# hyeeiin/ECG-Multimodal-Model

Hardware: AMD Instinct MI355X
Metric: samples/sec fwd+bwd, batch-256 multimodal (img+sig+clin), 1->8 MI355X (higher is better)
Workload: dtype bf16; 1 GPU; full multimodal (image 3x224x224 + 5000-pt signal + 16-dim clinical), fwd+bwd+Adam, encoders unfrozen; image_hw=224x224, per_gpu_batch=256, global_batch=256, parallelism=dp1

## Files before the change

ecg-multimodal-model_amd/csrc/api.hip:

```cpp
#include <stdarg.h>

#include "ops.h"

static thread_local char g_err[512] = "";

void ecg_set_error(const char* fmt, ...) {
  va_list ap;
  va_start(ap, fmt);
  vsnprintf(g_err, sizeof(g_err), fmt, ap);
  va_end(ap);
}

static inline ConvGeom geom_of(const ecgmm_conv_desc* c) {
  return make_geom(c->N, c->H, c->W, c->Cin, c->Cout, c->R, c->S, c->stride, c->pad_h, c->pad_w);
}
#define S_(x) ((hipStream_t)(x))

extern "C" {

int ecgmm_version(void) { return ECGMM_VERSION; }
const char* ecgmm_last_error(void) { return g_err; }

const char* ecgmm_switch_name(int i) { return i >= 0 && i < sw::COUNT ? sw::ALL[i]->env : nullptr; }
int ecgmm_switch_get(const char* env_name, int64_t* value) {
// ... 172 lines not shown
                      const float* addc, const void* y_a, const float* coef_a, const float* gamma_a, float* dgamma_a,
                      float* dbeta_a, void* dy_a, const void* y_b, const float* coef_b, const float* gamma_b,
                      float* dgamma_b, float* dbeta_b, void* dy_b, void* dz, float* dbias, int64_t M, int C, void* scratch_a,
                      void* scratch_b, void* stream) {
  return ecg_bn_bwd_dual(dtype, dout, maskref, mask_bits, gate, addc, y_a, coef_a, gamma_a, dgamma_a, dbeta_a, dy_a, y_b,
                         coef_b, gamma_b, dgamma_b, dbeta_b, dy_b, dz, dbias, (long)M, C, (float*)scratch_a, (float*)scratch_b,
                         S_(stream));
}

int ecgmm_conv_bwd_data_bnred(int dtype, const ecgmm_conv_desc* c, const void* dy, const void* w_dgrad,
                              const void* addend, void* dx, const void* bn_y, const void* bn_mask, const float* bn_coef,
                              float* rows, int* nrows, void* stream) {
  if (!bn_y || !bn_coef || !rows || !nrows) ECG_FAIL(ECGMM_ERR_SHAPE, "conv_bwd_data_bnred: null BatchNorm operand");
  const ConvGeom g = geom_of(c);
  *nrows = 0;
  if (!ecg_conv_halo_ok(dtype, 1, g))
    return ecg_conv_igemm(dtype, 1, g, dy, w_dgrad, dx, nullptr, addend, nullptr, 0, S_(stream));
  ConvEpi e = {};
  e.wg_rows = 1; e.red_y = bn_y; e.red_mask = bn_mask; e.red_coef = bn_coef; e.red_rows = rows;
  int rc = ecg_conv_igemm(dtype, 1, g, dy, w_dgrad, dx, nullptr, addend, nullptr, 0, S_(stream), &e);
  if (rc == 0 && e.red_done) *nrows = e.red_rows_n;
  return rc;
}
int ecgmm_conv_fwd_wgrows(int dtype, const ecgmm_conv_desc* c, const void* x, const void* w_fwd, const float* bias, void* y,
                          float* stats, int* nrows, int act, void* stream) {
  if (!stats || !nrows) ECG_FAIL(ECGMM_ERR_SHAPE, "conv_fwd_wgrows: null statistics buffer / row count");
  const ConvGeom g = geom_of(c);
  ConvEpi e = {};
  e.wg_rows = 1;
  int rc = ecg_conv_igemm(dtype, 0, g, x, w_fwd, y, bias, nullptr, stats, act, S_(stream), &e);
  *nrows = e.stats_rows > 0 ? e.stats_rows : ecg_conv_stats_rows((long)g.N * g.OH * g.OW);
  return rc;
}
int ecgmm_conv_bwd_data_bnred_rows(int dtype, const ecgmm_conv_desc* c) {
  const ConvGeom g = geom_of(c);
  return ecg_conv_halo_ok(dtype, 1, g) ? ecg_conv_halo_rows(1, g) : 0;
}
int ecgmm_conv_bwd_data_with_downsample(int dtype, const ecgmm_conv_desc* c, const void* dy, const void* w_dgrad,
                                        const void* dy_down, const void* w_down_dgrad, void* dx, void* tmp,
                                        void* stream) {
  if (!dy_down || !w_down_dgrad) ECG_FAIL(ECGMM_ERR_SHAPE, "conv_bwd_data_with_downsample: null downsample operand");
  const ConvGeom g = geom_of(c);
  if (g.stride != 2) ECG_FAIL(ECGMM_ERR_SHAPE, "conv_bwd_data_with_downsample: stride %d (the main convolution must have stride 2)", g.stride);
  ConvEpi e = {};
  e.src2 = dy_down; e.wpk2 = w_down_dgrad;
  ECG_TRY(ecg_conv_igemm(dtype, 1, g, dy, w_dgrad, dx, nullptr, nullptr, nullptr, 0, S_(stream), &e));
  if (e.src2_done) return 0;
  if (!tmp) ECG_FAIL(ECGMM_ERR_WORKSPACE, "conv_bwd_data_with_downsample: this geometry needs the temporary");
  ConvGeom gd = g;
  gd.R = gd.S = 1; gd.pad_h = gd.pad_w = 0;
  ECG_TRY(ecg_conv_igemm(dtype, 1, gd, dy_down, w_down_dgrad, tmp, nullptr, nullptr, nullptr, 0, S_(stream)));
  return ecg_conv_igemm(dtype, 1, g, dy, w_dgrad, dx, nullptr, tmp, nullptr, 0, S_(stream));
}
int ecgmm_bn_bwd_from_rows(int dtype, const void* dout, const void* maskref, const void* y, const float* coef,
                           const float* gamma, float* dgamma, float* dbeta, void* dy, const float* rows, int nrows,
                           int64_t M, int C, void* scratch, void* stream) {
  return ecg_bn_bwd_tail(dtype, dout, maskref, y, coef, gamma, dgamma, dbeta, dy, rows, nrows, (long)M, C,
                         (float*)scratch, S_(stream));
}

int ecgmm_bnrelu_maxpool(int dtype, const void* y, const float* coef, void* out, uint8_t* idx, int N, int H, int W,
                         int C, void* stream) {
  return ecg_bnrelu_maxpool(dtype, y, coef, out, idx, N, H, W, C, S_(stream));
}
int ecgmm_maxpool_relu_bwd(int dtype, const void* dp, const void* pooled, const uint8_t* idx, void* dz, int N, int H,
                           int W, int C, void* stream) {
  return ecg_maxpool_relu_bwd(dtype, dp, pooled, idx, dz, N, H, W, C, S_(stream));
}
int ecgmm_pool_bn_bwd(int dtype, const void* dp, const void* pooled, const uint8_t* idx, const void* y, const float* coef,
                      const float* gamma, float* dgamma, float* dbeta, void* dy, float* dbias, int N, int H, int W, int C,
                      void* scratch, void* stream) {
  return ecg_pool_bn_bwd(dtype, dp, pooled, idx, y, coef, gamma, dgamma, dbeta, dy, dbias, N, H, W, C, (float*)scratch,
                         S_(stream));
}
int ecgmm_conv_fwd_fused(int dtype, const ecgmm_conv_desc* c, const void* x, const void* w_fwd, const float* bias,
                         const void* addend, void* y, int act, void* stream) {
  if (dtype != ECGMM_BF16 && dtype != ECGMM_F32) ECG_FAIL(ECGMM_ERR_DTYPE, "conv_fwd_fused: bad dtype %d", dtype);
  if (!c || !x || !w_fwd || !y) ECG_FAIL(ECGMM_ERR_SHAPE, "conv_fwd_fused: null operand");
  if (act != ECGMM_ACT_NONE && act != ECGMM_ACT_RELU) ECG_FAIL(ECGMM_ERR_SHAPE, "conv_fwd_fused: act %d (none or ReLU)", act);
  if (c->N < 1 || c->H < 1 || c->W < 1 || c->Cin < 1 || c->Cout < 1 || c->R < 1 || c->S < 1 || c->stride < 1 ||
      c->pad_h < 0 || c->pad_w < 0 || c->H + 2 * c->pad_h < c->R || c->W + 2 * c->pad_w < c->S)
    ECG_FAIL(ECGMM_ERR_SHAPE, "conv_fwd_fused: bad geometry");
  return ecg_conv_igemm(dtype, 0, geom_of(c), x, w_fwd, y, bias, addend, nullptr, act, S_(stream));
}
int ecgmm_fold_conv_bn(int dtype, int layout, const float* w, const float* conv_bias, const float* gamma, const float* beta,
                       const float* running_mean, const float* running_var, float eps, void* w_out, float* b_out,
                       float* scale_out, int Cout, int Cin, int RS, void* stream) {
  if (layout != 0 && layout != 1) ECG_FAIL(ECGMM_ERR_SHAPE, "fold_conv_bn: layout %d (0 = forward pack, 1 = stem pack)", layout);
  if (dtype != ECGMM_BF16 && dtype != ECGMM_F32) ECG_FAIL(ECGMM_ERR_DTYPE, "fold_conv_bn: bad dtype %d", dtype);
  if (layout == 0 && RS > 9)
    ECG_FAIL(ECGMM_ERR_SHAPE, "fold_conv_bn: %d taps unsupported (1..9; a 5x5 convolution folds through ecgmm_fold_conv5_bn)", RS);
  EcgFoldItem it = {};
  it.kind = layout == 1 ? ECG_FOLD_STEM : ECG_FOLD_CONV;
  it.w = w; it.conv_bias = conv_bias; it.gamma = gamma; it.beta = beta; it.rm = running_mean; it.rv = running_var;
  it.wout = w_out; it.bout = b_out; it.scale_out = scale_out; it.Cout = Cout; it.Cin = Cin; it.RS = RS;
  return ecg_fold_batch(dtype, &it, 1, eps, S_(stream));
}
int ecgmm_fold_conv5_bn(int dtype, int layout, const float* w, const float* conv_bias, const float* gamma, const float* beta,
                        const float* running_mean, const float* running_var, float eps, void* w_out, float* b_out,
                        float* scale_out, int Cout, int Cin, void* stream) {
  if (layout != 0 && layout != 1)
    ECG_FAIL(ECGMM_ERR_SHAPE, "fold_conv5_bn: layout %d (0 = forward pack, 1 = OIHW fp32)", layout);
  EcgFoldItem it = {};
  it.kind = layout == 1 ? ECG_FOLD_OIHW : ECG_FOLD_CONV;
  it.w = w; it.conv_bias = conv_bias; it.gamma = gamma; it.beta = beta; it.rm = running_mean; it.rv = running_var;
  it.wout = w_out; it.bout = b_out; it.scale_out = scale_out; it.Cout = Cout; it.Cin = Cin; it.RS = 25;
// ... 193 lines not shown
```

ecg-multimodal-model_amd/csrc/common.h:

```cpp
#pragma once
#include <hip/hip_runtime.h>
#include <stdint.h>
#include <stdio.h>
#include <stdlib.h>
#include <string.h>

#include "../../include/ecgmm.h"

typedef unsigned short bf16_t;
typedef __attribute__((ext_vector_type(4))) float f32x4;
typedef __attribute__((ext_vector_type(8))) __bf16 bf16x8_t;
typedef __attribute__((ext_vector_type(4))) short s16x4;
typedef __attribute__((ext_vector_type(4))) unsigned int u32x4;

#define ECG_WAVE 64
#define ECG_TAIL_ROWS 64

void ecg_set_error(const char* fmt, ...);
#define ECG_FAIL(code, ...)       \
  do {                            \
    ecg_set_error(__VA_ARGS__);   \
    return (code);                \
  } while (0)
#define ECG_CHECK_LAUNCH(name)                                                     \
  do {                                                                             \
    hipError_t e_ = hipGetLastError();                                             \
    if (e_ != hipSuccess) ECG_FAIL(ECGMM_ERR_LAUNCH, "%s: %s", name, hipGetErrorString(e_)); \
  } while (0)
#define ECG_TRY(expr)             \
  do {                            \
    int rc_ = (expr);             \
    if (rc_ != 0) return rc_;     \
  } while (0)

__device__ __forceinline__ float bf2f(bf16_t v) { return __uint_as_float(((unsigned)v) << 16); }
__device__ __forceinline__ bf16_t f2bf(float f) {
  __bf16 b = (__bf16)f;
  return __builtin_bit_cast(bf16_t, b);
}

template <typename T> struct Elem;
template <> struct Elem<float> {
  static constexpr int VEC = 4;
  __device__ static __forceinline__ float ld(const float* p) { return *p; }
  __device__ static __forceinline__ void st(float* p, float v) { *p = v; }
};
template <> struct Elem<bf16_t> {
  static constexpr int VEC = 8;
  __device__ static __forceinline__ float ld(const bf16_t* p) { return bf2f(*p); }
  __device__ static __forceinline__ void st(bf16_t* p, float v) { *p = f2bf(v); }
};

template <typename T> __device__ __forceinline__ void unpack16(const u32x4& v, float* f);
template <> __device__ __forceinline__ void unpack16<float>(const u32x4& v, float* f) {
#pragma unroll
  for (int i = 0; i < 4; ++i) f[i] = __uint_as_float(v[i]);
}
template <> __device__ __forceinline__ void unpack16<bf16_t>(const u32x4& v, float* f) {
#pragma unroll
  for (int i = 0; i < 4; ++i) {
    f[2 * i] = __uint_as_float(v[i] << 16);
    f[2 * i + 1] = __uint_as_float(v[i] & 0xFFFF0000u);
  }
}
template <typename T> __device__ __forceinline__ u32x4 pack16(const float* f);
template <> __device__ __forceinline__ u32x4 pack16<float>(const float* f) {
  u32x4 v;
#pragma unroll
  for (int i = 0; i < 4; ++i) v[i] = __float_as_uint(f[i]);
  return v;
}
template <> __device__ __forceinline__ u32x4 pack16<bf16_t>(const float* f) {
  u32x4 v;
#pragma unroll
  for (int i = 0; i < 4; ++i) v[i] = (unsigned)f2bf(f[2 * i]) | ((unsigned)f2bf(f[2 * i + 1]) << 16);
  return v;
}

__device__ __forceinline__ float wave_sum(float v) {
#pragma unroll
  for (int o = 32; o > 0; o >>= 1) v += __shfl_xor(v, o, 64);
  return v;
}
__device__ __forceinline__ float wave_max(float v) {
#pragma unroll
  for (int o = 32; o > 0; o >>= 1) v = fmaxf(v, __shfl_xor(v, o, 64));
  return v;
}

template <int CTRL> __device__ __forceinline__ float dpp_mov(float v) {
  return __int_as_float(__builtin_amdgcn_update_dpp(0, __float_as_int(v), CTRL, 0xF, 0xF, true));
}
__device__ __forceinline__ float row16_sum(float v) {
  v += dpp_mov<0xB1>(v);
  v += dpp_mov<0x4E>(v);
  v += dpp_mov<0x141>(v);
  v += dpp_mov<0x140>(v);
  return v;
}

__device__ __forceinline__ void mfma_bf16_inplace(f32x4& acc, const u32x4& a, const u32x4& b) {
#if defined(__HIP_DEVICE_COMPILE__)
  asm volatile("s_nop 1\n\tv_mfma_f32_16x16x32_bf16 %0, %1, %2, %0" : "+a"(acc) : "v"(a), "v"(b));
#endif
}
__device__ __forceinline__ void mfma_bf16_first(f32x4& acc, const u32x4& a, const u32x4& b) {
#if defined(__HIP_DEVICE_COMPILE__)
  asm volatile("s_nop 1\n\tv_mfma_f32_16x16x32_bf16 %0, %1, %2, 0" : "=a"(acc) : "v"(a), "v"(b));
#endif
}
__device__ __forceinline__ void mfma_drain() {
#if defined(__HIP_DEVICE_COMPILE__)
  asm volatile("s_nop 7\n\ts_nop 7\n\ts_nop 3" ::: "memory");
#endif
}

static inline bool env_on(const char* name) { const char* e = getenv(name); return !(e && e[0] == '0'); }
static inline bool env_off(const char* name) { const char* e = getenv(name); return e && e[0] == '1'; }
static inline long env_int(const char* name, long def) { const char* e = getenv(name); return e ? atol(e) : def; }
static inline int env_level(const char* name, int hi, int def) {
  const char* e = getenv(name);
  return e && e[0] >= '0' && e[0] <= '0' + hi ? e[0] - '0' : def;
}

static inline int ceil_div(long a, long b) { return (int)((a + b - 1) / b); }
static inline size_t align_up(size_t a, size_t b) { return (a + b - 1) / b * b; }
static inline size_t dtype_size(int dt) { return dt == ECGMM_BF16 ? 2 : 4; }

struct ConvGeom {
  int N, H, W, Cin;
// ... 13 lines not shown
```

ecg-multimodal-model_amd/csrc/conv_halo.hip:

```cpp
#include <type_traits>

#include "ops.h"

namespace {

constexpr int HBM_ = 256;
constexpr unsigned H_OOB = 0x80000000u;

#ifdef ECG_STAMP
__device__ unsigned long long g_hstamp[8];
#define HSTAMP_AT(t)                                                          \
  do {                                                                        \
    __builtin_amdgcn_sched_barrier(0);                                        \
    asm volatile("s_memtime %0\n\ts_waitcnt lgkmcnt(0)" : "=s"(t)::"memory"); \
    __builtin_amdgcn_sched_barrier(0);                                        \
  } while (0)
#endif

struct HaloParams {
  const void* src;
  const void* wpk;
  void* dst;
  const float* bias;
  const void* addend;
  float* stats;
  const void* red_y;
  const void* red_mask;
  const float* red_coef;
  float* red_rows;
  int wg_rows;
  int M, H, W, Cs, Cd, ph, pw, act;
  int ncs;
  int HL;
  int hrows;
  int ntm;
  int ntn;
  int stagger;
  unsigned mul_hw, sh_hw, mul_w, sh_w;
};

__device__ __forceinline__ void hdma16(__amdgpu_buffer_rsrc_t rs, unsigned char* lds_wave_base, unsigned voffset,
                                       unsigned soffset) {
#if defined(__HIP_DEVICE_COMPILE__)
  __builtin_amdgcn_raw_ptr_buffer_load_lds(rs, (__attribute__((address_space(3))) void*)lds_wave_base, 16, voffset,
                                           soffset, 0, 0);
#endif
}

template <int N> __device__ __forceinline__ void wait_vmcnt() {
#if defined(__HIP_DEVICE_COMPILE__)
  asm volatile("s_waitcnt vmcnt(%0)" ::"n"(N) : "memory");
#endif
}
__device__ __forceinline__ void wait_lds() {
#if defined(__HIP_DEVICE_COMPILE__)
  __builtin_amdgcn_s_waitcnt(0xC07F);
#endif
}

typedef __attribute__((ext_vector_type(2))) float f32x2_t;
typedef __attribute__((ext_vector_type(2))) __bf16 bf16x2_t;
__device__ __forceinline__ unsigned pack_bf16x2(float lo, float hi) {
  return __builtin_bit_cast(unsigned, __builtin_convertvector((f32x2_t){lo, hi}, bf16x2_t));
}

template <int BN, int NW = 8> struct HaloCfg {
  static_assert(NW == 8 || (NW == 4 && BN == 64), "4-wave workgroups: 64-channel tiles only");
  static constexpr int HCAP = BN == 128 ? 320 : 384;
  static constexpr int HBUF = (HCAP + 8) * 128;
  static constexpr int NHB = NW == 8 ? 2 : 1;
  static constexpr int WSTAGE = BN * 128;
  static constexpr int NWS = NW == 8 ? 4 : 3;
  static constexpr int WBASE = NHB * HBUF;
  static constexpr int SBASE = WBASE + NWS * WSTAGE;
  static constexpr int CBASE = SBASE + 4 * 2 * BN * 4;
  static constexpr int TRASH = CBASE + 3 * BN * 4;
  static constexpr int MBASE = TRASH + 256;
  static constexpr int MBUF = 6 * 256 * 4;
  static constexpr int LDS = MBASE + (BN == 64 && NW == 8 ? 2 * MBUF : 0);
  static constexpr int WPS = BN / (8 * NW);
  static constexpr int NPW_MAX = HCAP / (8 * NW);
  static constexpr int WCN = NW / 4;
  static constexpr int CPW = BN / WCN;
};

template <int BN, int RS, int MODE, bool NCS1 = false, int NW = 8, bool PP = false, bool ST = false, bool AD = false>
__global__ __launch_bounds__(NW * 64, NW == 8 ? 2 : 2) void conv_halo_kernel(HaloParams p) {
  using C = HaloCfg<BN, NW>;
  static_assert(!ST || (BN == 64 && RS == 9 && NCS1 && NW == 8 && !PP && MODE != 1), "stream form: 64 -> 64 channel 3x3 tiles, no fused reduction");
  static_assert(!AD || (ST && MODE == 2), "AD = the stream form of the input gradient with a residual addend");
  static_assert(!PP || (NW == 8 && !NCS1), "ping-pong: 8-wave workgroups");
  static_assert(!(NCS1 && NW == 4), "one halo buffer: the next tile's halo cannot stream in during the K loop");
  static_assert(NW == 8 || RS % 3 == 0, "3-slot ring: the slot of a step is its tap index mod 3");
  constexpr int HTHREADS = NW * 64;
  constexpr int D = C::NWS - 1;
  constexpr int TP = 4;
  constexpr int TC = C::CPW / 16;
#ifndef HALO_HPS9
#define HALO_HPS9 1
#endif
  constexpr int HPS = RS == 9 ? HALO_HPS9 : C::NPW_MAX;
  extern __shared__ __attribute__((aligned(16))) unsigned char smem[];

  const int tid = threadIdx.x;
  const int lane = tid & 63;
  const int wv = __builtin_amdgcn_readfirstlane(tid >> 6);
  const int wp = wv & 3, wc = wv >> 2;
  const bool late = !PP && NW == 8 && BN == 64 && p.stagger != 0 && wv >= 4;
  auto slot_of = [](int g, int t) -> int { return C::NWS == 4 ? (g & 3) : (t % 3); };
  auto hbuf_of = [](int q) -> unsigned { return C::NHB == 2 ? (unsigned)(q & 1) * C::HBUF : 0u; };
  const int fr = lane & 15, fq = lane >> 4;
  const int G = gridDim.x;
  const int nt = (int)blockIdx.x % p.ntn, kq = (int)blockIdx.x / p.ntn, Gk = G / p.ntn;
  const int n0 = nt * BN;
  const unsigned pixb = (unsigned)p.Cs * 2u;
  const __amdgpu_buffer_rsrc_t rs_src = __builtin_amdgcn_make_buffer_rsrc((void*)p.src, 0, (int)((size_t)p.M * pixb), 0x00020000);
  const __amdgpu_buffer_rsrc_t rs_w = __builtin_amdgcn_make_buffer_rsrc(
      (void*)p.wpk, 0, (int)((size_t)p.Cd * RS * p.Cs * 2), 0x00020000);

  const int lrow8 = lane >> 3;
  const unsigned lchunkb = (unsigned)(((lane & 7) ^ lrow8) << 4);
  unsigned hoff[C::NPW_MAX];
  auto set_hoff = [&](int m0) {
#pragma unroll
    for (int kk = 0; kk < C::NPW_MAX; ++kk) {
      const int row = (kk * NW + wv) * 8 + lrow8;
      const int pix = m0 - p.HL + row;
      const bool ok = row < p.hrows && pix >= 0 && pix < p.M;
      hoff[kk] = ok ? (unsigned)pix * pixb + lchunkb : H_OOB;
    }
  };
  auto set_wrow = [&](unsigned (&wr)[C::WPS], int n0) {
#pragma unroll
    for (int i = 0; i < C::WPS; ++i) wr[i] = (unsigned)(n0 + (i * NW + wv) * 8 + lrow8) * (unsigned)RS * pixb + lchunkb;
  };
  auto dma_halo = [&](unsigned hbuf, int cs, int k0, int k1) {
#pragma unroll
    for (int kk = 0; kk < C::NPW_MAX; ++kk)
      if (kk >= k0 && kk < k1) hdma16(rs_src, smem + hbuf + (kk * NW + wv) * 1024, hoff[kk], (unsigned)cs * 128u);
  };
  auto dma_w = [&](const unsigned (&wr)[C::WPS], int slot, int cs, int t) {
// ... 96 lines not shown
        acc[a][b] = __builtin_amdgcn_mfma_f32_16x16x32_bf16(__builtin_bit_cast(bf16x8_t, fa[a]),
                                                            __builtin_bit_cast(bf16x8_t, fb[b]), (f32x4){0.f, 0.f, 0.f, 0.f}, 0, 0, 0);
    __builtin_amdgcn_s_setprio(0);
  };
  auto mma = [&](const u32x4 (&fa)[TC], const u32x4 (&fb)[TP]) {
#if defined(HALO_ABL) && HALO_ABL == 1
#pragma unroll
    for (int a = 0; a < TC; ++a) asm volatile("" ::"v"(fa[a]));
#pragma unroll
    for (int b = 0; b < TP; ++b) asm volatile("" ::"v"(fb[b]));
    return;
#endif
    __builtin_amdgcn_s_setprio(1);
#pragma unroll
    for (int a = 0; a < TC; ++a)
#pragma unroll
      for (int b = 0; b < TP; ++b)
        acc[a][b] = __builtin_amdgcn_mfma_f32_16x16x32_bf16(__builtin_bit_cast(bf16x8_t, fa[a]),
                                                            __builtin_bit_cast(bf16x8_t, fb[b]), acc[a][b], 0, 0, 0);
    __builtin_amdgcn_s_setprio(0);
  };

  int mt = kq;
  int m0 = mt * HBM_;
  unsigned wrow[C::WPS];
  set_wrow(wrow, n0);
  int g0 = 0;
  int qs = 0;
  auto tile_fills = [&](int m0_, bool with_halo) {
    if (with_halo) {
      set_hoff(m0_);
      dma_halo(hbuf_of(qs), 0, 0, C::NPW_MAX);
    }
#pragma unroll
    for (int t = 0; t < D; ++t) dma_w(wrow, slot_of(g0 + t, t), 0, t);
  };
  if (tid < 8 * C::NHB) *reinterpret_cast<u32x4*>(smem + (tid >> 3) * C::HBUF + C::HCAP * 128 + (tid & 7) * 16) = (u32x4){0u, 0u, 0u, 0u};
  float* const sacc = reinterpret_cast<float*>(smem + C::SBASE);
  for (int i = tid; i < 4 * 2 * BN; i += HTHREADS) sacc[i] = 0.f;
  float* const scoef = reinterpret_cast<float*>(smem + C::CBASE);
  if (MODE == 1 && p.red_y)
    for (int i = tid; i < 3 * BN; i += HTHREADS) scoef[i] = p.red_coef[(i / BN) * p.Cd + n0 + (i % BN)];
  tile_fills(m0, true);

  u32x4 fa0[TC], fb0[TP], fa1[TC], fb1[TP];

  const bf16_t* const pf_base[3] = {(const bf16_t*)p.addend, MODE == 1 ? (const bf16_t*)p.red_y : nullptr,
                                    MODE == 1 && p.red_mask != p.red_y ? (const bf16_t*)p.red_mask : nullptr};
  auto prefetch_epilogue_operands = [&]() {
#if defined(__HIP_DEVICE_COMPILE__)
    const size_t e = (size_t)(m0 + wp * 64 + lane) * p.Cd + n0 + wc * C::CPW;
#pragma unroll
    for (int k = 0; k < 3; ++k) {
      const bf16_t* g = pf_base[k] ? pf_base[k] + e : (const bf16_t*)p.wpk;
      __builtin_amdgcn_global_load_lds((const __attribute__((address_space(1))) void*)g,
                                       (__attribute__((address_space(3))) void*)(smem + C::TRASH), 4, 0, 0);
    }
#endif
  };

  auto slice = [&](int cs, auto last_tag) {
    constexpr bool LAST = decltype(last_tag)::value;
    const unsigned hb = hbuf_of(qs), hbn = hbuf_of(qs + 1);
#pragma unroll
    for (int b = 0; b < TP; ++b)
#pragma unroll
      for (int t2 = 0; t2 < RSP; ++t2) asm volatile("" : "+v"(baddr[b][t2]));
#pragma unroll
    for (int t = 0; t < RS; ++t) {
      const int s = g0 + t;
      ld_a(fa1, slot_of(s, t), 64u);
#pragma unroll
      for (int b = 0; b < TP; ++b) fb1[b] = ld_b((bad(b, t) ^ 64u) + hb);
      const auto n_halo = [](int tt, bool last) { return (!(last && !NCS1) && tt < RS - 1 && tt * HPS < C::NPW_MAX)
                                                      ? ((tt + 1) * HPS < C::NPW_MAX ? HPS : C::NPW_MAX - tt * HPS) : 0; };
      const auto n_fill = [&](int tt, bool last) {
        return ((last && tt + D >= RS) ? 0 : C::WPS) + n_halo(tt, last) + ((last && tt == 0) ? 3 : 0);
      };
      const bool wrap = t + D >= RS;
      if (LAST && t == 0) prefetch_epilogue_operands();
#if !(defined(HALO_ABL) && HALO_ABL == 3)
      if (!(LAST && wrap)) dma_w(wrow, slot_of(s + D, (t + D) % RS), cs + (wrap ? 1 : 0), (t + D) % RS);
      if (n_halo(t, LAST) > 0) dma_halo(hbn, NCS1 ? 0 : cs + 1, t * HPS, (t + 1) * HPS);
#endif
      if (!late) mma(fa0, fb0);
      const int outstanding = (D == 3 ? (t == 0 ? n_fill(RS - 1, false) : n_fill(t - 1, LAST)) : 0) + n_fill(t, LAST);
      if (outstanding == 0) wait_vmcnt<0>();
      else if (outstanding == 1) wait_vmcnt<1>();
      else if (outstanding == 2) wait_vmcnt<2>();
      else if (outstanding == 3) wait_vmcnt<3>();
      else if (outstanding == 4) wait_vmcnt<4>();
      else if (outstanding == 5) wait_vmcnt<5>();
      else if (outstanding == 6) wait_vmcnt<6>();
      else if (outstanding == 7) wait_vmcnt<7>();
      else if (outstanding == 8) wait_vmcnt<8>();
      else if (outstanding == 9) wait_vmcnt<9>();
      else if (outstanding == 10) wait_vmcnt<10>();
      else if (outstanding == 11) wait_vmcnt<11>();
      else if (outstanding == 12) wait_vmcnt<12>();
      else if (outstanding == 13) wait_vmcnt<13>();
      else if (outstanding == 14) wait_vmcnt<14>();
      else if (outstanding == 15) wait_vmcnt<15>();
      else wait_vmcnt<0>();
      wait_lds();
#if !(defined(HALO_ABL) && HALO_ABL == 5)
      __builtin_amdgcn_s_barrier();
#endif
// ... 72 lines not shown
  constexpr bool RACC = BN == 64 && MODE == 0 && NW == 8;
#endif
  constexpr int TA_ = TC / 2;
  float rs1[RACC && MODE == 0 ? TC : 1][4], rs2[RACC && MODE == 0 ? TC : 1][4];
  float rq1[RACC && MODE == 1 ? TA_ : 1][8], rq2[RACC && MODE == 1 ? TA_ : 1][8];
#pragma unroll
  for (int a = 0; a < (RACC && MODE == 0 ? TC : 1); ++a)
#pragma unroll
    for (int j = 0; j < 4; ++j) rs1[a][j] = rs2[a][j] = 0.f;
#pragma unroll
  for (int a = 0; a < (RACC && MODE == 1 ? TA_ : 1); ++a)
#pragma unroll
    for (int j = 0; j < 8; ++j) rq1[a][j] = rq2[a][j] = 0.f;
  const bool racc = RACC && p.wg_rows != 0;
  bool first_tile = true;
#ifdef ECG_STAMP
  unsigned long long hs_a, hs_b, hs_c, hs_d, hs_e, hs_w0, hs_acc[4] = {0, 0, 0, 0}, hs_tiles = 0, hs_bar = 0;
  HSTAMP_AT(hs_w0);
#endif
  if constexpr (ST) {
    auto produce_masks = [&](int m0_, unsigned buf) {
      const int pixel = tid & 255;
      const int q = m0_ + pixel;
      const int n = (int)(((unsigned long long)(unsigned)q * p.mul_hw) >> p.sh_hw), rem = q - n * HW;
      const int h = (int)(((unsigned long long)(unsigned)rem * p.mul_w) >> p.sh_w), w = rem - h * p.W;
      const unsigned first_r = MODE == 0 ? 0x007u : 0x1C0u, last_r = MODE == 0 ? 0x1C0u : 0x007u;
      const unsigned first_s = MODE == 0 ? 0x049u : 0x124u, last_s = MODE == 0 ? 0x124u : 0x049u;
      unsigned v = 0x1FFu;
      v &= h == 0 ? ~first_r : ~0u;
      v &= h == p.H - 1 ? ~last_r : ~0u;
      v &= w == 0 ? ~first_s : ~0u;
      v &= w == p.W - 1 ? ~last_s : ~0u;
      const int k0 = wc * 3;
      unsigned* tb = reinterpret_cast<unsigned*>(smem + C::MBASE + buf * C::MBUF) + k0 * 256 + pixel;
#pragma unroll
      for (int j = 0; j < 3; ++j) {
        const unsigned lo = (unsigned)__builtin_amdgcn_sbfe((int)v, 2 * (k0 + j), 1) & 0xFFFFu;
        const unsigned hi = (unsigned)__builtin_amdgcn_sbfe((int)v, 2 * (k0 + j) + 1, 1) & 0xFFFF0000u;
        tb[j * 256] = lo | hi;
      }
    };
    unsigned mk[TP];
    const unsigned mlane = (unsigned)C::MBASE + (unsigned)(wp * 64 + fr) * 4u;
    auto fetch_masks = [&](int t2, unsigned buf) {
#pragma unroll
      for (int b = 0; b < TP; ++b) mk[b] = *reinterpret_cast<const unsigned*>(smem + mlane + buf * C::MBUF + t2 * 1024 + b * 64);
    };
    auto rebuild = [&](int t2) {
      const unsigned zz = zaddr | (zaddr << 16);
#pragma unroll
      for (int b = 0; b < TP; ++b) baddr[b][t2] = (avalid[b][t2] & mk[b]) | (zz & ~mk[b]);
    };
    constexpr auto st_ = [](int t) { t = (t + RS) % RS; return AD ? (t >= 4 && t <= 7 ? 1 : 0) : (t >= 1 && t <= 4 ? 1 : 0); };
    constexpr auto ld_ = [](int t) { t = (t + RS) % RS; return AD && t >= 1 && t <= 4 ? 1 : 0; };
    constexpr auto pf_ = [](int t) { t = (t + RS) % RS; return AD && t == 5 ? 1 : 0; };
    constexpr auto ex_ = [=](int t) { return st_(t) + ld_(t) + pf_(t); };
    constexpr auto hl_ = [](int t) { t = (t + RS) % RS; return t < C::NPW_MAX ? 1 : 0; };
    static_assert(C::NPW_MAX <= RS - 1 && HPS == 1, "one halo piece per step, none in the tile's last step");
    const int cw = n0 + wc * C::CPW;
    const int cl = (fq & 1) ? 16 + (fq - 1) * 4 : fq * 4;
    f32x4 accp[TC][TP];
    static_assert(TC == 2, "one channel-tile pair per wave");
    u32x4 adv[3];
    auto load_addend = [&](int b, int m0_) {
      adv[b % 3] = *reinterpret_cast<const u32x4*>(addend + (size_t)(m0_ + wp * 64 + b * 16 + fr) * p.Cd + cw + cl);
    };
    auto prefetch_addend = [&](int m0_) {
#if defined(__HIP_DEVICE_COMPILE__)
      __builtin_amdgcn_global_load_lds((const __attribute__((address_space(1))) void*)(addend + (size_t)(m0_ + wp * 64 + lane) * p.Cd + cw),
                                       (__attribute__((address_space(3))) void*)(smem + C::TRASH), 4, 0, 0);
#endif
    };
    auto epi_unit = [&](int b, int m0_) {
#if defined(__HIP_DEVICE_COMPILE__)
      f32x4 v0 = accp[0][b], v1 = accp[1][b];
      if constexpr (AD) {
        const u32x4 ao = adv[b % 3];
        auto ax = __builtin_amdgcn_permlane16_swap(ao[0], ao[2], false, false);
        auto ay = __builtin_amdgcn_permlane16_swap(ao[1], ao[3], false, false);
        v0 += (f32x4){__uint_as_float(ax[0] << 16), __uint_as_float(ax[0] & 0xFFFF0000u), __uint_as_float(ay[0] << 16), __uint_as_float(ay[0] & 0xFFFF0000u)};
        v1 += (f32x4){__uint_as_float(ax[1] << 16), __uint_as_float(ax[1] & 0xFFFF0000u), __uint_as_float(ay[1] << 16), __uint_as_float(ay[1] & 0xFFFF0000u)};
      }
      if constexpr (MODE == 0) {
        if (b < TC) {
          f32x4 t1, t2;
#pragma unroll
          for (int bb = 0; bb < TP; ++bb) {
            const f32x4 v = accp[b][bb];
#pragma unroll
            for (int j = 0; j < 4; ++j) {
              t1[j] = bb == 0 ? v[j] : t1[j] + v[j];
              t2[j] = __builtin_fmaf(v[j], v[j], bb == 0 ? 0.f : t2[j]);
            }
          }
#pragma unroll
          for (int j = 0; j < 4; ++j) {
            rs1[b][j] += t1[j];
            rs2[b][j] += t2[j];
          }
        }
      }
      const unsigned x0 = pack_bf16x2(v0[0], v0[1]), y0 = pack_bf16x2(v0[2], v0[3]);
      const unsigned x1 = pack_bf16x2(v1[0], v1[1]), y1 = pack_bf16x2(v1[2], v1[3]);
      auto lo = __builtin_amdgcn_permlane16_swap(x0, x1, false, false);
      auto hi = __builtin_amdgcn_permlane16_swap(y0, y1, false, false);
#if defined(HALO_ABL) && HALO_ABL == 11
      asm volatile("" ::"v"(lo[0]), "v"(hi[0]), "v"(lo[1]), "v"(hi[1]));
      __builtin_amdgcn_global_load_lds((const __attribute__((address_space(1))) void*)p.wpk,
                                       (__attribute__((address_space(3))) void*)(smem + C::TRASH), 4, 0, 0);
#else
      *reinterpret_cast<u32x4*>(dst + (size_t)(m0_ + wp * 64 + b * 16 + fr) * p.Cd + cw + cl) = (u32x4){lo[0], hi[0], lo[1], hi[1]};
#endif
#endif
    };
    auto dummy_vm = [&]() {
#if defined(__HIP_DEVICE_COMPILE__)
      __builtin_amdgcn_global_load_lds((const __attribute__((address_space(1))) void*)p.wpk,
                                       (__attribute__((address_space(3))) void*)(smem + C::TRASH), 4, 0, 0);
#endif
    };
    set_baddr(m0);
    produce_masks(m0, 0u);
    set_hoff(mt + Gk < p.ntm ? (mt + Gk) * HBM_ : p.M + 4 * HBM_);
    wait_vmcnt<0>();
    wait_lds();
    __builtin_amdgcn_s_barrier();
    ld_a(fa0, slot_of(g0, 0), 0u);
#pragma unroll
    for (int b = 0; b < TP; ++b) fb0[b] = ld_b(bad(b, 0) + hbuf_of(qs));
#pragma unroll
    for (int a = 0; a < TC; ++a)
#pragma unroll
      for (int b = 0; b < TP; ++b) accp[a][b] = (f32x4){0.f, 0.f, 0.f, 0.f};
    int m0_prev = m0;
    for (;;) {
      const bool more = mt + Gk < p.ntm;
      const int m0n = (mt + Gk) * HBM_;
      const unsigned hb = hbuf_of(qs), hbn = hbuf_of(qs + 1);
      const unsigned mcur = (unsigned)(qs & 1);
#pragma unroll
      for (int b = 0; b < TP; ++b)
#pragma unroll
        for (int t2 = 0; t2 < RSP; ++t2) asm volatile("" : "+v"(baddr[b][t2]));
#pragma unroll
      for (int t = 0; t < RS; ++t) {
        const int s = g0 + t;
        if (t == 0) fetch_masks(4, mcur);
        if (t == 2 || t == 4 || t == 6 || t == 8) fetch_masks(t / 2 - 1, mcur ^ 1u);
        ld_a(fa1, slot_of(s, t), 64u);
#pragma unroll
        for (int b = 0; b < TP; ++b) fb1[b] = ld_b((bad(b, t) ^ 64u) + hb);
#if !(defined(HALO_ABL) && HALO_ABL == 13)
        dma_w(wrow, slot_of(s + D, (t + D) % RS), 0, (t + D) % RS);
        if (hl_(t)) dma_halo(hbn, 0, t, t + 1);
#endif
        auto extra = [&]() {
          if (st_(t)) {
#if defined(HALO_ABL) && HALO_ABL == 10
            dummy_vm();
#else
            epi_unit(AD ? t - 4 : t - 1, m0_prev);
#endif
          }
          if (ld_(t)) load_addend(t - 1, m0_prev);
// ... 104 lines not shown
      {
        const unsigned hb = hbuf_of(qs);
#pragma unroll
        for (int b = 0; b < TP; ++b) fb0[b] = ld_b(bad(b, 0) + hb);
      }
      for (int cs = 0; cs + 1 < p.ncs; ++cs) slice(cs, F_{});
      slice(p.ncs - 1, T_{});
    }
#pragma unroll
    for (int a = 0; a < TC; ++a)
#pragma unroll
      for (int b = 0; b < TP; ++b) asm volatile("" : "+v"(acc[a][b]));
    __builtin_amdgcn_sched_barrier(0);
#ifdef ECG_STAMP
    HSTAMP_AT(hs_d);
#endif
    const bool more = mt + Gk < p.ntm;
    const int mt_cur = mt, m0_cur = m0, n0_cur = n0;
    if (more) {
      mt += Gk;
      m0 = mt * HBM_;
    }

#if !(defined(HALO_ABL) && HALO_ABL == 4)
    {
      constexpr int TA = TC / 2;
      const bf16_t* __restrict__ red_y = MODE == 1 ? (const bf16_t*)p.red_y : nullptr;
      const bf16_t* __restrict__ red_m = MODE == 1 ? (const bf16_t*)p.red_mask : nullptr;
      const bool red = red_y != nullptr, red_sep = red && red_m != red_y;
      const int cw = n0_cur + wc * C::CPW;
      const int cl = (fq & 1) ? 16 + (fq - 1) * 4 : fq * 4;
      size_t prow[TP];
#pragma unroll
      for (int b = 0; b < TP; ++b) prow[b] = (size_t)(m0_cur + wp * 64 + b * 16 + fr) * p.Cd + cw;
      float s1[TC][4], s2[TC][4];
      float q1[TA][8], q2[TA][8];
      f32x4 bias4[TC];
#pragma unroll
      for (int a = 0; a < TC; ++a) {
#pragma unroll
        for (int j = 0; j < 4; ++j) s1[a][j] = s2[a][j] = 0.f;
        bias4[a] = p.bias ? *reinterpret_cast<const f32x4*>(p.bias + cw + a * 16 + fq * 4) : (f32x4){0.f, 0.f, 0.f, 0.f};
      }
#pragma unroll
      for (int ap = 0; ap < TA; ++ap)
#pragma unroll
        for (int j = 0; j < 8; ++j) q1[ap][j] = q2[ap][j] = 0.f;
      auto unpk = [](unsigned lo, unsigned hi) -> f32x4 {
        return (f32x4){__uint_as_float(lo << 16), __uint_as_float(lo & 0xFFFF0000u), __uint_as_float(hi << 16),
                       __uint_as_float(hi & 0xFFFF0000u)};
      };
      uint2 adv[2][TC][2];
      u32x4 yq[2][TA][2], mq[2][TA][2], oq[2][TA][2];
      auto loads = [&](auto h_tag) {
        constexpr int h = decltype(h_tag)::value;
#pragma unroll
        for (int bb = 0; bb < 2; ++bb) {
          const int b = h * 2 + bb;
          if (addend) {
#pragma unroll
            for (int a = 0; a < TC; ++a) adv[h][a][bb] = *reinterpret_cast<const uint2*>(addend + prow[b] + a * 16 + fq * 4);
          }
          if (MODE == 1 && red) {
#pragma unroll
            for (int ap = 0; ap < TA; ++ap) {
              yq[h][ap][bb] = *reinterpret_cast<const u32x4*>(red_y + prow[b] + ap * 32 + cl);
              if (red_sep) mq[h][ap][bb] = *reinterpret_cast<const u32x4*>(red_m + prow[b] + ap * 32 + cl);
            }
          }
        }
      };
      auto compute = [&](auto h_tag) {
        constexpr int h = decltype(h_tag)::value;
#if defined(__HIP_DEVICE_COMPILE__)
#pragma unroll
        for (int ap = 0; ap < TA; ++ap) {
          const int a = 2 * ap;
          f32x4 c_sc[2], c_sh[2], c_mu[2];
          if (MODE == 1 && red) {
            const float* cf = scoef + wc * C::CPW + ap * 32 + cl;
            c_sc[0] = *reinterpret_cast<const f32x4*>(cf); c_sc[1] = *reinterpret_cast<const f32x4*>(cf + 4);
            c_sh[0] = *reinterpret_cast<const f32x4*>(cf + BN); c_sh[1] = *reinterpret_cast<const f32x4*>(cf + BN + 4);
            c_mu[0] = *reinterpret_cast<const f32x4*>(cf + 2 * BN); c_mu[1] = *reinterpret_cast<const f32x4*>(cf + 2 * BN + 4);
          }
#pragma unroll
          for (int bb = 0; bb < 2; ++bb) {
            const int b = h * 2 + bb;
            f32x4 v0 = acc[a][b], v1 = acc[a + 1][b];
            if (p.bias) {
              v0 += bias4[a];
              v1 += bias4[a + 1];
            }
            if (addend) {
              v0 += unpk(adv[h][a][bb].x, adv[h][a][bb].y);
              v1 += unpk(adv[h][a + 1][bb].x, adv[h][a + 1][bb].y);
            }
            if (p.act == 1) {
#pragma unroll
              for (int j = 0; j < 4; ++j) {
                v0[j] = fmaxf(v0[j], 0.f);
                v1[j] = fmaxf(v1[j], 0.f);
              }
            }
            if (MODE == 0) {
#pragma unroll
              for (int j = 0; j < 4; ++j) {
                s1[a][j] += v0[j];
                s2[a][j] = __builtin_fmaf(v0[j], v0[j], s2[a][j]);
                s1[a + 1][j] += v1[j];
                s2[a + 1][j] = __builtin_fmaf(v1[j], v1[j], s2[a + 1][j]);
              }
            }
            const unsigned x0 = pack_bf16x2(v0[0], v0[1]), y0 = pack_bf16x2(v0[2], v0[3]);
            const unsigned x1 = pack_bf16x2(v1[0], v1[1]), y1 = pack_bf16x2(v1[2], v1[3]);
            auto lo = __builtin_amdgcn_permlane16_swap(x0, x1, false, false);
            auto hi = __builtin_amdgcn_permlane16_swap(y0, y1, false, false);
            u32x4 o = (u32x4){lo[0], hi[0], lo[1], hi[1]};
            if (MODE == 1 && red) {
              const f32x4 d[2] = {unpk(o[0], o[1]), unpk(o[2], o[3])};
              const u32x4 yr = yq[h][ap][bb];
              const f32x4 yv[2] = {unpk(yr[0], yr[1]), unpk(yr[2], yr[3])};
              f32x4 g[2];
              if (red_sep) {
                const u32x4 mr = mq[h][ap][bb];
                const f32x4 mv[2] = {unpk(mr[0], mr[1]), unpk(mr[2], mr[3])};
#pragma unroll
                for (int u = 0; u < 2; ++u)
#pragma unroll
                  for (int j = 0; j < 4; ++j) g[u][j] = mv[u][j] > 0.f ? d[u][j] : 0.f;
                o = (u32x4){pack_bf16x2(g[0][0], g[0][1]), pack_bf16x2(g[0][2], g[0][3]), pack_bf16x2(g[1][0], g[1][1]),
                            pack_bf16x2(g[1][2], g[1][3])};
              } else {
#pragma unroll
                for (int u = 0; u < 2; ++u)
#pragma unroll
                  for (int j = 0; j < 4; ++j) g[u][j] = (yv[u][j] * c_sc[u][j] + c_sh[u][j]) > 0.f ? d[u][j] : 0.f;
              }
#pragma unroll
              for (int u = 0; u < 2; ++u)
#pragma unroll
                for (int j = 0; j < 4; ++j) {
                  q1[ap][u * 4 + j] += g[u][j];
                  q2[ap][u * 4 + j] += g[u][j] * (yv[u][j] - c_mu[u][j]);
                }
            }
            oq[h][ap][bb] = o;
          }
        }
#endif
      };
      auto stores = [&](auto h_tag) {
        constexpr int h = decltype(h_tag)::value;
#if defined(HALO_ABL) && HALO_ABL == 6
#pragma unroll
        for (int ap = 0; ap < TA; ++ap)
#pragma unroll
          for (int bb = 0; bb < 2; ++bb) asm volatile("" ::"v"(oq[h][ap][bb]));
        return;
#endif
#pragma unroll
        for (int ap = 0; ap < TA; ++ap)
#pragma unroll
          for (int bb = 0; bb < 2; ++bb) *reinterpret_cast<u32x4*>(dst + prow[h * 2 + bb] + ap * 32 + cl) = oq[h][ap][bb];
      };
      using H0 = std::integral_constant<int, 0>;
      using H1 = std::integral_constant<int, 1>;
      if (addend == nullptr && !red) {
        if (more) tile_fills(m0, !NCS1);
        __builtin_amdgcn_sched_barrier(0);
        compute(H0{});
        stores(H0{});
        compute(H1{});
        stores(H1{});
      } else {
        loads(H0{});
        compute(H0{});
        loads(H1{});
        __builtin_amdgcn_sched_barrier(0);
        if (more) tile_fills(m0, !NCS1);
        __builtin_amdgcn_sched_barrier(0);
        stores(H0{});
        compute(H1{});
        stores(H1{});
      }
#if defined(HALO_ABL) && HALO_ABL == 7
      if (false) {
#else
      if ((MODE == 0 && p.stats) || (MODE == 1 && red)) {
#endif
        float* lrow = sacc + wp * 2 * BN + wc * C::CPW;
        if (RACC && racc) {
          if constexpr (RACC && MODE == 0) {
#pragma unroll
            for (int a = 0; a < TC; ++a)
#pragma unroll
              for (int j = 0; j < 4; ++j) {
                rs1[a][j] += s1[a][j];
                rs2[a][j] += s2[a][j];
              }
          }
          if constexpr (RACC && MODE == 1) {
#pragma unroll
            for (int ap = 0; ap < TA; ++ap)
#pragma unroll
              for (int j = 0; j < 8; ++j) {
                rq1[ap][j] += q1[ap][j];
                rq2[ap][j] += q2[ap][j];
              }
          }
        } else if (MODE == 0) {
          float* srow = p.stats + (size_t)(mt_cur * 4 + wp) * 2 * p.Cd + cw + fq * 4;
#pragma unroll
          for (int a = 0; a < TC; ++a) {
            f32x4 r1, r2;
#pragma unroll
            for (int j = 0; j < 4; ++j) {
              r1[j] = row16_sum(s1[a][j]);
              r2[j] = row16_sum(s2[a][j]);
            }
            if (fr == 0) {
// ... 72 lines not shown
      for (int ap = 0; ap < TA_; ++ap) {
        f32x4 r1[2], r2[2];
#pragma unroll
        for (int j = 0; j < 8; ++j) {
          r1[j >> 2][j & 3] = row16_sum(rq1[ap][j]);
          r2[j >> 2][j & 3] = row16_sum(rq2[ap][j]);
        }
        if (fr == 0) {
#pragma unroll
          for (int u = 0; u < 2; ++u) {
            *reinterpret_cast<f32x4*>(lrow + ap * 32 + cl + u * 4) = r1[u];
            *reinterpret_cast<f32x4*>(lrow + BN + ap * 32 + cl + u * 4) = r2[u];
          }
        }
      }
    }
  }
  if (p.wg_rows && (p.stats || p.red_y)) {
    __syncthreads();
    float* rows = p.red_y ? p.red_rows : p.stats;
    for (int i = tid; i < 2 * BN; i += HTHREADS) {
      const int which = i / BN, c = i - which * BN;
      const float v = ((sacc[0 * 2 * BN + i] + sacc[1 * 2 * BN + i]) + sacc[2 * 2 * BN + i]) + sacc[3 * 2 * BN + i];
      rows[((size_t)kq * 2 + which) * p.Cd + n0 + c] = v;
    }
  }
}

void halo_magic_div(unsigned d, unsigned& m, unsigned& sh) {
  int l = 0;
  while ((1u << l) < d) ++l;
  m = (unsigned)(((1ull << (31 + l)) + d - 1) / d);
  sh = 31 + l;
}
int halo_gk(int ntn, int ntm, int wg_per_cu = 1) {
  static int ncu[16] = {0};
  int dev = 0, cus = 256;
  (void)hipGetDevice(&dev);
  if (dev >= 0 && dev < 16) {
    if (ncu[dev] == 0) {
      hipDeviceProp_t prop;
      ncu[dev] = hipGetDeviceProperties(&prop, dev) == hipSuccess && prop.multiProcessorCount > 0 ? prop.multiProcessorCount : 256;
    }
    cus = ncu[dev];
  }
  const long cu_cap = sw::HALO_CUS.get();
  if (cu_cap > 0 && cus > cu_cap) cus = (int)cu_cap;
  int Gk = cus * wg_per_cu / (ntn < 1 ? 1 : ntn);
  if (Gk > ntm) Gk = ntm;
  if (Gk > 512) Gk = 512;
  return Gk < 1 ? 1 : Gk;
}

template <int BN, int RS, int MODE, bool NCS1 = false, int NW = 8, bool PP = false, bool ST = false, bool AD = false>
int launch_halo(const HaloParams& p, int* rows_out, hipStream_t stream) {
  using C = HaloCfg<BN, NW>;
  static bool attr_set[16] = {false};
  int dev = 0;
  (void)hipGetDevice(&dev);
  if (dev >= 0 && dev < 16 && !attr_set[dev]) {
    if (hipFuncSetAttribute((const void*)conv_halo_kernel<BN, RS, MODE, NCS1, NW, PP, ST, AD>, hipFuncAttributeMaxDynamicSharedMemorySize,
                            C::LDS) != hipSuccess)
      ECG_FAIL(ECGMM_ERR_LAUNCH, "conv_halo: cannot reserve %d bytes of LDS", C::LDS);
    attr_set[dev] = true;
  }
  HaloParams q = p;
  q.ntm = p.M / HBM_;
  q.ntn = p.Cd / BN;
  const int Gk = halo_gk(q.ntn, q.ntm, NW == 4 ? 2 : 1);
  *rows_out = Gk;
  hipLaunchKernelGGL((conv_halo_kernel<BN, RS, MODE, NCS1, NW, PP, ST, AD>), dim3(Gk * q.ntn), dim3(NW * 64), C::LDS, stream, q);
  ECG_CHECK_LAUNCH("conv_halo_kernel");
  return 0;
}

}

#ifdef ECG_STAMP
extern "C" int ecgmm_hstamp_read(unsigned long long* out8, int reset) {
  if (hipMemcpyFromSymbol(out8, HIP_SYMBOL(g_hstamp), sizeof(g_hstamp)) != hipSuccess) return 1;
  if (reset) {
    unsigned long long z[8] = {0};
    if (hipMemcpyToSymbol(HIP_SYMBOL(g_hstamp), z, sizeof(z)) != hipSuccess) return 1;
  }
  return 0;
}
#endif

bool ecg_conv_halo_ok(int dtype, int mode, const ConvGeom& g) {
  const long level = sw::CONV_HALO.get();
  if (!level || dtype != ECGMM_BF16 || g.stride != 1 || g.S != 3) return false;
  if (!((g.R == 3 && g.pad_h == 1) || (g.R == 1 && g.pad_h == 0)) || g.pad_w != 1) return false;
  if (g.OH != g.H || g.OW != g.W) return false;
  const int Cs = mode == 0 ? g.Cin : g.Cout, Cd = mode == 0 ? g.Cout : g.Cin;
  const long M = (long)g.N * g.H * g.W;
  if (M % HBM_ != 0 || Cs % 64 != 0 || Cd % 64 != 0 || (Cd > 64 && Cd % 128 != 0)) return false;
  const int HL = g.pad_h * g.W + g.pad_w, hrows = 256 + 2 * HL;
  if (hrows > (Cd > 64 ? HaloCfg<128>::HCAP : HaloCfg<64>::HCAP)) return false;
  if ((double)M * Cs * 2.0 > 2.0e9 || (double)M * Cd * 2.0 > 8.0e9) return false;
  if (level == 2) return true;
  return g.R == 3 || Cs >= 128;
}

static bool halo_w4(const ConvGeom& g, int Cs, int Cd) {
  return sw::HALO_W4.get() && g.R == 3 && Cs == 64 && Cd == 64;
}
int ecg_conv_halo_rows(int mode, const ConvGeom& g) {
  const int Cd = mode == 0 ? g.Cout : g.Cin;
  const int ntn = Cd > 64 ? Cd / 128 : 1, ntm = g.N * g.H * g.W / HBM_;
  return halo_gk(ntn, ntm, 1);
}

int ecg_conv_halo(int mode, const ConvGeom& g, const void* src, const void* wpk, void* dst, const float* bias,
                  const void* addend, float* stats, int act, ConvEpi* epi, hipStream_t stream) {
  HaloParams p;
  memset(&p, 0, sizeof(p));
  p.src = src; p.wpk = wpk; p.dst = dst; p.bias = bias; p.addend = addend; p.stats = stats; p.act = act;
  p.M = g.N * g.H * g.W; p.H = g.H; p.W = g.W; p.ph = g.pad_h; p.pw = g.pad_w;
  p.Cs = mode == 0 ? g.Cin : g.Cout;
  p.Cd = mode == 0 ? g.Cout : g.Cin;
  p.ncs = p.Cs / 64;
  p.HL = g.pad_h * g.W + g.pad_w;
  p.hrows = 256 + 2 * p.HL;
  halo_magic_div((unsigned)(g.H * g.W), p.mul_hw, p.sh_hw);
  halo_magic_div((unsigned)g.W, p.mul_w, p.sh_w);
  if (epi) {
    p.wg_rows = epi->wg_rows;
    if (epi->red_y) {
      if (stats || !epi->red_coef || !epi->red_rows || !epi->wg_rows)
        ECG_FAIL(ECGMM_ERR_SHAPE, "conv_halo: fused BatchNorm-backward reduction needs coefficients, rows, wg_rows and no forward statistics");
      p.red_y = epi->red_y; p.red_mask = epi->red_mask ? epi->red_mask : epi->red_y; p.red_coef = epi->red_coef;
      p.red_rows = epi->red_rows;
    }
  }
  p.stagger = (int)sw::HALO_STAGGER.get();
  int wg = 0;
  const bool wide = p.Cd > 64;
  int rc;
  if (halo_w4(g, p.Cs, p.Cd) && !p.red_y) {
    if (mode == 0) rc = launch_halo<64, 9, 0, false, 4>(p, &wg, stream);
    else rc = launch_halo<64, 9, 2, false, 4>(p, &wg, stream);
  } else if (g.R == 3 && !wide && p.ncs == 1 && sw::HALO_NCS1.get()) {
    const bool st = sw::HALO_STREAM.get() != 0;
    if (mode == 0 && st && (!p.stats || p.wg_rows) && !p.addend && !p.bias && p.act != 1) rc = launch_halo<64, 9, 0, true, 8, false, true>(p, &wg, stream);
    else if (mode != 0 && st && !p.red_y && !p.addend && !p.bias && p.act != 1) rc = launch_halo<64, 9, 2, true, 8, false, true>(p, &wg, stream);
    else if (mode != 0 && st && !p.red_y && p.addend && !p.bias && p.act != 1) rc = launch_halo<64, 9, 2, true, 8, false, true, true>(p, &wg, stream);
    else if (mode == 0) rc = launch_halo<64, 9, 0, true>(p, &wg, stream);
    else if (p.red_y) rc = launch_halo<64, 9, 1, true>(p, &wg, stream);
    else rc = launch_halo<64, 9, 2, true>(p, &wg, stream);
  } else if (wide && g.R == 3 && sw::HALO_PP.get()) {
    if (mode == 0) rc = launch_halo<128, 9, 0, false, 8, true>(p, &wg, stream);
    else if (p.red_y) rc = launch_halo<128, 9, 1, false, 8, true>(p, &wg, stream);
    else rc = launch_halo<128, 9, 2, false, 8, true>(p, &wg, stream);
  } else if (g.R == 3) {
    if (mode == 0) rc = wide ? launch_halo<128, 9, 0>(p, &wg, stream) : launch_halo<64, 9, 0>(p, &wg, stream);
    else if (p.red_y) rc = wide ? launch_halo<128, 9, 1>(p, &wg, stream) : launch_halo<64, 9, 1>(p, &wg, stream);
    else rc = wide ? launch_halo<128, 9, 2>(p, &wg, stream) : launch_halo<64, 9, 2>(p, &wg, stream);
  } else {
    if (mode == 0) rc = wide ? launch_halo<128, 3, 0>(p, &wg, stream) : launch_halo<64, 3, 0>(p, &wg, stream);
    else if (p.red_y) rc = wide ? launch_halo<128, 3, 1>(p, &wg, stream) : launch_halo<64, 3, 1>(p, &wg, stream);
    else rc = wide ? launch_halo<128, 3, 2>(p, &wg, stream) : launch_halo<64, 3, 2>(p, &wg, stream);
  }
  if (epi) {
    epi->stats_rows = p.wg_rows ? wg : 2 * ceil_div(p.M, 128);
    epi->red_done = p.red_y != nullptr;
    epi->red_rows_n = p.red_y ? wg : 0;
  }
  return rc;
}
```

ecg-multimodal-model_amd/csrc/conv_igemm.hip:

```cpp
#include "ops.h"

namespace {

template <typename T> struct Mma;
template <> struct Mma<bf16_t> {
  static __device__ __forceinline__ void run(f32x4& acc, const u32x4& a, const u32x4& b) {
    acc = __builtin_amdgcn_mfma_f32_16x16x32_bf16(__builtin_bit_cast(bf16x8_t, a), __builtin_bit_cast(bf16x8_t, b),
                                                  acc, 0, 0, 0);
  }
};
template <> struct Mma<float> {
  static __device__ __forceinline__ void run(f32x4& acc, const u32x4& a, const u32x4& b) {
#pragma unroll
    for (int j = 0; j < 4; ++j)
      acc = __builtin_amdgcn_mfma_f32_16x16x4f32(__uint_as_float(a[j]), __uint_as_float(b[j]), acc, 0, 0, 0);
  }
};

__device__ __forceinline__ void dma16(__amdgpu_buffer_rsrc_t rs, unsigned char* lds_wave_base, unsigned voffset) {
#if defined(__HIP_DEVICE_COMPILE__)
  __builtin_amdgcn_raw_ptr_buffer_load_lds(rs, (__attribute__((address_space(3))) void*)lds_wave_base, 16, voffset, 0, 0,
                                           0);
#endif
}

struct IgemmParams {
  const void* src;
  const void* wpk;
  void* dst;
  const float* bias;
  const void* addend;
  float* stats;
  int Nimg, Hs, Ws, Cs, Hd, Wd, Cd, R, S, stride, pad_h, pad_w;
  int M;
  int act;
  const void* src2;
  const void* wpk2;
  unsigned mul_hw[4], sh_hw[4], mul_w[4], sh_w[4];
};

#ifdef ECG_STAMP
__device__ unsigned long long g_stamp[8];
#define ECG_STAMP_AT(t)                                                                   \
  do {                                                                                    \
    __builtin_amdgcn_sched_barrier(0);                                                    \
    asm volatile("s_memtime %0\n\ts_waitcnt lgkmcnt(0)" : "=s"(t)::"memory");             \
    __builtin_amdgcn_sched_barrier(0);                                                    \
  } while (0)
#endif

constexpr int BM = 128;
constexpr int ROWB = 128;
constexpr int NTHREADS = 256;

template <typename T, int BN, int MODE, int ST>
__global__ __launch_bounds__(NTHREADS) void igemm_kernel(IgemmParams p) {
  constexpr int VEC = Elem<T>::VEC;
  constexpr int KBE = ROWB / (int)sizeof(T);
  constexpr int TP = 4;
  constexpr int TC = BN / 32;
  constexpr int NWV = BN / 32;
  extern __shared__ __attribute__((aligned(16))) unsigned char smem[];
  constexpr int STAGE_BYTES = (BN + BM) * ROWB;

  const int tid = threadIdx.x;
  const int lane = tid & 63, wave = tid >> 6;
  const int wp = wave & 1, wc = wave >> 1;
  int mt;
  {
    const int nwg = gridDim.x, q = nwg >> 3, r = nwg & 7, xcd = blockIdx.x & 7, k = blockIdx.x >> 3;
    mt = (xcd < r ? xcd * (q + 1) : r * (q + 1) + (xcd - r) * q) + k;
  }
  const int m0 = mt * BM, n0 = blockIdx.y * BN;
  const T* __restrict__ src = (const T*)p.src;
  const T* __restrict__ wpk = (const T*)p.wpk;

  const int wv = __builtin_amdgcn_readfirstlane(wave);
  const int lrow8 = lane >> 3;
  const int lchunk = (lane & 7) ^ (lrow8 & 7);
  constexpr bool PAR = (MODE == 1 && ST == 2);
  constexpr int TSTEP = PAR ? 2 : 1;
  int ph = 0, pw = 0, Hc = p.Hd, Wc = p.Wd, r0 = 0, s0 = 0, Rc = p.R, Sc = p.S, Mc = p.M;
  const int cz = PAR ? (p.Hd > 1 ? 3 - (int)blockIdx.z : (int)blockIdx.z) : 0;
  if (PAR) {
    ph = cz >> 1;
    pw = cz & 1;
    Hc = (p.Hd - ph + 1) >> 1;
    Wc = (p.Wd - pw + 1) >> 1;
    r0 = (ph + p.pad_h) & 1;
    s0 = (pw + p.pad_w) & 1;
    Rc = p.R > r0 ? (p.R - r0 + 1) >> 1 : 0;
    Sc = p.S > s0 ? (p.S - s0 + 1) >> 1 : 0;
    Mc = p.Nimg * Hc * Wc;
    if (m0 >= Mc) return;
  }
  const int HWd = Hc * Wc;
  const int cls = PAR ? cz : 0;
  const unsigned mhw = p.mul_hw[cls], shw = p.sh_hw[cls], mw = p.mul_w[cls], sw_ = p.sh_w[cls];
  auto div_hw = [&](int x) -> int { return (int)(((unsigned long long)(unsigned)x * mhw) >> shw); };
  auto div_w = [&](int x) -> int { return (int)(((unsigned long long)(unsigned)x * mw) >> sw_); };
  const int n_first = div_hw(m0);
  const size_t img_elems = (size_t)p.Hs * p.Ws * p.Cs;
  const size_t left = ((size_t)p.Nimg - n_first) * img_elems * sizeof(T);
  const __amdgpu_buffer_rsrc_t rs_src = __builtin_amdgcn_make_buffer_rsrc(
      (void*)(src + (size_t)n_first * img_elems), 0, left > 0xFFFFFFF0ull ? (int)0xFFFFFFF0u : (int)left, 0x00020000);
  const __amdgpu_buffer_rsrc_t rs_w = __builtin_amdgcn_make_buffer_rsrc(
      (void*)wpk, 0, (int)((size_t)p.Cd * p.R * p.S * p.Cs * sizeof(T)), 0x00020000);
  constexpr unsigned OOB = 0xFFFFFFFFu;
  constexpr int SGN = MODE == 0 ? 1 : -1;
// ... 41 lines not shown
      left > 0xFFFFFFF0ull ? (int)0xFFFFFFF0u : (int)left, 0x00020000);
  const __amdgpu_buffer_rsrc_t rs_w2 = __builtin_amdgcn_make_buffer_rsrc(
      (void*)(has2 ? p.wpk2 : p.wpk), 0, (int)((size_t)p.Cd * p.Cs * sizeof(T)), 0x00020000);
  int g_n = 0;

  int g_r = 0, g_s = 0, g_cc = 0;
  auto dma = [&](int stage) {
    unsigned char* sW = smem + stage * STAGE_BYTES;
    unsigned char* sX = sW + BN * ROWB;
    if (PAR && g_n >= nk_main) {
      const int ch = (g_n - nk_main) * KBE + lchunk * VEC;
      const unsigned chb = ch < p.Cs ? (unsigned)ch * (unsigned)sizeof(T) : OOB;
#pragma unroll
      for (int i = 0; i < 4; ++i) {
        const bool ok = (unsigned)hq[i] < (unsigned)p.Hs && (unsigned)wq[i] < (unsigned)p.Ws;
        dma16(rs_src2, sX + (wv * 4 + i) * 1024, (ok && chb != OOB) ? offb[i] + chb : OOB);
      }
#pragma unroll
      for (int i = 0; i < NWV; ++i)
        dma16(rs_w2, sW + (wv * NWV + i) * 1024, (wrow[i] != OOB && chb != OOB) ? wrow[i] / (unsigned)RS + chb : OOB);
      ++g_n;
      return;
    }
    ++g_n;
    const int r = r0 + g_r * TSTEP, s = s0 + g_s * TSTEP;
    const int ch = g_cc * KBE + lchunk * VEC;
    const unsigned chb = ch < p.Cs ? (unsigned)ch * (unsigned)sizeof(T) : OOB;
    const unsigned tapd = (unsigned)(SGN * (g_r * p.Ws + g_s)) * pix_bytes;
#pragma unroll
    for (int i = 0; i < 4; ++i) {
      const bool ok = (unsigned)(hq[i] + SGN * g_r) < (unsigned)p.Hs && (unsigned)(wq[i] + SGN * g_s) < (unsigned)p.Ws;
      dma16(rs_src, sX + (wv * 4 + i) * 1024, (ok && chb != OOB) ? offb[i] + tapd + chb : OOB);
    }
    const unsigned tapb = (unsigned)(r * p.S + s) * pix_bytes + chb;
#pragma unroll
    for (int i = 0; i < NWV; ++i)
      dma16(rs_w, sW + (wv * NWV + i) * 1024, (wrow[i] != OOB && chb != OOB) ? wrow[i] + tapb : OOB);
    if (++g_cc == cpt) {
      g_cc = 0;
      if (++g_s == Sc) {
        g_s = 0;
        ++g_r;
      }
    }
  };

  f32x4 acc[TC][TP];
#pragma unroll
  for (int a = 0; a < TC; ++a)
#pragma unroll
    for (int b = 0; b < TP; ++b) acc[a][b] = (f32x4){0.f, 0.f, 0.f, 0.f};

  const int fr = lane & 15, fq = lane >> 4;
  auto compute = [&](int stage) {
    const unsigned char* sW = smem + stage * STAGE_BYTES;
    const unsigned char* sX = sW + BN * ROWB;
#pragma unroll
    for (int ks = 0; ks < 2; ++ks) {
      u32x4 fa[TC], fb[TP];
      const int lch = ks * 4 + fq;
#pragma unroll
      for (int a = 0; a < TC; ++a) {
        int row = wc * (BN / 2) + a * 16 + fr;
        fa[a] = *reinterpret_cast<const u32x4*>(sW + row * ROWB + ((lch ^ (row & 7)) << 4));
      }
#pragma unroll
      for (int b = 0; b < TP; ++b) {
        int row = wp * 64 + b * 16 + fr;
        fb[b] = *reinterpret_cast<const u32x4*>(sX + row * ROWB + ((lch ^ (row & 7)) << 4));
      }
      if (BN == 128) __builtin_amdgcn_s_setprio(1);
#pragma unroll
      for (int a = 0; a < TC; ++a)
#pragma unroll
        for (int b = 0; b < TP; ++b) Mma<T>::run(acc[a][b], fa[a], fb[b]);
      if (BN == 128) __builtin_amdgcn_s_setprio(0);
    }
  };

  if (nk > 0) {
    dma(0);
    __syncthreads();
  }
#ifdef ECG_STAMP
  unsigned long long sA = 0, sB = 0, sC = 0, t0, t1, t2, t3, tk0, tk1;
  ECG_STAMP_AT(tk0);
#endif
  for (int it = 0; it < nk; ++it) {
#ifdef ECG_STAMP
    ECG_STAMP_AT(t0);
#endif
    if (it + 1 < nk) dma((it + 1) & 1);
#ifdef ECG_STAMP
    ECG_STAMP_AT(t1);
#endif
    compute(it & 1);
#ifdef ECG_STAMP
    ECG_STAMP_AT(t2);
#endif
    __syncthreads();
#ifdef ECG_STAMP
    ECG_STAMP_AT(t3);
    sA += t1 - t0; sB += t2 - t1; sC += t3 - t2;
#endif
  }
#ifdef ECG_STAMP
// ... 24 lines not shown
        prow[b] = (size_t)pix * p.Cd + n0 + wc * (BN / 2);
      }
      float s1[TC][4], s2[TC][4];
      f32x4 bias4[TC];
#pragma unroll
      for (int a = 0; a < TC; ++a) {
#pragma unroll
        for (int j = 0; j < 4; ++j) s1[a][j] = s2[a][j] = 0.f;
        bias4[a] = p.bias ? *reinterpret_cast<const f32x4*>(p.bias + n0 + wc * (BN / 2) + a * 16 + fq * 4)
                          : (f32x4){0.f, 0.f, 0.f, 0.f};
      }
#ifdef ECG_STAMP
      unsigned long long tf0;
      ECG_STAMP_AT(tf0);
#endif
#pragma unroll
      for (int a = 0; a < TC; a += 2)
#pragma unroll
        for (int b = 0; b < TP; ++b) {
          f32x4 v0 = acc[a][b], v1 = acc[a + 1][b];
          if (p.bias) {
            v0 += bias4[a];
            v1 += bias4[a + 1];
          }
          if (addend) {
            const T* ap = addend + prow[b] + fq * 4;
            const uint2 p0 = *reinterpret_cast<const uint2*>(ap + a * 16), p1 = *reinterpret_cast<const uint2*>(ap + (a + 1) * 16);
            v0 += (f32x4){__uint_as_float(p0.x << 16), __uint_as_float(p0.x & 0xFFFF0000u), __uint_as_float(p0.y << 16),
                          __uint_as_float(p0.y & 0xFFFF0000u)};
            v1 += (f32x4){__uint_as_float(p1.x << 16), __uint_as_float(p1.x & 0xFFFF0000u), __uint_as_float(p1.y << 16),
                          __uint_as_float(p1.y & 0xFFFF0000u)};
          }
          if (p.act == 1) {
#pragma unroll
            for (int j = 0; j < 4; ++j) {
              v0[j] = fmaxf(v0[j], 0.f);
              v1[j] = fmaxf(v1[j], 0.f);
            }
          }
#pragma unroll
          for (int j = 0; j < 4; ++j) {
            s1[a][j] += v0[j];
            s2[a][j] += v0[j] * v0[j];
            s1[a + 1][j] += v1[j];
            s2[a + 1][j] += v1[j] * v1[j];
          }
          const unsigned x0 = (unsigned)f2bf(v0[0]) | ((unsigned)f2bf(v0[1]) << 16);
          const unsigned y0 = (unsigned)f2bf(v0[2]) | ((unsigned)f2bf(v0[3]) << 16);
          const unsigned x1 = (unsigned)f2bf(v1[0]) | ((unsigned)f2bf(v1[1]) << 16);
          const unsigned y1 = (unsigned)f2bf(v1[2]) | ((unsigned)f2bf(v1[3]) << 16);
          auto lo = __builtin_amdgcn_permlane16_swap(x0, x1, false, false);
          auto hi = __builtin_amdgcn_permlane16_swap(y0, y1, false, false);
          const int ch = (fq & 1) ? (a + 1) * 16 + (fq - 1) * 4 : a * 16 + fq * 4;
          *reinterpret_cast<u32x4*>(dst + prow[b] + ch) = (u32x4){lo[0], hi[0], lo[1], hi[1]};
        }
#ifdef ECG_STAMP
      unsigned long long tf1;
      ECG_STAMP_AT(tf1);
      if (threadIdx.x == 0) {
        atomicAdd(&g_stamp[7], tf1 - tf0);
      }
#endif
      if (p.stats) {
        float* srow = p.stats + (size_t)(mt * 2 + wp) * 2 * p.Cd + n0 + wc * (BN / 2) + fq * 4;
#pragma unroll
        for (int a = 0; a < TC; ++a) {
          f32x4 r1, r2;
#pragma unroll
          for (int j = 0; j < 4; ++j) {
            r1[j] = row16_sum(s1[a][j]);
            r2[j] = row16_sum(s2[a][j]);
          }
          if (fr == 0) {
            *reinterpret_cast<f32x4*>(srow + a * 16) = r1;
            *reinterpret_cast<f32x4*>(srow + p.Cd + a * 16) = r2;
          }
        }
      }
#ifdef ECG_STAMP
      ECG_STAMP_AT(te1);
#endif
    }
  }
#endif
  if (!fast) {
  uint2 opk[TC][TP];
  int wpix[TP];
#pragma unroll
  for (int a = 0; a < TC; ++a) {
    const int ch0 = n0 + wc * (BN / 2) + a * 16 + fq * 4;
    float bv[4] = {0.f, 0.f, 0.f, 0.f};
    if (p.bias) {
#pragma unroll
      for (int j = 0; j < 4; ++j)
        if (ch0 + j < p.Cd) bv[j] = p.bias[ch0 + j];
    }
    float s1[4] = {0.f, 0.f, 0.f, 0.f}, s2[4] = {0.f, 0.f, 0.f, 0.f};
#pragma unroll
    for (int b = 0; b < TP; ++b) {
      int pix = m0 + wp * 64 + b * 16 + fr;
      const bool pok = pix < Mc;
      if (PAR) {
        int pp = pok ? pix : m0;
        int n = div_hw(pp);
        int rem = pp - n * HWd;
        int h2 = div_w(rem), w2 = rem - h2 * Wc;
        pix = (n * p.Hd + h2 * 2 + ph) * p.Wd + w2 * 2 + pw;
// ... 66 lines not shown
          if (ch0 + j < p.Cd) {
            row[ch0 + j] = s1[j];
            row[p.Cd + ch0 + j] = s2[j];
          }
      }
    }
  }
#ifdef ECG_STAMP
  ECG_STAMP_AT(te1);
#endif
  if (wide) {
#if defined(__HIP_DEVICE_COMPILE__)
#pragma unroll
    for (int a = 0; a < TC; a += 2)
#pragma unroll
      for (int b = 0; b < TP; ++b) {
        auto lo = __builtin_amdgcn_permlane16_swap(opk[a][b].x, opk[a + 1][b].x, false, false);
        auto hi = __builtin_amdgcn_permlane16_swap(opk[a][b].y, opk[a + 1][b].y, false, false);
        const int ch = n0 + wc * (BN / 2) + ((fq & 1) ? (a + 1) * 16 + (fq - 1) * 4 : a * 16 + fq * 4);
        if (wpix[b] >= 0 && n0 + wc * (BN / 2) + a * 16 < p.Cd)
          *reinterpret_cast<u32x4*>(dst + (size_t)wpix[b] * p.Cd + ch) = (u32x4){lo[0], hi[0], lo[1], hi[1]};
      }
#endif
  }
  }
#ifdef ECG_STAMP
  {
    unsigned long long te;
    ECG_STAMP_AT(te);
    if (threadIdx.x == 0) {
      atomicAdd(&g_stamp[0], sA);
      atomicAdd(&g_stamp[1], sB);
      atomicAdd(&g_stamp[2], sC);
      atomicAdd(&g_stamp[3], te1 - tk1);
      atomicAdd(&g_stamp[4], tk1 - tk0);
      atomicAdd(&g_stamp[5], te - tk1);
      atomicAdd(&g_stamp[6], 1ull);
    }
  }
#endif
}

#ifdef ECG_STAMP
extern "C" int ecgmm_stamp_read(unsigned long long* out8, int reset) {
  if (hipMemcpyFromSymbol(out8, HIP_SYMBOL(g_stamp), sizeof(g_stamp)) != hipSuccess) return 1;
  if (reset) {
    unsigned long long z[8] = {0};
    if (hipMemcpyToSymbol(HIP_SYMBOL(g_stamp), z, sizeof(z)) != hipSuccess) return 1;
  }
  return 0;
}
#endif

template <typename T, int BN, int MODE, int ST>
int launch_one(const IgemmParams& p, hipStream_t stream) {
  dim3 grid(ceil_div(p.M, BM), ceil_div(p.Cd, BN));
  if (MODE == 1 && ST == 2) {
    long mc = (long)p.Nimg * ((p.Hd + 1) / 2) * ((p.Wd + 1) / 2);
    grid = dim3(ceil_div(mc, BM), ceil_div(p.Cd, BN), 4);
  }
  size_t lds = 2 * (size_t)(BN + BM) * ROWB;
  static bool attr_set = false;
  if (!attr_set) {
    (void)hipFuncSetAttribute((const void*)igemm_kernel<T, BN, MODE, ST>, hipFuncAttributeMaxDynamicSharedMemorySize,
                        (int)lds);
    attr_set = true;
  }
  hipLaunchKernelGGL((igemm_kernel<T, BN, MODE, ST>), grid, dim3(NTHREADS), lds, stream, p);
  ECG_CHECK_LAUNCH("igemm_kernel");
  return 0;
}

template <typename T>
int launch_T(const IgemmParams& p, int mode, hipStream_t stream) {
  const bool wide = p.Cd > 64;
  if (mode == 0) return wide ? launch_one<T, 128, 0, 1>(p, stream) : launch_one<T, 64, 0, 1>(p, stream);
  if (p.stride == 1) return wide ? launch_one<T, 128, 1, 1>(p, stream) : launch_one<T, 64, 1, 1>(p, stream);
  if (p.stride == 2) return wide ? launch_one<T, 128, 1, 2>(p, stream) : launch_one<T, 64, 1, 2>(p, stream);
  ECG_FAIL(ECGMM_ERR_SHAPE, "conv dgrad: stride %d unsupported (1 or 2)", p.stride);
}

}

int ecg_conv_stats_rows(long M) { return 2 * ceil_div(M, BM); }

static inline double conv_flops(const ConvGeom& g) {
  return 2.0 * (double)g.N * g.OH * g.OW * g.Cout * g.R * g.S * g.Cin;
}

int ecg_conv_igemm(int dtype, int mode, const ConvGeom& g, const void* src, const void* wpk, void* dst,
                   const float* bias, const void* addend, float* stats, int act, hipStream_t stream, ConvEpi* epi) {
  IgemmParams p;
  memset(&p, 0, sizeof(p));
  p.src = src; p.wpk = wpk; p.dst = dst; p.bias = bias; p.addend = addend; p.stats = stats; p.act = act;
  p.Nimg = g.N; p.R = g.R; p.S = g.S; p.stride = g.stride; p.pad_h = g.pad_h; p.pad_w = g.pad_w;
  if (mode == 0) {
    p.Hs = g.H; p.Ws = g.W; p.Cs = g.Cin; p.Hd = g.OH; p.Wd = g.OW; p.Cd = g.Cout;
  } else {
    p.Hs = g.OH; p.Ws = g.OW; p.Cs = g.Cout; p.Hd = g.H; p.Wd = g.W; p.Cd = g.Cin;
  }
  long M = (long)g.N * p.Hd * p.Wd;
  if (M <= 0 || M > 0x7fffffffL) ECG_FAIL(ECGMM_ERR_SHAPE, "conv: pixel count %ld out of range", M);
  {
    auto magic = [](unsigned d, unsigned& m, unsigned& sh) {
      if (d < 1) d = 1;
      int l = 0;
      while ((1u << l) < d) ++l;
      m = (unsigned)(((1ull << (31 + l)) + d - 1) / d);
      sh = 31 + l;
    };
    const bool par = mode == 1 && g.stride == 2;
    for (int c = 0; c < 4; ++c) {
      const int ph_ = par ? c >> 1 : 0, pw_ = par ? c & 1 : 0;
      const int Hc_ = par ? (p.Hd - ph_ + 1) >> 1 : p.Hd, Wc_ = par ? (p.Wd - pw_ + 1) >> 1 : p.Wd;
      magic((unsigned)(Hc_ * Wc_), p.mul_hw[c], p.sh_hw[c]);
      magic((unsigned)Wc_, p.mul_w[c], p.sh_w[c]);
    }
  }
  p.M = (int)M;
  const int vec = dtype == ECGMM_BF16 ? 8 : 4;
  if (p.Cs % vec != 0) ECG_FAIL(ECGMM_ERR_SHAPE, "conv: reduction channels %d not a multiple of %d", p.Cs, vec);
  if (dtype != ECGMM_BF16 && dtype != ECGMM_F32) ECG_FAIL(ECGMM_ERR_DTYPE, "conv: bad dtype %d", dtype);
  {
    const double esz = (double)dtype_size(dtype);
    double bytes = esz * ((double)g.N * p.Hs * p.Ws * p.Cs + (double)M * p.Cd * (addend ? 2.0 : 1.0) +
                          (double)g.R * g.S * g.Cin * g.Cout);
    if (epi && epi->red_y) bytes += esz * (double)M * p.Cd * (epi->red_mask ? 2.0 : 1.0);
    if (epi && epi->src2 && mode == 1 && g.stride == 2) bytes += esz * ((double)g.N * p.Hs * p.Ws * p.Cs + (double)g.Cin * g.Cout);
    ecg_prof_begin(dtype == ECGMM_F32 ? (mode == 0 ? ECG_PROF_IGEMM_F32_FWD : ECG_PROF_IGEMM_F32_DGRAD)
                                      : (mode == 0 ? ECG_PROF_IGEMM_FWD : ECG_PROF_IGEMM_DGRAD),
                   conv_flops(g), bytes, stream);
  }
  if (epi) epi->src2_done = 0;
  if (epi && epi->src2 && mode == 1 && g.stride == 2 && g.pad_h <= 1 && g.pad_w <= 1 && !addend) {
    p.src2 = epi->src2; p.wpk2 = epi->wpk2;
    epi->src2_done = 1;
  }
  int rc;
  if (ecg_conv_halo_ok(dtype, mode, g)) {
    rc = ecg_conv_halo(mode, g, src, wpk, dst, bias, addend, stats, act, epi, stream);
  } else {
    if (epi) {
      epi->stats_rows = ecg_conv_stats_rows(M);
      epi->red_done = 0;
      epi->red_rows_n = 0;
    }
    rc = dtype == ECGMM_BF16 ? launch_T<bf16_t>(p, mode, stream) : launch_T<float>(p, mode, stream);
  }
  ecg_prof_end(stream);
  return rc;
}
```

ecg-multimodal-model_amd/csrc/elementwise.hip:

```cpp
#include "ops.h"

namespace {

constexpr int EW_THREADS = 256;

__device__ __forceinline__ u32x4 ld16(const void* p) { return *reinterpret_cast<const u32x4*>(p); }
__device__ __forceinline__ u32x4 ld16s(const void* p) {
#ifndef EW_NO_NT
  return __builtin_nontemporal_load(reinterpret_cast<const u32x4*>(p));
#else
  return *reinterpret_cast<const u32x4*>(p);
#endif
}
struct RowDiv { unsigned mul, sh; };
__device__ __forceinline__ long row_div(long r, RowDiv d) { return (long)(((unsigned long long)(unsigned)r * d.mul) >> d.sh); }
static RowDiv make_row_div(int d) {
  unsigned dd = d < 1 ? 1u : (unsigned)d;
  int l = 0;
  while ((1u << l) < dd) ++l;
  RowDiv r;
  r.mul = (unsigned)(((1ull << (31 + l)) + dd - 1) / dd);
  r.sh = 31u + (unsigned)l;
  return r;
}
// ... 529 lines not shown
  const T* ya = (const T*)p.y[0];
  const T* yb = (const T*)p.y[1];
  const long rfirst = (long)blockIdx.x * rpi + r0;
  const float* bc[2] = {p.bcoef[0] + c0, p.bcoef[1] + c0};
  int bcs = p.C;
  u32x4 pd = {}, pa = {}, pb = {};
  bool pre = APPLY && p.fin[0].partial != nullptr && rfirst < p.M;
  if (pre) {
    pd = ld16s(dout + rfirst * p.C + c0);
    pa = ld16s(ya + rfirst * p.C + c0);
    pb = ld16s(yb + rfirst * p.C + c0);
  }
  if (APPLY && p.fin[0].partial) {
    bn_bwd_fin_prologue<BWD_THREADS>(p.fin[0], p.coef[0], p.C, cs, s_bcoef, s_red);
    bn_bwd_fin_prologue<BWD_THREADS>(p.fin[1], p.coef[1], p.C, cs, s_bcoef + 3 * 512, s_red);
    bc[0] = s_bcoef + chunk * VEC;
    bc[1] = s_bcoef + 3 * 512 + chunk * VEC;
    bcs = cs.W;
  }
  float mean[2][VEC], inv[2][VEC], k1[2][VEC], k2[2][VEC], k3[2][VEC], a1[VEC], a2[2][VEC];
#pragma unroll
  for (int b = 0; b < 2; ++b) {
#pragma unroll
    for (int j = 0; j < VEC; ++j) {
      mean[b][j] = p.coef[b][2 * p.C + c0 + j];
      inv[b][j] = p.coef[b][3 * p.C + c0 + j];
      a1[j] = a2[b][j] = 0.f;
      if (APPLY) {
        k1[b][j] = bc[b][j];
        k2[b][j] = bc[b][bcs + j];
        k3[b][j] = bc[b][2 * bcs + j];
      }
    }
  }
  const T* mref = (const T*)p.maskref;
  for (long r = rfirst; r < p.M; r += (long)gridDim.x * rpi) {
    float d[VEC], va[VEC], vb[VEC];
    if (pre) {
      unpack16<T>(pd, d);
      unpack16<T>(pa, va);
      unpack16<T>(pb, vb);
      pre = false;
    } else {
      const u32x4 qd = ld16s(dout + r * p.C + c0), qa = ld16s(ya + r * p.C + c0), qb = ld16s(yb + r * p.C + c0);
      unpack16<T>(qd, d);
      unpack16<T>(qa, va);
      unpack16<T>(qb, vb);
    }
    if (!APPLY) {
      if (VEC == 8 && p.mask_bits) {
        const unsigned bits = p.mask_bits[r * (p.C / VEC) + c0 / VEC];
#pragma unroll
        for (int j = 0; j < VEC; ++j) d[j] = (bits >> j) & 1u ? d[j] : 0.f;
      } else {
        float m[VEC];
        unpack16<T>(ld16s(mref + r * p.C + c0), m);
#pragma unroll
        for (int j = 0; j < VEC; ++j) d[j] = m[j] > 0.f ? d[j] : 0.f;
      }
      st16((T*)p.dz + r * p.C + c0, pack16<T>(d));
#pragma unroll
      for (int j = 0; j < VEC; ++j) {
        const float xa = (va[j] - mean[0][j]) * inv[0][j];
        const float xb = (vb[j] - mean[1][j]) * inv[1][j];
        a1[j] += d[j];
        a2[0][j] += d[j] * xa;
        a2[1][j] += d[j] * xb;
      }
    } else {
      float oa[VEC], ob[VEC];
#pragma unroll
      for (int j = 0; j < VEC; ++j) {
        const float xa = (va[j] - mean[0][j]) * inv[0][j];
        oa[j] = k1[0][j] * (d[j] - k2[0][j] - xa * k3[0][j]);
      }
      st16((T*)p.dy[0] + r * p.C + c0, pack16<T>(oa));
#pragma unroll
      for (int j = 0; j < VEC; ++j) {
        const float xb = (vb[j] - mean[1][j]) * inv[1][j];
        ob[j] = k1[1][j] * (d[j] - k2[1][j] - xb * k3[1][j]);
      }
      st16((T*)p.dy[1] + r * p.C + c0, pack16<T>(ob));
    }
  }
  if (!APPLY) {
#pragma unroll
    for (int b = 0; b < 2; ++b) {
      if (b) __syncthreads();
#pragma unroll
      for (int j = 0; j < VEC; ++j) {
        shm[threadIdx.x][j] = a1[j];
        shm[threadIdx.x][VEC + j] = a2[b][j];
      }
      __syncthreads();
      for (int o = threadIdx.x; o < 2 * p.C; o += BWD_THREADS) {
        int which = o / p.C, c = o % p.C;
        int ck = c / VEC, j = c % VEC;
        float s = 0.f;
        for (int k = 0; k < rpi; ++k) s += shm[k * cpr + ck][which * VEC + j];
        p.partial[b][(size_t)blockIdx.x * 2 * p.C + o] = s;
      }
    }
  }
}

__global__ __launch_bounds__(1024) void bn_bwd_finalize_kernel(const float* __restrict__ partial, int rows, int C,
                                                               double count, const float* __restrict__ gamma,
                                                               const float* __restrict__ coef, float* dgamma,
                                                               float* dbeta, float* __restrict__ bcoef, int centered) {
  __shared__ double sh[2][16][64];
  const int c = blockIdx.x * 64 + (threadIdx.x & 63);
  const int slice = threadIdx.x >> 6;
  double s1 = 0.0, s2 = 0.0;
// ... 563 lines not shown
  float* const outs[4] = {dg, a1o, a2o, a3o};
#pragma unroll
  for (int q = 0; q < 4; ++q) {
#pragma unroll
    for (int j = 0; j < VEC; ++j) sh[threadIdx.x][j] = q == 0 ? ag[j] : q == 1 ? a1[j] : q == 2 ? a2[j] : a3[j];
    __syncthreads();
    for (int c = threadIdx.x; c < C; c += EW_THREADS) {
      const int ck = c / VEC, j = c % VEC;
      float s_ = 0.f;
      for (int k = 0; k < nsl; ++k) s_ += sh[k * cpr + ck][j];
      outs[q][(size_t)n * C + c] = s_;
    }
    __syncthreads();
  }
}

constexpr int SE_ROWS = 16;
__global__ __launch_bounds__(256) void se_bn_rows_kernel(const float* __restrict__ a1, const float* __restrict__ a2,
                                                         const float* __restrict__ a3, const float* __restrict__ gate,
                                                         const float* __restrict__ addc, int N, int R, int C,
                                                         float* __restrict__ rows) {
  __shared__ float sh[2][4][64];
  const int c = blockIdx.x * 64 + (threadIdx.x & 63), sl = threadIdx.x >> 6, j = blockIdx.y;
  float s1 = 0.f, s2 = 0.f;
  if (c < C)
    for (int n = j + SE_ROWS * sl; n < N; n += SE_ROWS * 4) {
      const size_t o = (size_t)n * C + c;
      const float g = gate ? gate[o] : 1.f, ad = addc ? addc[o] : 0.f;
      s1 += g * a1[o] + ad * (float)R;
      s2 += g * a2[o] + ad * a3[o];
    }
  sh[0][sl][threadIdx.x & 63] = s1;
  sh[1][sl][threadIdx.x & 63] = s2;
  __syncthreads();
  if (sl == 0 && c < C) {
    float* row = rows + (size_t)j * 2 * C;
    row[c] = (sh[0][0][threadIdx.x] + sh[0][1][threadIdx.x]) + (sh[0][2][threadIdx.x] + sh[0][3][threadIdx.x]);
    row[C + c] = (sh[1][0][threadIdx.x] + sh[1][1][threadIdx.x]) + (sh[1][2][threadIdx.x] + sh[1][3][threadIdx.x]);
  }
}

template <typename T>
__global__ void bcast_rows_kernel(const float* __restrict__ v, T* __restrict__ out, long total, int R, int C,
                                  float scale) {
  for (long i = (long)blockIdx.x * blockDim.x + threadIdx.x; i < total; i += (long)gridDim.x * blockDim.x) {
    int c = (int)(i % C);
    long n = i / ((long)R * C);
    Elem<T>::st(out + i, v[n * C + c] * scale);
  }
}

template <typename T>
__global__ __launch_bounds__(1024) void bcast_rows_vec_kernel(const float* __restrict__ v, T* __restrict__ out, long M,
                                                              RowDiv rdiv, int C, float scale) {
  constexpr int VEC = Elem<T>::VEC;
  const int cpr = C / VEC, rpi = 1024 / cpr;
  const int c0 = (threadIdx.x % cpr) * VEC, r0 = threadIdx.x / cpr;
  for (long r = (long)blockIdx.x * rpi + r0; r < M; r += (long)gridDim.x * rpi) {
    const float* src = v + row_div(r, rdiv) * C + c0;
    float f[VEC];
#pragma unroll
    for (int j = 0; j < VEC; ++j) f[j] = src[j] * scale;
    st16(out + r * C + c0, pack16<T>(f));
  }
}

template <typename T>
__global__ void pack_weight_kernel(const float* __restrict__ w, T* __restrict__ fwd, T* __restrict__ dgr, int Cout,
                                   int Cin, int RS) {
  long total = (long)Cout * Cin * RS;
  for (long i = (long)blockIdx.x * blockDim.x + threadIdx.x; i < total; i += (long)gridDim.x * blockDim.x) {
    int tap = (int)(i % RS);
    long r = i / RS;
    int ci = (int)(r % Cin), co = (int)(r / Cin);
    float v = w[i];
    if (fwd) Elem<T>::st(fwd + ((size_t)co * RS + tap) * Cin + ci, v);
    if (dgr) Elem<T>::st(dgr + ((size_t)ci * RS + tap) * Cout + co, v);
  }
}

struct PackBatch {
  const float* w[ECG_PACK_MAX];
  void* fwd[ECG_PACK_MAX];
  void* dgr[ECG_PACK_MAX];
  int cout[ECG_PACK_MAX], cin[ECG_PACK_MAX], rs[ECG_PACK_MAX];
  int blk0[ECG_PACK_MAX + 1];
  int n;
};
constexpr int PACK_T = 32, PACK_RS_MAX = 9;
template <typename T>
__global__ __launch_bounds__(256) void pack_weight_batch_kernel(PackBatch b) {
  __shared__ float tile[PACK_T][PACK_T * PACK_RS_MAX + 1];
  int t = 0;
  while (t + 1 < b.n && (int)blockIdx.x >= b.blk0[t + 1]) ++t;
  const int Cout = b.cout[t], Cin = b.cin[t], RS = b.rs[t];
  const float* __restrict__ w = b.w[t];
  T* __restrict__ fwd = (T*)b.fwd[t];
  T* __restrict__ dgr = (T*)b.dgr[t];
  const int ci_tiles = (Cin + PACK_T - 1) / PACK_T;
  const int lb = blockIdx.x - b.blk0[t];
  const int co0 = (lb / ci_tiles) * PACK_T, ci0 = (lb % ci_tiles) * PACK_T;
  const int nci = min(PACK_T, Cin - ci0), nco = min(PACK_T, Cout - co0);
  const int run = nci * RS;
  for (int i = threadIdx.x; i < nco * run; i += 256) {
    const int co = i / run, k = i - co * run;
    tile[co][k] = w[((size_t)(co0 + co) * Cin + ci0) * RS + k];
  }
  __syncthreads();
  if (fwd) {
    for (int i = threadIdx.x; i < nco * RS * PACK_T; i += 256) {
      const int ci = i % PACK_T, ct = i / PACK_T, tap = ct % RS, co = ct / RS;
      if (ci < nci) Elem<T>::st(fwd + ((size_t)(co0 + co) * RS + tap) * Cin + ci0 + ci, tile[co][ci * RS + tap]);
    }
  }
  if (dgr) {
// ... 224 lines not shown
  p.mask_bits = mask_bits;
  const bool dz_early = dy && dz_out && (mask_bits || (maskref && maskref != y)) && dz_out != dout;
  if (dz_early) p.dz_out = dz_out;
  DISPATCH_T(dtype, (bn_bwd_launch<bf16_t, false>(p, grid, stream)), (bn_bwd_launch<float, false>(p, grid, stream)), "bn_bwd");
  ECG_CHECK_LAUNCH("bn_bwd_reduce");
  const bool fold = dy && !dbias && ecg_bn_fold_ok(C, grid);
  if (!fold) {
    const float* pr = partial;
    int rows = grid;
    hipLaunchKernelGGL(bn_bwd_finalize_kernel, dim3(ceil_div(C, 64)), dim3(1024), 0, stream, pr, rows, C, (double)M,
                       gamma, coef, dgamma, dbeta, bcoef, 0);
    ECG_CHECK_LAUNCH("bn_bwd_finalize");
  }
  if (!dy) return 0;
  p.bcoef = bcoef; p.dy = dy; p.dz_out = dz_out;
  if (fold) {
    p.fin.partial = partial; p.fin.rows = grid; p.fin.count = (double)M; p.fin.gamma = gamma; p.fin.dgamma = dgamma;
    p.fin.dbeta = dbeta; p.fin.centered = 0;
  }
  if (dz_early) { p.dout = dz_out; p.maskref = nullptr; p.mask_bits = nullptr; p.dz_out = nullptr; }
  p.partial = dbias ? partial : nullptr;
  const dim3 agrid = bn_bwd_apply_grid(dtype, p, grid);
  DISPATCH_T(dtype, (bn_bwd_launch<bf16_t, true>(p, agrid, stream)), (bn_bwd_launch<float, true>(p, agrid, stream)), "bn_bwd");
  ECG_CHECK_LAUNCH("bn_bwd_apply");
  if (dbias) {
    hipLaunchKernelGGL(rows_sum_kernel, dim3(ceil_div(C, 64)), dim3(1024), 0, stream, partial, grid, C, dbias, 0);
    ECG_CHECK_LAUNCH("rows_sum");
  }
  return 0;
}

static int g_bn_dual = 1;
void ecg_bn_dual_set(int on) { g_bn_dual = on != 0; }
bool ecg_bn_dual_on() { return g_bn_dual != 0; }

template <typename T, bool APPLY>
static void bn_bwd_dual_launch(const BnBwdDualParams& p, dim3 grid, hipStream_t stream) {
  constexpr size_t lds = APPLY ? 0 : (size_t)BWD_THREADS * (2 * Elem<T>::VEC + 1) * sizeof(float);
  static bool attr_set = false;
  if (lds > 64 * 1024 && !attr_set) {
    (void)hipFuncSetAttribute((const void*)bn_bwd_dual_kernel<T, APPLY>, hipFuncAttributeMaxDynamicSharedMemorySize, (int)lds);
    attr_set = true;
  }
  hipLaunchKernelGGL((bn_bwd_dual_kernel<T, APPLY>), grid, dim3(BWD_THREADS), lds, stream, p);
}

int ecg_bn_bwd_dual(int dtype, const void* dout, const void* maskref, const unsigned char* mask_bits, const float* gate,
                    const float* addc, const void* y_a, const float* coef_a, const float* gamma_a, float* dgamma_a,
                    float* dbeta_a, void* dy_a, const void* y_b, const float* coef_b, const float* gamma_b, float* dgamma_b,
                    float* dbeta_b, void* dy_b, void* dz, float* dbias, long M, int C, float* scratch_a, float* scratch_b,
                    hipStream_t stream) {
  if (!chunk_ok(C, dtype)) ECG_FAIL(ECGMM_ERR_SHAPE, "bn_bwd_dual: C=%d unsupported", C);
  if (gate || addc || dbias) ECG_FAIL(ECGMM_ERR_SHAPE, "bn_bwd_dual: gate / addc / dbias are not supported");
  if (dtype != ECGMM_BF16) mask_bits = nullptr;
  if (!dout || !y_a || !y_b || !coef_a || !coef_b || !dy_a || !dy_b || !dz || !scratch_a || !scratch_b || M < 1)
    ECG_FAIL(ECGMM_ERR_SHAPE, "bn_bwd_dual: null operand");
  if ((!mask_bits && !maskref) || maskref == y_a || maskref == y_b)
    ECG_FAIL(ECGMM_ERR_SHAPE, "bn_bwd_dual: needs the ReLU mask as bits (bf16) or as a tensor of its own");
  const int grid = bn_bwd_rows(dtype, M, C);
  const float* const gamma[2] = {gamma_a, gamma_b};
  float* const dgamma[2] = {dgamma_a, dgamma_b};
  float* const dbeta[2] = {dbeta_a, dbeta_b};
  float* bcoef[2];
  BnBwdDualParams p;
  memset(&p, 0, sizeof(p));
  p.dout = dout; p.maskref = mask_bits ? nullptr : maskref; p.mask_bits = mask_bits; p.dz = dz; p.M = M; p.C = C;
  p.y[0] = y_a; p.y[1] = y_b; p.coef[0] = coef_a; p.coef[1] = coef_b;
  for (int b = 0; b < 2; ++b) {
    p.partial[b] = b ? scratch_b : scratch_a;
    bcoef[b] = p.partial[b] + (size_t)(grid + ECG_TAIL_ROWS) * 2 * C;
  }
  DISPATCH_T(dtype, (bn_bwd_dual_launch<bf16_t, false>(p, grid, stream)), (bn_bwd_dual_launch<float, false>(p, grid, stream)),
             "bn_bwd_dual");
  ECG_CHECK_LAUNCH("bn_bwd_dual_reduce");
  const bool fold = ecg_bn_fold_ok(C, grid);
  dim3 agrid(grid);
  for (int b = 0; b < 2; ++b) {
    if (fold) {
      p.fin[b].partial = p.partial[b]; p.fin[b].rows = grid; p.fin[b].count = (double)M; p.fin[b].gamma = gamma[b];
      p.fin[b].dgamma = dgamma[b]; p.fin[b].dbeta = dbeta[b]; p.fin[b].centered = 0;
    } else {
      hipLaunchKernelGGL(bn_bwd_finalize_kernel, dim3(ceil_div(C, 64)), dim3(1024), 0, stream, (const float*)p.partial[b], grid, C,
                         (double)M, gamma[b], p.coef[b], dgamma[b], dbeta[b], bcoef[b], 0);
      ECG_CHECK_LAUNCH("bn_bwd_finalize");
    }
    p.bcoef[b] = bcoef[b];
  }
  if (fold) agrid = bn_fold_grid(dtype, M, C, bn_fold_slices(C), BWD_THREADS, 8);
  p.dout = dz; p.maskref = nullptr; p.mask_bits = nullptr; p.dz = nullptr;
  p.dy[0] = dy_a; p.dy[1] = dy_b;
  DISPATCH_T(dtype, (bn_bwd_dual_launch<bf16_t, true>(p, agrid, stream)), (bn_bwd_dual_launch<float, true>(p, agrid, stream)),
             "bn_bwd_dual");
  ECG_CHECK_LAUNCH("bn_bwd_dual_apply");
  return 0;
}

int ecg_bn_bwd_tail(int dtype, const void* dout, const void* maskref, const void* y, const float* coef,
                    const float* gamma, float* dgamma, float* dbeta, void* dy, const float* partial, int rows, long M,
                    int C, float* scratch, hipStream_t stream, const float* gate, const float* addc,
                    int rows_per_sample, float* dbias) {
  if (!chunk_ok(C, dtype)) ECG_FAIL(ECGMM_ERR_SHAPE, "bn_bwd: C=%d unsupported", C);
  if (rows < 1 || rows > 512) ECG_FAIL(ECGMM_ERR_SHAPE, "bn_bwd_tail: %d partial rows (1..512)", rows);
  const int grid = bn_bwd_rows(dtype, M, C);
  float* bcoef = scratch + (size_t)(grid + ECG_TAIL_ROWS) * 2 * C;
  const bool fold = ecg_bn_fold_ok(C, rows);
  if (!fold) {
    hipLaunchKernelGGL(bn_bwd_finalize_kernel, dim3(ceil_div(C, 64)), dim3(1024), 0, stream, partial, rows, C, (double)M,
                       gamma, coef, dgamma, dbeta, bcoef, 1);
    ECG_CHECK_LAUNCH("bn_bwd_finalize");
  }
  BnBwdParams p;
  memset(&p, 0, sizeof(p));
  p.dout = dout; p.maskref = maskref; p.y = y; p.coef = coef; p.M = M; p.C = C;
  p.gate = gate; p.addc = addc; p.rows_per_sample = rows_per_sample > 0 ? rows_per_sample : 1;
  p.rdiv = make_row_div(p.rows_per_sample);
  p.bcoef = bcoef; p.dy = dy;
  if (fold) {
    p.fin.partial = partial; p.fin.rows = rows; p.fin.count = (double)M; p.fin.gamma = gamma; p.fin.dgamma = dgamma;
    p.fin.dbeta = dbeta; p.fin.centered = 1;
  }
  p.partial = dbias ? scratch : nullptr;
  const dim3 agrid = bn_bwd_apply_grid(dtype, p, grid);
  DISPATCH_T(dtype, (bn_bwd_launch<bf16_t, true>(p, agrid, stream)), (bn_bwd_launch<float, true>(p, agrid, stream)), "bn_bwd");
  ECG_CHECK_LAUNCH("bn_bwd_apply");
  if (dbias) {
    hipLaunchKernelGGL(rows_sum_kernel, dim3(ceil_div(C, 64)), dim3(1024), 0, stream, (const float*)scratch, grid, C, dbias, 0);
    ECG_CHECK_LAUNCH("rows_sum");
  }
  return 0;
}

template <typename T>
static void pool_bwd_launch(const void* dp, const void* pooled, const unsigned char* idx, const void* y, const float* coef,
                            const float* gamma, float* dgamma, float* dbeta, void* dy, float* dbias, int N, int H, int W,
                            int C, int OH, int OW, float* scratch, int rows, hipStream_t stream) {
  constexpr int VEC = Elem<T>::VEC;
  constexpr size_t lds2 = (size_t)BWD_THREADS * (2 * VEC + 1) * sizeof(float), ldsp = (size_t)POOL_THREADS * (VEC + 1) * sizeof(float);
  static bool attr_set = false;
  if (!attr_set) {
    (void)hipFuncSetAttribute((const void*)pool_bwd_reduce_kernel<T>, hipFuncAttributeMaxDynamicSharedMemorySize, (int)lds2);
    attr_set = true;
  }
// ... 62 lines not shown
  return 0;
}

int ecg_rows_sum(const float* partial, int rows, int C, float* out, int accumulate, hipStream_t stream) {
  hipLaunchKernelGGL(rows_sum_kernel, dim3(ceil_div(C, 64)), dim3(1024), 0, stream, partial, rows, C, out, accumulate);
  ECG_CHECK_LAUNCH("rows_sum");
  return 0;
}

int ecg_bnrelu_maxpool(int dtype, const void* y, const float* coef, void* out, unsigned char* idx, int N, int H, int W,
                       int C, hipStream_t stream) {
  if (!chunk_ok(C, dtype)) ECG_FAIL(ECGMM_ERR_SHAPE, "maxpool: C=%d unsupported", C);
  int OH = (H + 2 - 3) / 2 + 1, OW = (W + 2 - 3) / 2 + 1;
  int vec = dtype == ECGMM_BF16 ? 8 : 4;
  int grid = ew_grid((long)N * OH * ((OW + 1) / 2) * (C / vec), EW_THREADS);
  DISPATCH_T(dtype,
             hipLaunchKernelGGL(bnrelu_maxpool_kernel<bf16_t>, dim3(grid), dim3(EW_THREADS), 0, stream,
                                (const bf16_t*)y, coef, (bf16_t*)out, idx, N, H, W, C, OH, OW),
             hipLaunchKernelGGL(bnrelu_maxpool_kernel<float>, dim3(grid), dim3(EW_THREADS), 0, stream, (const float*)y,
                                coef, (float*)out, idx, N, H, W, C, OH, OW),
             "maxpool");
  ECG_CHECK_LAUNCH("bnrelu_maxpool");
  return 0;
}

int ecg_maxpool_relu_bwd(int dtype, const void* dp, const void* pooled, const unsigned char* idx, void* dz, int N,
                         int H, int W, int C, hipStream_t stream) {
  if (!chunk_ok(C, dtype)) ECG_FAIL(ECGMM_ERR_SHAPE, "maxpool bwd: C=%d unsupported", C);
  int OH = (H + 2 - 3) / 2 + 1, OW = (W + 2 - 3) / 2 + 1;
  int vec = dtype == ECGMM_BF16 ? 8 : 4;
  int grid = ew_grid((long)N * ((H + 1) / 2) * ((W + 1) / 2) * (C / vec), EW_THREADS);
  DISPATCH_T(dtype,
             hipLaunchKernelGGL(maxpool_relu_bwd_kernel<bf16_t>, dim3(grid), dim3(EW_THREADS), 0, stream,
                                (const bf16_t*)dp, (const bf16_t*)pooled, idx, (bf16_t*)dz, N, H, W, C, OH, OW),
             hipLaunchKernelGGL(maxpool_relu_bwd_kernel<float>, dim3(grid), dim3(EW_THREADS), 0, stream,
                                (const float*)dp, (const float*)pooled, idx, (float*)dz, N, H, W, C, OH, OW),
             "maxpool bwd");
  ECG_CHECK_LAUNCH("maxpool_relu_bwd");
  return 0;
}

int ecg_avgpool(int dtype, const void* x, float* out, int N, int R, int C, const float* coef, hipStream_t stream) {
  if (!chunk_ok(C, dtype)) ECG_FAIL(ECGMM_ERR_SHAPE, "avgpool: C=%d unsupported", C);
  DISPATCH_T(dtype,
             hipLaunchKernelGGL((sample_reduce_kernel<bf16_t, false>), dim3(N), dim3(EW_THREADS), 0, stream,
                                (const bf16_t*)x, (const bf16_t*)nullptr, (const bf16_t*)nullptr, coef, out, R, C),
             hipLaunchKernelGGL((sample_reduce_kernel<float, false>), dim3(N), dim3(EW_THREADS), 0, stream,
                                (const float*)x, (const float*)nullptr, (const float*)nullptr, coef, out, R, C),
             "avgpool");
  ECG_CHECK_LAUNCH("avgpool");
  return 0;
}

int ecg_bcast_rows(int dtype, const float* v, void* out, int N, int R, int C, float scale, hipStream_t stream) {
  long total = (long)N * R * C;
  const int vecw = dtype == ECGMM_BF16 ? 8 : 4;
  if (C % vecw == 0 && C / vecw <= 1024 && 1024 % (C / vecw) == 0 && ((uintptr_t)out & 15) == 0) {
    const long M = (long)N * R;
    int g = ew_grid(M, (1024 / (C / vecw)) * 4);
    if (g > 256) g = 256;
    DISPATCH_T(dtype,
               hipLaunchKernelGGL(bcast_rows_vec_kernel<bf16_t>, dim3(g), dim3(1024), 0, stream, v, (bf16_t*)out, M, make_row_div(R), C, scale),
               hipLaunchKernelGGL(bcast_rows_vec_kernel<float>, dim3(g), dim3(1024), 0, stream, v, (float*)out, M, make_row_div(R), C, scale),
               "bcast_rows");
    ECG_CHECK_LAUNCH("bcast_rows_vec");
    return 0;
  }
  int grid = ew_grid(total, 256);
  DISPATCH_T(dtype,
             hipLaunchKernelGGL(bcast_rows_kernel<bf16_t>, dim3(grid), dim3(256), 0, stream, v, (bf16_t*)out, total, R,
                                C, scale),
             hipLaunchKernelGGL(bcast_rows_kernel<float>, dim3(grid), dim3(256), 0, stream, v, (float*)out, total, R, C,
                                scale),
             "bcast_rows");
  ECG_CHECK_LAUNCH("bcast_rows");
  return 0;
}

int ecg_se_gate_grad(int dtype, const void* dout, const void* maskref, const void* y, const float* coef, float* dg,
                     int N, int R, int C, hipStream_t stream) {
  if (!chunk_ok(C, dtype)) ECG_FAIL(ECGMM_ERR_SHAPE, "se_gate_grad: C=%d unsupported", C);
  DISPATCH_T(dtype,
             hipLaunchKernelGGL((sample_reduce_kernel<bf16_t, true>), dim3(N), dim3(EW_THREADS), 0, stream,
                                (const bf16_t*)dout, (const bf16_t*)maskref, (const bf16_t*)y, coef, dg, R, C),
             hipLaunchKernelGGL((sample_reduce_kernel<float, true>), dim3(N), dim3(EW_THREADS), 0, stream,
                                (const float*)dout, (const float*)maskref, (const float*)y, coef, dg, R, C),
             "se_gate_grad");
  ECG_CHECK_LAUNCH("se_gate_grad");
  return 0;
}

int ecg_se_gate_bn(int dtype, const void* dout, const void* maskref, const void* y, const float* coef, void* dz,
                   float* dg, float* a1, float* a2, float* a3, int N, int R, int C, hipStream_t stream) {
  if (!chunk_ok(C, dtype)) ECG_FAIL(ECGMM_ERR_SHAPE, "se_gate_bn: C=%d unsupported", C);
  DISPATCH_T(dtype,
             hipLaunchKernelGGL(se_gate_bn_kernel<bf16_t>, dim3(N), dim3(EW_THREADS), 0, stream, (const bf16_t*)dout,
                                (const bf16_t*)maskref, (const bf16_t*)y, coef, (bf16_t*)dz, dg, a1, a2, a3, R, C),
             hipLaunchKernelGGL(se_gate_bn_kernel<float>, dim3(N), dim3(EW_THREADS), 0, stream, (const float*)dout,
                                (const float*)maskref, (const float*)y, coef, (float*)dz, dg, a1, a2, a3, R, C),
             "se_gate_bn");
  ECG_CHECK_LAUNCH("se_gate_bn");
  return 0;
}
int ecg_se_bn_rows(const float* a1, const float* a2, const float* a3, const float* gate, const float* addc, int N, int R,
                   int C, float* rows, hipStream_t stream) {
  hipLaunchKernelGGL(se_bn_rows_kernel, dim3(ceil_div(C, 64), SE_ROWS), dim3(256), 0, stream, a1, a2, a3, gate, addc, N, R,
                     C, rows);
  ECG_CHECK_LAUNCH("se_bn_rows");
  return 0;
}
int ecg_se_bn_nrows() { return SE_ROWS; }

int ecg_pack_weight(int dtype, const float* w_oihw, void* fwd, void* dgrad, int Cout, int Cin, int RS,
                    hipStream_t stream) {
  long total = (long)Cout * Cin * RS;
  int grid = ew_grid(total, 256);
// ... 68 lines not shown
```

ecg-multimodal-model_amd/csrc/ops.h:

```cpp
#pragma once
#include "common.h"
#include "switches.h"

int ecg_iir_lanes(const double* a, int order, int E);

int ecg_conv_stats_rows(long M);
struct ConvEpi {
  const void* red_y;
  const void* red_mask;
  const float* red_coef;
  float* red_rows;
  int wg_rows;
  const void* src2;
  const void* wpk2;
  int src2_done;
  int stats_rows;
  int red_done;
  int red_rows_n;
};
int ecg_conv_igemm(int dtype, int mode, const ConvGeom& g, const void* src, const void* wpk, void* dst,
                   const float* bias, const void* addend, float* stats, int act, hipStream_t stream,
                   ConvEpi* epi = nullptr);
bool ecg_conv_halo_ok(int dtype, int mode, const ConvGeom& g);
int ecg_conv_halo_rows(int mode, const ConvGeom& g);
int ecg_conv_halo(int mode, const ConvGeom& g, const void* src, const void* wpk, void* dst, const float* bias,
                  const void* addend, float* stats, int act, ConvEpi* epi, hipStream_t stream);
size_t ecg_conv_wgrad_workspace(int dtype, const ConvGeom& g);
void ecg_conv_wgrad_narrow(bool narrow, int slots = 256);
int ecg_conv_wgrad(int dtype, const ConvGeom& g, const void* x, const void* dy, float* grad_oihw, int accumulate,
                   void* workspace, size_t workspace_bytes, hipStream_t stream);
size_t ecg_stem_packed_elems(int Cin, int R);
int ecg_stem_stats_rows(int N, int Cin, int H, int W, int R);
int ecg_stem_pack(int dtype, const float* w, void* out, int Cin, int R, hipStream_t stream);
int ecg_stem_fwd(int dtype, const float* x, const void* wpk, const float* bias, void* y, float* stats, int N, int Cin,
                 int H, int W, int R, hipStream_t stream);
size_t ecg_stem_wgrad_workspace(int N, int Cin, int H, int W, int R);
int ecg_stem_wgrad(int dtype, const float* x, const void* dy, float* grad, int accumulate, void* workspace,
                   size_t workspace_bytes, int N, int Cin, int H, int W, int R, hipStream_t stream);
int ecg_stem_stats_only_rows(int N, int Cin, int H, int W, int R);
int ecg_stem_wg_stats_rows(int N, int Cin, int H, int W, int R);
int ecg_stem_fwd_wgrows(int dtype, const float* x, const void* wpk, const float* bias, void* y, float* stats, int N, int Cin,
                        int H, int W, int R, hipStream_t stream);
int ecg_stem_stats_only(int dtype, const float* x, const void* wpk, const float* bias, float* stats, int N, int Cin, int H,
                        int W, int R, hipStream_t stream);
int ecg_stem_wgrad_reduce(const float* slab, float* grad, int rows, int NG, int accumulate, hipStream_t stream);
int ecg_stem_dgrad(int dtype, const void* dy, const float* w, float* dx, int N, int Cin, int H, int W, int R,
                   hipStream_t stream);
bool ecg_stem_fused_ok(int dtype, int Cin, int R);
int ecg_stem_pool_fwd(const float* x, const void* wpk, const float* coef, void* pooled, unsigned char* idx, int N, int Cin,
                      int H, int W, hipStream_t stream);
size_t ecg_stem_pool_bwd_workspace(int N, int Cin, int H, int W);
int ecg_stem_pool_bwd(const float* x, const void* wpk, const float* coef, const float* gamma, const void* dp, const void* pooled,
                      const unsigned char* idx, float* dgamma, float* dbeta, float* dw, void* ws, size_t ws_bytes, int N,
                      int Cin, int H, int W, hipStream_t stream);
int ecg_pool_bn_bwd_reduce(int dtype, const void* dp, const void* pooled, const float* coef, const float* gamma, float* dgamma,
                           float* dbeta, int N, int H, int W, int C, float* scratch, const float** bcoef_out,
                           hipStream_t stream);
int ecg_bn_rows(int dtype, long M, int C);
int ecg_bn_finalize(const float* partial, int rows, int C, double count, const float* gamma, const float* beta,
                    float* rm, float* rv, long long* nbt, float momentum, float eps, float* coef, hipStream_t stream);
int ecg_bn_eval_coef(int C, const float* gamma, const float* beta, const float* rm, const float* rv, float eps,
                     float* coef, hipStream_t stream);
int ecg_col_stats(int dtype, const void* x, long M, int C, float* partial, int* rows_out, hipStream_t stream);
struct EcgBnFold {
  const float* partial; int rows; double count;
  const float* gamma; const float* beta;
  float* rm; float* rv; long long* nbt;
  float momentum, eps;
};
bool ecg_bn_fold_ok(int C, int rows);
int ecg_bn_act_fold(int dtype, const void* y, float* coef, const EcgBnFold& f, const void* res, const float* rcoef,
                    const float* gate, int rows_per_sample, int relu, void* out, long M, int C, hipStream_t stream,
                    unsigned char* relu_bits = nullptr);
int ecg_bn_act(int dtype, const void* y, const float* coef, const void* res, const float* rcoef, const float* gate,
               int rows_per_sample, int relu, void* out, long M, int C, hipStream_t stream, unsigned char* relu_bits = nullptr);
size_t ecg_bn_bwd_scratch(int dtype, long M, int C);
int ecg_bn_bwd(int dtype, const void* dout, const void* maskref, const float* gate, const float* addc,
               int rows_per_sample, const void* y, const float* coef, const float* gamma, float* dgamma, float* dbeta,
               void* dy, void* dz_out, float* dbias, long M, int C, float* scratch, hipStream_t stream,
               const unsigned char* mask_bits = nullptr);
int ecg_bn_bwd_dual(int dtype, const void* dout, const void* maskref, const unsigned char* mask_bits, const float* gate,
                    const float* addc, const void* y_a, const float* coef_a, const float* gamma_a, float* dgamma_a,
                    float* dbeta_a, void* dy_a, const void* y_b, const float* coef_b, const float* gamma_b, float* dgamma_b,
                    float* dbeta_b, void* dy_b, void* dz, float* dbias, long M, int C, float* scratch_a, float* scratch_b,
                    hipStream_t stream);
void ecg_bn_dual_set(int on);
bool ecg_bn_dual_on();
int ecg_bn_bwd_tail(int dtype, const void* dout, const void* maskref, const void* y, const float* coef,
                    const float* gamma, float* dgamma, float* dbeta, void* dy, const float* partial, int rows, long M,
                    int C, float* scratch, hipStream_t stream, const float* gate = nullptr, const float* addc = nullptr,
                    int rows_per_sample = 1, float* dbias = nullptr);
int ecg_bn_eval_bwd(int dtype, const void* dout, const void* maskref, const float* gate, const float* addc,
                    int rows_per_sample, const void* y, const float* coef, float* dgamma, float* dbeta, void* dy,
                    void* dz_out, float* dbias, long M, int C, float* scratch, hipStream_t stream);
int ecg_bn_small_eval_bwd(const float* x, const float* dy, const float* gamma, const float* save, float* dx, float* dgamma,
                          float* dbeta, int N, int C, int accumulate, hipStream_t stream);
int ecg_gradcam(int dtype, const void* act, const float* dpooled, float* small, float* out, int N, int Hs, int Ws, int C,
                int H, int W, hipStream_t stream);
size_t ecg_crnn_gradcam_workspace(int B, int Tp, int Fp, int C);
int ecg_crnn_gradcam(const float* seq, const float* dseq, const int* steps, const int* frames, void* ws, size_t ws_bytes,
                     float* cam, int B, int Tp, int C, int Fp, int F, int T, hipStream_t stream);
int ecg_se_gate_bn(int dtype, const void* dout, const void* maskref, const void* y, const float* coef, void* dz,
                   float* dg, float* a1, float* a2, float* a3, int N, int R, int C, hipStream_t stream);
int ecg_se_bn_nrows();
int ecg_se_bn_rows(const float* a1, const float* a2, const float* a3, const float* gate, const float* addc, int N, int R,
                   int C, float* rows, hipStream_t stream);
int ecg_rows_sum(const float* partial, int rows, int C, float* out, int accumulate, hipStream_t stream);
int ecg_bnrelu_maxpool(int dtype, const void* y, const float* coef, void* out, unsigned char* idx, int N, int H, int W,
                       int C, hipStream_t stream);
int ecg_maxpool_relu_bwd(int dtype, const void* dp, const void* pooled, const unsigned char* idx, void* dz, int N,
                         int H, int W, int C, hipStream_t stream);
int ecg_pool_bn_bwd(int dtype, const void* dp, const void* pooled, const unsigned char* idx, const void* y,
                    const float* coef, const float* gamma, float* dgamma, float* dbeta, void* dy, float* dbias, int N,
                    int H, int W, int C, float* scratch, hipStream_t stream);
bool ecg_stem_fuse_on();
int ecg_avgpool(int dtype, const void* x, float* out, int N, int R, int C, const float* coef, hipStream_t stream);
int ecg_bcast_rows(int dtype, const float* v, void* out, int N, int R, int C, float scale, hipStream_t stream);
int ecg_se_gate_grad(int dtype, const void* dout, const void* maskref, const void* y, const float* coef, float* dg,
                     int N, int R, int C, hipStream_t stream);
constexpr int ECG_PACK_MAX = 24;
struct EcgPackItem {
  const float* w;
  void* fwd;
  void* dgrad;
  int Cout, Cin, RS;
};
int ecg_pack_weight_batch(int dtype, const EcgPackItem* items, int n, hipStream_t stream);
constexpr int ECG_FOLD_MAX = 32;
enum { ECG_FOLD_CONV = 0,
       ECG_FOLD_STEM = 1,
       ECG_FOLD_COPY = 2,
       ECG_FOLD_OIHW = 3 };
struct EcgFoldItem {
  int kind;
  const float* w;
  const float* conv_bias;
  const float *gamma, *beta, *rm, *rv;
  void* wout;
  float* bout;
  float* scale_out;
  int Cout, Cin, RS;
};
int ecg_fold_batch(int dtype, const EcgFoldItem* items, int n, float eps, hipStream_t stream);
int ecg_relu_maxpool(int dtype, const void* y, void* out, int N, int H, int W, int C, hipStream_t stream);
int ecg_gate_res_relu(int dtype, const void* y, const float* gate, const void* res, void* out, long M, int C,
                      int rows_per_sample, hipStream_t stream);
int ecg_resnet1d_side_enable(int on);
int ecg_pack_weight(int dtype, const float* w_oihw, void* fwd, void* dgrad, int Cout, int Cin, int RS,
                    hipStream_t stream);
int ecg_nchw_to_nhwc(int dtype, const float* src, void* dst, int N, int C, long HW, hipStream_t stream);
int ecg_nhwc_to_nchw(int dtype, const void* src, float* dst, int N, int C, long HW, hipStream_t stream);
int ecg_cast(int dtype, const float* src, void* dst, long n, hipStream_t stream);
int ecg_uncast(int dtype, const void* src, float* dst, long n, hipStream_t stream);
int ecg_linear_fwd_valu(const float* x, const float* w, const float* bias, float* y, int B, int In, int Out, int act,
                        hipStream_t s);
int ecg_linear_dgrad_valu(const float* dy, const float* w, float* dx, int B, int In, int Out, int accumulate,
                          hipStream_t s);
int ecg_linear_wgrad_valu(const float* dy, const float* x, float* dw, float* db, int B, int In, int Out,
                          int accumulate, hipStream_t s);
int ecg_act_bwd(const float* dy, const float* y, float* dz, long n, int act, hipStream_t s);
int ecg_axpby(float a, const float* x, float b, float* y, long n, hipStream_t s);
int ecg_layernorm_fwd(const float* const* seg, const int* dims, int nseg, const float* fusion_w, const float* gamma,
                      const float* beta, float* out, float* stat, float* soft_w, int B, float eps, hipStream_t s);
size_t ecg_layernorm_bwd_scratch(int B, int D);
int ecg_layernorm_bwd(const float* const* seg, const int* dims, int nseg, const float* fusion_w, const float* gamma,
                      const float* stat, const float* dout, float* const* dseg, int dseg_accumulate, float* dgamma,
                      float* dbeta, float* dfusion_w, int B, float* scratch, hipStream_t s);
bool ecg_head_fused_ok(const int* dim, int B, int hidden, int num_classes);
int ecg_head_partial_floats(const int* dim, int num_classes);
int ecg_head_bwd_blocks(int B);
// ... 119 lines not shown
```

ecg-multimodal-model_amd/csrc/plan_resnet18.hip:

```cpp
#include "plan_common.h"
#include "side_stream.h"

namespace {
bool stem_recompute(int dtype) {
  return sw::STEM_RECOMPUTE.get() && ecg_stem_fused_ok(dtype, 3, 7);
}
bool relu_bits_on() { return sw::RELU_BITS.get() != 0; }

int build(const ecgmm_resnet18_desc* d, Net18& r) {
  ECG_TRY(net18_static(d, r, "resnet18"));
  return net18_shape(r, "resnet18");
}

struct FwdWs {
  void* wstem;
  void* y0; float* coef0; void* p0; unsigned char* idx0;
  BlockWs b[8];
  float* pooled;
  float* stats;
  float* stats_d;
  size_t bytes;
};

void layout_fwd(const Net18& r, void* base, FwdWs& w, WsTable* views = nullptr) {
// ... 237 lines not shown
      ECG_TRY(bn_coef(r.bn, w.stats_d, rows, k.cout, M, params, k.p_dbn, buffers, k.b_dbn, b.coefd, g_side.s));
      down_done = side_mark();
    }
    ECG_TRY(ecg_conv_igemm(dt, 0, g1, cur, b.w1f, b.y1, nullptr, nullptr, stats_rows ? w.stats : nullptr, 0, s, &e1));
    ECG_TRY(bn_then_act(r, w.stats, e1.stats_rows, k.cout, M, params, k.p_bn1, buffers, k.b_bn1, b.coef1, b.y1, nullptr,
                        nullptr, b.a1, s));
    ECG_TRY(ecg_conv_igemm(dt, 0, g2, b.a1, b.w2f, b.y2, nullptr, nullptr, stats_rows ? w.stats : nullptr, 0, s, &e2));
    if (k.down) {
      if (down_side) {
        main_wait(s, down_done);
      } else {
        ConvGeom gd = k.down_geom(N);
        ECG_TRY(ecg_conv_igemm(dt, 0, gd, cur, b.wdf, b.yd, nullptr, nullptr, stats_rows ? w.stats_d : nullptr, 0, s));
        ECG_TRY(bn_coef(r.bn, w.stats_d, rows, k.cout, M, params, k.p_dbn, buffers, k.b_dbn, b.coefd, s));
      }
      ECG_TRY(bn_then_act(r, w.stats, e2.stats_rows, k.cout, M, params, k.p_bn2, buffers, k.b_bn2, b.coef2, b.y2, b.yd,
                          b.coefd, b.out, s, r.d.training && relu_bits_on() ? b.bits : nullptr));
    } else {
      ECG_TRY(bn_then_act(r, w.stats, e2.stats_rows, k.cout, M, params, k.p_bn2, buffers, k.b_bn2, b.coef2, b.y2, cur,
                          nullptr, b.out, s, r.d.training && relu_bits_on() ? b.bits : nullptr));
    }
    cur = b.out;
    ecg_tl_mark(102 + i, s);
  }
  const Blk18& last = r.blk[7];
  ECG_TRY(ecg_avgpool(dt, cur, w.pooled, N, last.hout * last.wout, 512, nullptr, s));
  ECG_TRY(ecg_linear_fwd(w.pooled, P(params, r.p_fc), P(params, r.p_fc + 1), feat_out, N, 512, r.d.out_dim, 0, nullptr,
                         s));
  ecg_tl_mark(110, s);
  return 0;
}

static int r18_backward(const ecgmm_resnet18_desc* d, const float* image, const float* dfeat, const void* const* params,
                        void* const* grads, void* ws_fwd, void* ws_bwd, size_t ws_bwd_bytes, int stage_begin, int stage_end,
                        float* dimage, hipStream_t s) {
  Net18 r;
  ECG_TRY(build(d, r));
  const bool train = r.d.training != 0;
  if (stem_recompute(r.d.dtype) && (dimage || !train))
    ECG_FAIL(ECGMM_ERR_SHAPE, "resnet18 bwd: %s needs the stored stem conv output; switch ecgmm_stem_recompute(0) "
             "(ECGMM_STEM_RECOMPUTE) off", dimage ? "the input gradient" : "an eval-mode backward");
  FwdWs w;
  layout_fwd(r, ws_fwd, w);
  BwdWs q;
  layout_bwd(r, ws_bwd, q);
  ECG_NEED(ws_fwd && ws_bwd, ws_bwd_bytes, q.bytes, "resnet18 bwd: workspace");
  const int dt = r.d.dtype, N = r.d.N;
  ECG_TRY(side_init());
  const bool side = g_side.enabled;
  ecg_conv_wgrad_narrow(side, N >= 192 ? 192 : 256);
  struct NarrowOff { ~NarrowOff() { ecg_conv_wgrad_narrow(false); } } narrow_off;
  hipStream_t ws = side ? g_side.s : s;

  if (stage_begin == 0) ecg_tl_mark(200, s);
  for (int st = stage_begin; st < stage_end; ++st) {
    if (st > 0) ecg_tl_mark(200 + st, s);
    if (st == 0) {
      g_side.doneA = g_side.doneB = g_side.doneC = nullptr;
      for (int a = 0; a < 3; ++a) g_side.done2[a][0] = g_side.done2[a][1] = nullptr;
      const Blk18& last = r.blk[7];
      ECG_TRY(fc_bwd(r, w, q, dfeat, params, grads, s));
      const int R = last.hout * last.wout;
      ECG_TRY(ecg_bcast_rows(dt, q.dpooled, q.X[0], N, R, 512, 1.f / (float)R, s));
    } else if (st <= 8) {
      const int i = 8 - st;
      const Blk18& k = r.blk[i];
      BlockWs& b = w.b[i];
      const void* in = i == 0 ? w.p0 : w.b[i - 1].out;
      const void* dcur = q.X[(st - 1) & 1];
      void* din = q.X[st & 1];
      const long M = (long)N * k.hout * k.wout;
      ConvGeom g1 = k.conv1_geom(N);
      ConvGeom g2 = k.conv2_geom(N);
      const int pp = st & 1;
      void *dyb = q.dy[pp], *dy1b = q.dy1[pp], *dydb = q.dyd[pp];
      bool fused2 = false;
      int fused2_rows = 0;
      const bool fuse_here = train && sw::BN_FUSE.get() && M >= sw::BN_FUSE_MIN_M.get();
      if (fuse_here && i + 1 < 8 && !r.blk[i + 1].down) {
        const Blk18& kn = r.blk[i + 1];
        const ConvGeom gn = kn.conv1_geom(N);
        fused2 = ecg_conv_halo_ok(dt, 1, gn);
        fused2_rows = fused2 ? ecg_conv_halo_rows(1, gn) : 0;
      }
      main_wait(s, g_side.done2[0][pp]);
      const void* dzp = q.dz;
      const bool dual = k.down && train && !fused2 && ecg_bn_dual_on() &&
                        ecg_bn_bwd_scratch(dt, M, k.cout) <= RED_ROWS_FLOATS * sizeof(float);
      if (dual) {
        main_wait(s, g_side.done2[2][pp]);
        ECG_TRY(ecg_bn_bwd_dual(dt, dcur, b.out, relu_bits_on() ? b.bits : nullptr, nullptr, nullptr, b.y2, b.coef2,
                                P(params, k.p_bn2), G(grads, k.p_bn2), G(grads, k.p_bn2 + 1), dyb, b.yd, b.coefd,
                                P(params, k.p_dbn), G(grads, k.p_dbn), G(grads, k.p_dbn + 1), dydb, q.dz, nullptr, M, k.cout,
                                q.bn_scratch, q.red2, s));
      } else if (fused2) {
        dzp = dcur;
        ECG_TRY(ecg_bn_bwd_tail(dt, dcur, nullptr, b.y2, b.coef2, P(params, k.p_bn2), G(grads, k.p_bn2),
                                G(grads, k.p_bn2 + 1), dyb, q.red2, fused2_rows, M, k.cout, q.bn_scratch, s));
      } else {
        ECG_TRY(bn_bwd_mode(r.bn, dcur, b.out, nullptr, nullptr, 1, b.y2, b.coef2, P(params, k.p_bn2), G(grads, k.p_bn2),
                            G(grads, k.p_bn2 + 1), dyb, q.dz, nullptr, M, k.cout, q.bn_scratch, s,
                            train && relu_bits_on() ? b.bits : nullptr));
      }
      if (G(grads, k.p_conv2)) {
        if (side) side_fork(s);
        ECG_TRY(ecg_conv_wgrad(dt, g2, b.a1, dyb, G(grads, k.p_conv2), 0, q.wg_ws, q.wg_bytes, ws));
        if (side) g_side.done2[0][pp] = side_mark();
      }
      ConvEpi ea = {};
      if (fuse_here) { ea.wg_rows = 1; ea.red_y = b.y1; ea.red_mask = b.y1; ea.red_coef = b.coef1; ea.red_rows = q.red1; }
      ECG_TRY(ecg_conv_igemm(dt, 1, g2, dyb, b.w2d, q.da, nullptr, nullptr, nullptr, 0, s, &ea));
      main_wait(s, g_side.done2[1][pp]);
      if (ea.red_done) {
        ECG_TRY(ecg_bn_bwd_tail(dt, q.da, b.y1, b.y1, b.coef1, P(params, k.p_bn1), G(grads, k.p_bn1),
                                G(grads, k.p_bn1 + 1), dy1b, q.red1, ea.red_rows_n, M, k.cout, q.bn_scratch, s));
      } else {
        ECG_TRY(bn_bwd_mode(r.bn, q.da, b.y1, nullptr, nullptr, 1, b.y1, b.coef1, P(params, k.p_bn1), G(grads, k.p_bn1),
                            G(grads, k.p_bn1 + 1), dy1b, nullptr, nullptr, M, k.cout, q.bn_scratch, s));
      }
      if (G(grads, k.p_conv1)) {
        if (side) side_fork(s);
        ECG_TRY(ecg_conv_wgrad(dt, g1, in, dy1b, G(grads, k.p_conv1), 0, q.wg_ws, q.wg_bytes, ws));
        if (side) g_side.done2[1][pp] = side_mark();
      }
      if (k.down) {
        ConvGeom gd = k.down_geom(N);
        if (!dual) {
          main_wait(s, g_side.done2[2][pp]);
          ECG_TRY(bn_bwd_mode(r.bn, dzp, nullptr, nullptr, nullptr, 1, b.yd, b.coefd, P(params, k.p_dbn), G(grads, k.p_dbn),
                              G(grads, k.p_dbn + 1), dydb, nullptr, nullptr, M, k.cout, q.bn_scratch, s));
        }
        if (G(grads, k.p_dconv)) {
          if (side) side_fork(s);
          ECG_TRY(ecg_conv_wgrad(dt, gd, in, dydb, G(grads, k.p_dconv), 0, q.wg_ws, q.wg_bytes, ws));
          if (side) g_side.done2[2][pp] = side_mark();
        }
        ConvEpi ed = {};
        ed.src2 = dydb; ed.wpk2 = b.wdd;
        if (!sw::DOWN_FOLD.get()) ed.src2 = nullptr;
        if (ed.src2) {
          ECG_TRY(ecg_conv_igemm(dt, 1, g1, dy1b, b.w1d, din, nullptr, nullptr, nullptr, 0, s, &ed));
        }
        if (!ed.src2_done) {
          ECG_TRY(ecg_conv_igemm(dt, 1, gd, dydb, b.wdd, q.dtmp, nullptr, nullptr, nullptr, 0, s));
          ECG_TRY(ecg_conv_igemm(dt, 1, g1, dy1b, b.w1d, din, nullptr, q.dtmp, nullptr, 0, s));
        }
      } else {
        ConvEpi eb = {};
        if (fuse_here && i > 0 && ecg_conv_halo_ok(dt, 1, g1)) {
          const BlockWs& pb = w.b[i - 1];
          eb.wg_rows = 1; eb.red_y = pb.y2; eb.red_mask = pb.out; eb.red_coef = pb.coef2; eb.red_rows = q.red2;
        }
        ECG_TRY(ecg_conv_igemm(dt, 1, g1, dy1b, b.w1d, din, nullptr, dzp, nullptr, 0, s, &eb));
      }
    } else if (st == 9) {
      const void* dp0 = q.X[8 & 1];
      if (stem_recompute(dt)) {
        ECG_TRY(ecg_stem_pool_bwd(image, w.wstem, w.coef0, P(params, 1), dp0, w.p0, w.idx0, G(grads, 1), G(grads, 2),
                                  G(grads, 0), q.stem_ws, q.stem_bytes, N, 3, r.d.H, r.d.W, s));
        continue;
      }
      if (train && ecg_stem_fuse_on()) {
        ECG_TRY(ecg_pool_bn_bwd(dt, dp0, w.p0, w.idx0, w.y0, w.coef0, P(params, 1), G(grads, 1), G(grads, 2), q.big1,
                                nullptr, N, r.H1, r.W1, 64, q.bn_scratch, s));
      } else {
        ECG_TRY(ecg_maxpool_relu_bwd(dt, dp0, w.p0, w.idx0, q.big0, N, r.H1, r.W1, 64, s));
        ECG_TRY(bn_bwd_mode(r.bn, q.big0, nullptr, nullptr, nullptr, 1, w.y0, w.coef0, P(params, 1), G(grads, 1), G(grads, 2),
                            q.big1, nullptr, nullptr, (long)N * r.H1 * r.W1, 64, q.bn_scratch, s));
      }
      if (G(grads, 0)) {
        ECG_TRY(ecg_stem_wgrad(dt, image, q.big1, G(grads, 0), 0, q.stem_ws, q.stem_bytes, N, 3, r.d.H, r.d.W, 7, s));
      }
      if (dimage) ECG_TRY(ecg_stem_dgrad(dt, q.big1, P(params, 0), dimage, N, 3, r.d.H, r.d.W, 7, s));
    } else {
      ECG_FAIL(ECGMM_ERR_SHAPE, "resnet18 bwd: stage %d out of range", st);
    }
  }
  if (stage_end == 10) ecg_tl_mark(210, s);
  if (side && !g_side.defer_join) {
    hipEvent_t e = side_next_ev();
    (void)hipEventRecord(e, g_side.s);
    (void)hipStreamWaitEvent(s, e, 0);
  }
  if (stage_end == 10) ecg_tl_mark(211, s);
  return 0;
}

extern "C" int ecgmm_resnet18_backward(const ecgmm_resnet18_desc* d, const float* image, const float* dfeat,
                                       const void* const* params, void* const* grads, void* ws_fwd, void* ws_bwd,
                                       size_t ws_bwd_bytes, int stage_begin, int stage_end, void* stream_) {
  return r18_backward(d, image, dfeat, params, grads, ws_fwd, ws_bwd, ws_bwd_bytes, stage_begin, stage_end, nullptr,
                      (hipStream_t)stream_);
}

extern "C" int ecgmm_resnet18_backward_dx(const ecgmm_resnet18_desc* d, const float* image, const float* dfeat,
                                          const void* const* params, void* const* grads, void* ws_fwd, void* ws_bwd,
                                          size_t ws_bwd_bytes, int stage_begin, int stage_end, float* dimage,
                                          void* stream_) {
  return r18_backward(d, image, dfeat, params, grads, ws_fwd, ws_bwd, ws_bwd_bytes, stage_begin, stage_end, dimage,
                      (hipStream_t)stream_);
}

extern "C" int ecgmm_resnet18_gradcam(const ecgmm_resnet18_desc* d, const float* dfeat, const void* const* params,
                                      void* ws_fwd, void* ws_bwd, size_t ws_bwd_bytes, float* cam, void* stream_) {
  hipStream_t s = (hipStream_t)stream_;
  Net18 r;
  ECG_TRY(build(d, r));
// ... 13 lines not shown
```

ecg-multimodal-model_amd/csrc/switches.h:

```cpp
#pragma once
#include <limits.h>

#include "common.h"

struct Switch {
  enum Kind {
    ON,
    OFF,
    LEVEL,
    INT
  };
  const char* env;
  Kind kind;
  long def;
  long hi, neg;
  bool runtime;
  const char* doc;
  long v = LONG_MIN;

  long clamp(long x) const {
    if (kind == LEVEL) return x < 0 ? 0 : x > hi ? hi : x;
    if (kind == INT) return x < 0 ? neg : x;
    return x != 0;
  }
  long from_env() const {
    if (kind == ON) return env_on(env);
    if (kind == OFF) return env_off(env);
    if (kind == LEVEL) return env_level(env, (int)hi, (int)def);
    return clamp(env_int(env, def));
  }
  long get() {
    if (v == LONG_MIN) v = from_env();
    return v;
  }
  void set(long x) { v = clamp(x); }
};

namespace sw {
constexpr long NEVER = 1L << 40;
inline Switch CONV_HALO      {"ECGMM_CONV_HALO",       Switch::LEVEL, 1,     2, 0,     true,  "halo-resident conv kernel: 0 = never, 1 = where it is faster, 2 = wherever applicable"};
inline Switch HALO_CUS       {"ECGMM_HALO_CUS",        Switch::INT,   0,     0, 0,     true,  "cap on the CUs (persistent workgroups) of a halo-kernel launch; 0 or negative = all"};
inline Switch HALO_W4        {"ECGMM_HALO_W4",         Switch::OFF,   0,     0, 0,     true,  "64 -> 64 channel 3x3 tiles on 4-wave workgroups, two per CU"};
inline Switch HALO_STAGGER   {"ECGMM_HALO_STAGGER",    Switch::ON,    1,     0, 0,     true,  "waves 4-7 run a step's first MFMA block behind its barrier (0: lock step); bit-identical"};
inline Switch HALO_STREAM    {"ECGMM_HALO_STREAM",     Switch::ON,    1,     0, 0,     true,  "stream form of the 64 -> 64 channel 3x3 tiles (0: one tile at a time); bit-identical"};
inline Switch HALO_PP        {"ECGMM_HALO_PP",         Switch::ON,    1,     0, 0,     true,  "ping-pong K loop on the 128-channel 3x3 tiles (0: lock step); bit-identical"};
inline Switch HALO_NCS1      {"ECGMM_HALO_NCS1",       Switch::ON,    1,     0, 0,     false, "64-channel 3x3 layers prefetch the next tile's halo during the K loop"};
inline Switch WGRAD_RING     {"ECGMM_WGRAD_RING",      Switch::LEVEL, 1,     2, 0,     true,  "ring weight-gradient kernel: 0 = never, 1 = where it is faster, 2 = wherever applicable"};
inline Switch WGRAD_PP       {"ECGMM_WGRAD_PP",        Switch::OFF,   0,     0, 0,     true,  "ping-pong between the two wave groups of the ring weight gradient; bit-identical"};
inline Switch WGRAD_GROUPS   {"ECGMM_WGRAD_GROUPS",    Switch::OFF,   0,     0, 0,     false, "1 = 256-thread weight-gradient workgroups instead of two 4-wave groups sharing a slab tile"};
inline Switch WGRAD_WGS      {"ECGMM_WGRAD_WGS",       Switch::INT,   0,     0, 0,     false, "four-wave slots of a weight-gradient launch; 0 or negative = 512 alone, the plan's choice on the side stream"};
inline Switch BN_FOLD        {"ECGMM_BN_FOLD",         Switch::ON,    1,     0, 0,     true,  "BatchNorm finalize folded into its consumer pass (0: separate launches)"};
inline Switch BN_FOLD_SLICE  {"ECGMM_BN_FOLD_SLICE",   Switch::ON,    1,     0, 0,     true,  "folded passes at C >= 256 as (pixel chunk, 128-channel slice) workgroups; bit-identical"};
inline Switch BN_FUSE        {"ECGMM_BN_FUSE",         Switch::ON,    1,     0, 0,     false, "0 = BatchNorm-backward reductions always as their own pass, whatever the threshold"};
inline Switch BN_FUSE_MIN_M  {"ECGMM_BN_FUSE_MIN_M",   Switch::INT,   NEVER, 0, NEVER, true,  "pixel count from which a BatchNorm-backward reduction is fused into the producing dgrad; negative = never"};
inline Switch RELU_BITS      {"ECGMM_RELU_BITS",       Switch::ON,    1,     0, 0,     false, "bn2's backward reads the ReLU mask as bits the forward wrote (forward and backward must agree)"};
inline Switch STEM_FUSE      {"ECGMM_STEM_FUSE",       Switch::ON,    1,     0, 0,     false, "stem backward as one pool + BatchNorm pass (0: max-pool backward + full BatchNorm backward)"};
inline Switch STEM_RECOMPUTE {"ECGMM_STEM_RECOMPUTE",  Switch::OFF,   0,     0, 0,     true,  "image stem by recompute, without its full-resolution conv output (changes the workspace layouts)"};
inline Switch DOWN_FOLD      {"ECGMM_DOWN_FOLD",       Switch::ON,    1,     0, 0,     false, "downsample branch's input gradient folded into the stride-2 dgrad (0: own launch + addend)"};
inline Switch DOWN_SIDE      {"ECGMM_DOWN_SIDE",       Switch::ON,    1,     0, 0,     false, "downsample branch of the training forward on the side stream (0: the caller's stream)"};
inline Switch SIDE_WGRAD     {"ECGMM_SIDE_WGRAD",      Switch::ON,    1,     0, 0,     false, "initial state of each plan's weight-gradient side stream; per plan at run time: ecgmm_side_wgrad()"};
inline Switch INFER_DOWN_SIDE{"ECGMM_INFER_DOWN_SIDE", Switch::OFF,   0,     0, 0,     true,  "downsample convolution of the inference plans on a side stream beside conv1"};
inline Switch SE_MERGE       {"ECGMM_SE_MERGE",        Switch::ON,    1,     0, 0,     false, "ResNet1D_SE backward: SE-gate gradient and bn2's reduction in one pass (0: two passes)"};
inline Switch SE_MLP_FUSED   {"ECGMM_SE_MLP_FUSED",    Switch::ON,    1,     0, 0,     false, "the SE MLP as fused kernels (0: per-op launches)"};
inline Switch HEAD_FUSED     {"ECGMM_HEAD_FUSED",      Switch::ON,    1,     0, 0,     false, "fusion head on the row kernels of head_fused.hip (0: ~45 per-op launches)"};
inline Switch DENSE16        {"ECGMM_DENSE16",         Switch::ON,    1,     0, 0,     false, "batch-sized Linear layers on dense16_kernel (0: the implicit-GEMM route)"};

inline Switch* const ALL[] = {
    &CONV_HALO,  &HALO_CUS,      &HALO_W4,       &HALO_STAGGER, &HALO_STREAM,   &HALO_PP,   &HALO_NCS1,  &WGRAD_RING,      &WGRAD_PP,
    &WGRAD_GROUPS, &WGRAD_WGS,   &BN_FOLD,       &BN_FOLD_SLICE, &BN_FUSE,      &BN_FUSE_MIN_M, &RELU_BITS, &STEM_FUSE,    &STEM_RECOMPUTE,
    &DOWN_FOLD,  &DOWN_SIDE,     &SIDE_WGRAD,    &INFER_DOWN_SIDE, &SE_MERGE,   &SE_MLP_FUSED, &HEAD_FUSED, &DENSE16};
constexpr int COUNT = (int)(sizeof(ALL) / sizeof(ALL[0]));

inline Switch* find(const char* env) {
  for (Switch* s : ALL)
    if (env && strcmp(s->env, env) == 0) return s;
  return nullptr;
}
}
```

ecg-multimodal-model_amd/hip/lib.py:

```python
import ctypes as C
import os

F32, BF16 = 0, 1
ACT_NONE, ACT_RELU, ACT_SIGMOID = 0, 1, 2
RESNET18_NPARAMS, RESNET18_NBUFFERS = 62, 60
RESNET1D_NPARAMS, RESNET1D_NBUFFERS = 52, 27

_PKG_DIR = os.path.dirname(os.path.dirname(os.path.abspath(__file__)))
LIB_PATH = os.environ.get("ECGMM_LIB") or os.path.join(_PKG_DIR, "libecgmm_hip.so")

vp, i32, i64, u64, f32, f64, sz = C.c_void_p, C.c_int, C.c_int64, C.c_uint64, C.c_float, C.c_double, C.c_size_t


class ConvDesc(C.Structure):
    _fields_ = [(n, i32) for n in ("N", "H", "W", "Cin", "Cout", "R", "S", "stride", "pad_h", "pad_w")]


class ResNet18Desc(C.Structure):
    _fields_ = [("N", i32), ("H", i32), ("W", i32), ("out_dim", i32), ("dtype", i32), ("training", i32),
                ("bn_momentum", f32), ("bn_eps", f32)]


class ResNet1DDesc(C.Structure):
    _fields_ = [("N", i32), ("cin", i32), ("L", i32), ("num_classes", i32), ("dtype", i32), ("training", i32),
# ... 69 lines not shown
    "ecgmm_nhwc_to_nchw": (i32, [i32, vp, vp, i32, i32, i64, vp]),
    "ecgmm_cast": (i32, [i32, vp, vp, i64, vp]),
    "ecgmm_uncast": (i32, [i32, vp, vp, i64, vp]),
    "ecgmm_pack_conv_weight": (i32, [i32, vp, vp, vp, i32, i32, i32, vp]),
    "ecgmm_conv_stats_rows": (i32, [i64]),
    "ecgmm_conv_fwd": (i32, [i32, P(ConvDesc), vp, vp, vp, vp, vp, i32, vp]),
    "ecgmm_conv_fwd_wgrows": (i32, [i32, P(ConvDesc), vp, vp, vp, vp, vp, vp, i32, vp]),
    "ecgmm_conv_bwd_data": (i32, [i32, P(ConvDesc), vp, vp, vp, vp, vp]),
    "ecgmm_conv_bwd_weight_workspace": (sz, [i32, P(ConvDesc)]),
    "ecgmm_conv_bwd_weight": (i32, [i32, P(ConvDesc), vp, vp, vp, i32, vp, sz, vp]),
    "ecgmm_stem_packed_elems": (sz, [i32, i32]),
    "ecgmm_stem_stats_rows": (i32, [i32, i32, i32, i32, i32]),
    "ecgmm_stem_pack": (i32, [i32, vp, vp, i32, i32, vp]),
    "ecgmm_stem_fwd": (i32, [i32, vp, vp, vp, vp, vp, i32, i32, i32, i32, i32, vp]),
    "ecgmm_stem_wg_stats_rows": (i32, [i32, i32, i32, i32, i32]),
    "ecgmm_stem_fwd_wgrows": (i32, [i32, vp, vp, vp, vp, vp, i32, i32, i32, i32, i32, vp]),
    "ecgmm_stem_stats_only_rows": (i32, [i32, i32, i32, i32, i32]),
    "ecgmm_stem_stats_only": (i32, [i32, vp, vp, vp, vp, i32, i32, i32, i32, i32, vp]),
    "ecgmm_stem_pool_fwd": (i32, [vp, vp, vp, vp, vp, i32, i32, i32, i32, vp]),
    "ecgmm_stem_pool_bwd_workspace": (sz, [i32, i32, i32, i32]),
    "ecgmm_stem_pool_bwd": (i32, [vp, vp, vp, vp, vp, vp, vp, vp, vp, vp, vp, sz, i32, i32, i32, i32, vp]),
    "ecgmm_stem_bwd_weight_workspace": (sz, [i32, i32, i32, i32, i32]),
    "ecgmm_stem_bwd_weight": (i32, [i32, vp, vp, vp, i32, vp, sz, i32, i32, i32, i32, i32, vp]),
    "ecgmm_stem_bwd_data": (i32, [i32, vp, vp, vp, i32, i32, i32, i32, i32, vp]),
    "ecgmm_col_stats_rows": (i32, [i32, i64, i32]),
    "ecgmm_col_stats": (i32, [i32, vp, i64, i32, vp, vp]),
    "ecgmm_bn_finalize": (i32, [vp, i32, i32, f64, vp, vp, vp, vp, vp, f32, f32, vp, vp]),
    "ecgmm_bn_eval_coef": (i32, [i32, vp, vp, vp, vp, f32, vp, vp]),
    "ecgmm_bn_act": (i32, [i32, vp, vp, vp, vp, vp, i32, i32, vp, i64, i32, vp]),
    "ecgmm_bn_act_from_rows": (i32, [i32, vp, vp, i32, f64, vp, vp, vp, vp, vp, f32, f32, vp, vp, vp, vp, i32, i32, vp, i64, i32, vp]),
    "ecgmm_bn_bwd_scratch": (sz, [i32, i64, i32]),
    "ecgmm_bn_bwd": (i32, [i32, vp, vp, vp, vp, i32, vp, vp, vp, vp, vp, vp, vp, vp, i64, i32, vp, vp]),
    "ecgmm_bn_eval_bwd": (i32, [i32, vp, vp, vp, vp, i32, vp, vp, vp, vp, vp, vp, vp, i64, i32, vp, vp]),
    "ecgmm_conv_bwd_data_with_downsample": (i32, [i32, P(ConvDesc), vp, vp, vp, vp, vp, vp, vp]),
    "ecgmm_conv_bwd_data_bnred": (i32, [i32, P(ConvDesc), vp, vp, vp, vp, vp, vp, vp, vp, P(i32), vp]),
    "ecgmm_conv_bwd_data_bnred_rows": (i32, [i32, P(ConvDesc)]),
    "ecgmm_bn_bwd_from_rows": (i32, [i32, vp, vp, vp, vp, vp, vp, vp, vp, vp, i32, i64, i32, vp, vp]),
    "ecgmm_bnrelu_maxpool": (i32, [i32, vp, vp, vp, vp, i32, i32, i32, i32, vp]),
    "ecgmm_maxpool_relu_bwd": (i32, [i32, vp, vp, vp, vp, i32, i32, i32, i32, vp]),
    "ecgmm_bn_fuse_min_pixels": (i32, [i64]),
    "ecgmm_bn_fold": (i32, [i32]),
    "ecgmm_bn_fold_slice": (i32, [i32]),
    "ecgmm_bn_act_from_rows_bits": (i32, [i32, vp, vp, i32, f64, vp, vp, vp, vp, vp, f32, f32, vp, vp, vp, vp, i32, i32, vp, vp, i64, i32, vp]),
    "ecgmm_bn_bwd_bits": (i32, [i32, vp, vp, vp, vp, i32, vp, vp, vp, vp, vp, vp, vp, vp, i64, i32, vp, vp]),
    "ecgmm_bn_bwd_dual": (i32, [i32] + [vp] * 19 + [i64, i32, vp, vp, vp]),
    "ecgmm_bn_dual": (i32, [i32]),
    "ecgmm_tl_enable": (i32, [i32]),
    "ecgmm_tl_mark": (i32, [i32, vp]),
    "ecgmm_tl_collect": (i32, [i32, vp, vp]),
    "ecgmm_stem_recompute": (i32, [i32]),
    "ecgmm_pool_bn_bwd": (i32, [i32, vp, vp, vp, vp, vp, vp, vp, vp, vp, vp, i32, i32, i32, i32, vp, vp]),
    "ecgmm_avgpool": (i32, [i32, vp, vp, i32, i32, i32, vp, vp]),
    "ecgmm_bcast_rows": (i32, [i32, vp, vp, i32, i32, i32, f32, vp]),
    "ecgmm_se_gate_grad": (i32, [i32, vp, vp, vp, vp, vp, i32, i32, i32, vp]),
    "ecgmm_se_gate_bn": (i32, [i32, vp, vp, vp, vp, vp, vp, vp, vp, vp, i32, i32, i32, vp]),
    "ecgmm_se_mlp_fwd": (i32, [vp, vp, vp, vp, vp, vp, vp, i32, i32, i32, vp]),
    "ecgmm_se_mlp_bwd": (i32, [vp, vp, vp, vp, vp, vp, vp, vp, vp, vp, vp, vp, vp, i32, i32, i32, f32, vp]),
    "ecgmm_linear_fwd": (i32, [vp, vp, vp, vp, i32, i32, i32, i32, vp]),
    "ecgmm_linear_bwd_scratch": (sz, [i32, i32, i32]),
    "ecgmm_linear_bwd": (i32, [vp, vp, vp, vp, vp, vp, i32, i32, i32, vp, sz, vp]),
    "ecgmm_act_bwd": (i32, [vp, vp, vp, i64, i32, vp]),
    "ecgmm_layernorm_fwd": (i32, [P(vp), P(i32), i32, vp, vp, vp, vp, vp, vp, i32, f32, vp]),
    "ecgmm_layernorm_bwd_scratch": (sz, [i32, i32]),
    "ecgmm_layernorm_bwd": (i32, [P(vp), P(i32), i32, vp, vp, vp, vp, P(vp), i32, vp, vp, vp, i32, vp, vp]),
    "ecgmm_varloss_fwd": (i32, [vp, vp, vp, i32, i32, i32, i32, vp, vp, vp]),
    "ecgmm_varloss_bwd": (i32, [vp, i32, i32, vp, vp, i32, vp, i32, vp]),
    "ecgmm_ce_fwd": (i32, [vp, vp, i32, i32, i32, f32, f32, vp, vp, vp]),
    "ecgmm_ce_bwd": (i32, [vp, vp, i32, i32, vp, vp, vp, vp]),
    "ecgmm_ce_plus_fwd": (i32, [vp, vp, i32, i32, vp, f32, vp, vp, vp]),
    "ecgmm_ce_plus_bwd": (i32, [vp, vp, i32, i32, vp, vp, vp, vp, f32, vp]),
    "ecgmm_dropout_fwd": (i32, [vp, vp, vp, i64, f32, u64, u64, vp]),
    "ecgmm_dropout_bwd": (i32, [vp, vp, vp, i64, f32, vp]),
    "ecgmm_adam": (i32, [vp, vp, vp, vp, i64, f32, f32, f32, f32, f32, i64, f32, vp]),
    "ecgmm_axpby": (i32, [f32, vp, f32, vp, i64, vp]),
    "ecgmm_signal_preprocess_workspace": (sz, [i32, i32, i32]),
    "ecgmm_signal_preprocess": (i32, [vp, vp, i32, i32, vp, vp, i32, P(f64), P(f64), P(f64), i32, vp, sz, vp]),
    "ecgmm_signal_preprocess_i16": (i32, [vp, i32, i32, i32, P(i32), i32, vp, vp, i32, vp, i32, i32, P(f64), P(f64), P(f64),
                                          i32, vp]),
    "ecgmm_weighted_sample": (i32, [vp, i64, i64, vp, vp, i64, u64, u64, vp]),
    "ecgmm_signal_filter_zscore": (i32, [vp, vp, i32, i32, P(f64), P(f64), P(f64), i32, i32, f64, vp]),
    "ecgmm_signal_filter_lanes": (i32, [P(f64), i32, i32]),
    "ecgmm_signal_resample_len": (i32, [i32, f64]),
    "ecgmm_signal_resample_workspace": (sz, [i32, i32, i32]),
    "ecgmm_signal_resample": (i32, [vp, i32, i32, vp, i32, f64, vp, i32, vp, vp, sz, vp]),
    "ecgmm_signal_gather_augment": (i32, [vp, i64, i32, vp, i32, vp, vp, i32, f32, f32, f32, f32, i32, i32, u64, u64, vp]),
    "ecgmm_glu_fwd": (i32, [vp, vp, i64, i32, vp]),
    "ecgmm_glu_bwd": (i32, [vp, vp, vp, i64, i32, vp]),
    "ecgmm_sparsemax_fwd": (i32, [vp, vp, i64, i32, vp]),
    "ecgmm_sparsemax_bwd": (i32, [vp, vp, vp, i64, i32, vp]),
    "ecgmm_ew": (i32, [i32, vp, vp, vp, i64, f32, vp]),
    "ecgmm_split_cols": (i32, [vp, vp, vp, i64, i32, i32, i32, vp]),
    "ecgmm_split_cols_bwd": (i32, [vp, vp, vp, vp, i64, i32, i32, i32, vp]),
    "ecgmm_bn_small_fwd": (i32, [vp, vp, vp, vp, vp, vp, vp, vp, i32, i32, i32, f32, f32, vp]),
    "ecgmm_bn_small_bwd": (i32, [vp, vp, vp, vp, vp, vp, vp, i32, i32, i32, vp]),
    "ecgmm_bn_small_eval_bwd": (i32, [vp, vp, vp, vp, vp, vp, vp, i32, i32, i32, vp]),
    "ecgmm_entropy_fwd": (i32, [vp, vp, i64, i32, f32, vp]),
    "ecgmm_entropy_bwd": (i32, [vp, vp, vp, i64, i32, f32, vp]),
    "ecgmm_image_resize_tables_bytes": (sz, [i32, i32, i32, i32]),
    "ecgmm_image_resize_tables": (i32, [i32, i32, i32, i32, vp, sz]),
    "ecgmm_image_transform": (i32, [vp, vp, i32, i32, i32, i32, i32, vp, sz, P(f32), P(f32), vp]),
    "ecgmm_resnet18_infer_prepared_bytes": (sz, [P(ResNet18Desc)]),
    "ecgmm_resnet18_infer_prepare": (i32, [P(ResNet18Desc), P(vp), P(vp), vp, sz, vp]),
    "ecgmm_resnet18_infer_workspace": (sz, [P(ResNet18Desc)]),
    "ecgmm_resnet18_infer": (i32, [P(ResNet18Desc), vp, vp, sz, vp, vp, sz, vp]),
    "ecgmm_resnet1d_infer_prepared_bytes": (sz, [P(ResNet1DDesc)]),
    "ecgmm_resnet1d_infer_prepare": (i32, [P(ResNet1DDesc), P(vp), P(vp), vp, sz, vp]),
# ... 59 lines not shown
    "ecgmm_mha_weights": (i32, [P(MHADesc), vp, vp, vp, vp, i32, vp]),
    "ecgmm_mha_rollout_step": (i32, [P(MHADesc), vp, vp, vp, vp, vp, f32, vp]),
    "ecgmm_embed1d_fwd": (i32, [vp, vp, vp, vp, vp, i32, i32, i32, i32, vp]),
    "ecgmm_embed1d_bwd_workspace": (sz, [i32, i32, i32, i32]),
    "ecgmm_embed1d_bwd": (i32, [vp, vp, vp, vp, vp, vp, vp, i32, i32, i32, i32, i32, vp, sz, vp]),
    "ecgmm_linear_res_ln": (i32, [vp, vp, vp, vp, vp, vp, vp, i64, i32, i32, f32, vp]),
    "ecgmm_ffn_res_ln": (i32, [vp, vp, vp, vp, vp, vp, vp, vp, i64, i32, i32, f32, vp]),
    "ecgmm_transformer_infer_prepared_bytes": (sz, [P(TransformerInferDesc)]),
    "ecgmm_transformer_infer_prepare": (i32, [P(TransformerInferDesc), P(vp), vp, sz, vp]),
    "ecgmm_transformer_infer_workspace": (sz, [P(TransformerInferDesc)]),
    "ecgmm_transformer_infer": (i32, [P(TransformerInferDesc), vp, vp, vp, sz, vp, vp, sz, vp]),
    "ecgmm_tabnet_infer_prepared_bytes": (sz, [P(TabNetInferDesc)]),
    "ecgmm_tabnet_infer_prepare": (i32, [P(TabNetInferDesc), P(vp), vp, sz, vp]),
    "ecgmm_tabnet_infer": (i32, [P(TabNetInferDesc), vp, i64, vp, sz, vp, vp, vp, vp, vp]),
}

LATER_SYMBOLS = ("ecgmm_resnet18_backward_dx", "ecgmm_resnet18_gradcam", "ecgmm_resnet1d_backward_dx",
                 "ecgmm_resnet1d_gradcam", "ecgmm_stem_bwd_data", "ecgmm_bn_eval_bwd", "ecgmm_bn_small_eval_bwd",
                 "ecgmm_resnet18_infer_prepared_bytes", "ecgmm_resnet18_infer_prepare", "ecgmm_resnet18_infer_workspace",
                 "ecgmm_resnet18_infer", "ecgmm_resnet1d_infer_prepared_bytes", "ecgmm_resnet1d_infer_prepare",
                 "ecgmm_resnet1d_infer_workspace", "ecgmm_resnet1d_infer", "ecgmm_infer_down_side", "ecgmm_conv_fwd_fused",
                 "ecgmm_fold_conv_bn", "ecgmm_relu_maxpool", "ecgmm_gate_res_relu",
                 "ecgmm_signal_filter_zscore", "ecgmm_signal_gather_augment",
                 "ecgmm_lstm_fwd_workspace", "ecgmm_lstm_bwd_workspace", "ecgmm_lstm_forward", "ecgmm_lstm_backward",
                 "ecgmm_conv5_in1_stats_rows", "ecgmm_conv5_in1_fwd", "ecgmm_conv5_in1_bwd_weight_workspace",
                 "ecgmm_conv5_in1_bwd_weight", "ecgmm_conv5_bwd_weight_workspace", "ecgmm_conv5_bwd_weight",
                 "ecgmm_bnrelu_maxpool2", "ecgmm_pool2_bn_bwd_workspace", "ecgmm_pool2_bn_bwd",
                 "ecgmm_crnn_front_fwd_workspace", "ecgmm_crnn_front_bwd_workspace", "ecgmm_crnn_front_forward",
                 "ecgmm_crnn_front_backward",
                 "ecgmm_switch_name", "ecgmm_switch_get", "ecgmm_switch_set",
                 "ecgmm_log_spectrogram_frames", "ecgmm_log_spectrogram",
                 "ecgmm_se_mlp_fwd", "ecgmm_se_mlp_bwd",
                 "ecgmm_signal_preprocess_i16", "ecgmm_weighted_sample",
                 "ecgmm_resnet18_ws_view", "ecgmm_resnet1d_ws_view",
                 "ecgmm_lime_perturb", "ecgmm_lime_ridge_workspace", "ecgmm_lime_ridge", "ecgmm_lime_prob",
                 "ecgmm_shap_mlp_workspace", "ecgmm_shap_gradient", "ecgmm_shap_deep",
                 "ecgmm_bn_bwd_dual", "ecgmm_bn_dual",
                 "ecgmm_mha_bwd_workspace", "ecgmm_mha_forward", "ecgmm_mha_backward", "ecgmm_mha_keep_mask",
                 "ecgmm_embed1d_fwd", "ecgmm_embed1d_bwd_workspace", "ecgmm_embed1d_bwd",
                 "ecgmm_se_gate_bn",
                 "ecgmm_lstm_forward_varlen", "ecgmm_lstm_backward_varlen", "ecgmm_seq_mean_varlen_fwd",
                 "ecgmm_seq_mean_varlen_bwd",
                 "ecgmm_signal_filter_lanes",
                 "ecgmm_mha_forward_varlen", "ecgmm_mha_backward_varlen",
                 "ecgmm_mha_weights", "ecgmm_mha_rollout_step",
                 "ecgmm_crnn_front_backward_dx", "ecgmm_conv5_in1_bwd_data", "ecgmm_conv5_in1_bwd_data_tile",
                 "ecgmm_crnn_gradcam_workspace", "ecgmm_crnn_gradcam",
                 "ecgmm_signal_resample_len", "ecgmm_signal_resample_workspace", "ecgmm_signal_resample",
                 "ecgmm_relu_maxpool2", "ecgmm_conv5_in1_relu_pool2", "ecgmm_fold_conv5_bn",
                 "ecgmm_crnn_front_infer_prepared_bytes", "ecgmm_crnn_front_infer_prepare",
                 "ecgmm_crnn_front_infer_workspace", "ecgmm_crnn_front_infer",
                 "ecgmm_linear_res_ln", "ecgmm_ffn_res_ln", "ecgmm_transformer_infer_prepared_bytes",
                 "ecgmm_transformer_infer_prepare", "ecgmm_transformer_infer_workspace", "ecgmm_transformer_infer",
                 "ecgmm_tabnet_infer_prepared_bytes", "ecgmm_tabnet_infer_prepare", "ecgmm_tabnet_infer")

_lib = None


def _missing(name):
    def fail(*_a):
        raise RuntimeError(f"{LIB_PATH} does not export {name}: rebuild the HIP library (there is no fallback)")
    return fail


def lib():
    global _lib
    if _lib is None:
        if not os.path.exists(LIB_PATH):
            raise RuntimeError(
                f"libecgmm_hip.so not found at {LIB_PATH}: the HIP extension is the only compute path "
                "(no CPU fallback). Build it with `python __graft_entry__.py` or "
                "`make -C ecg-multimodal-model_amd/csrc`.")
        import torch
        h = C.CDLL(LIB_PATH)
        for name, (res, args) in SIGNATURES.items():
            if name in LATER_SYMBOLS and os.environ.get("ECGMM_LIB") and not hasattr(h, name):
                setattr(h, name, _missing(name))
                continue
            fn = getattr(h, name)
            fn.restype, fn.argtypes = res, args
        if h.ecgmm_version() != 100:
            raise RuntimeError(f"libecgmm_hip.so version {h.ecgmm_version()} != 100 (stale build?)")
        _lib = h
    return _lib


def check(rc, what=""):
    if rc != 0:
        msg = lib().ecgmm_last_error().decode(errors="replace")
        raise RuntimeError(f"ecgmm {what} failed (code {rc}): {msg}")
```

include/ecgmm.h:

```cpp
#ifndef ECGMM_H
#define ECGMM_H
#include <stddef.h>
#include <stdint.h>

#ifdef __cplusplus
extern "C" {
#endif

#define ECGMM_VERSION 100

enum { ECGMM_F32 = 0, ECGMM_BF16 = 1 };
enum { ECGMM_ACT_NONE = 0, ECGMM_ACT_RELU = 1, ECGMM_ACT_SIGMOID = 2 };
enum {
  ECGMM_OK = 0,
  ECGMM_ERR_SHAPE = 1,
  ECGMM_ERR_DTYPE = 2,
  ECGMM_ERR_WORKSPACE = 3,
  ECGMM_ERR_LAUNCH = 4
};

int ecgmm_version(void);
const char* ecgmm_last_error(void);

const char* ecgmm_switch_name(int i);
// ... 146 lines not shown
                        const void* pooled, const uint8_t* idx, float* dgamma, float* dbeta, float* dw_oihw, void* ws,
                        size_t ws_bytes, int N, int Cin, int H, int W, void* stream);

#define ECGMM_BN_TAIL_ROWS 64
int ecgmm_col_stats_rows(int dtype, int64_t M, int C);
int ecgmm_col_stats(int dtype, const void* x, int64_t M, int C, float* partial, void* stream);
int ecgmm_bn_finalize(const float* partial, int rows, int C, double count, const float* gamma, const float* beta,
                      float* running_mean, float* running_var, int64_t* num_batches_tracked, float momentum, float eps,
                      float* coef, void* stream);
int ecgmm_bn_eval_coef(int C, const float* gamma, const float* beta, const float* running_mean,
                       const float* running_var, float eps, float* coef, void* stream);
int ecgmm_bn_act(int dtype, const void* y, const float* coef, const void* res, const float* rcoef, const float* gate,
                 int rows_per_sample, int relu, void* out, int64_t M, int C, void* stream);
int ecgmm_bn_act_from_rows(int dtype, const void* y, const float* partial, int rows, double count, const float* gamma,
                           const float* beta, float* running_mean, float* running_var, int64_t* num_batches_tracked,
                           float momentum, float eps, float* coef_out, const void* res, const float* rcoef,
                           const float* gate, int rows_per_sample, int relu, void* out, int64_t M, int C, void* stream);
size_t ecgmm_bn_bwd_scratch(int dtype, int64_t M, int C);
int ecgmm_bn_bwd(int dtype, const void* dout, const void* maskref, const float* gate, const float* addc,
                 int rows_per_sample, const void* y, const float* coef, const float* gamma, float* dgamma,
                 float* dbeta, void* dy, void* dz_out, float* dbias, int64_t M, int C, void* scratch, void* stream);
int ecgmm_bn_eval_bwd(int dtype, const void* dout, const void* maskref, const float* gate, const float* addc,
                      int rows_per_sample, const void* y, const float* coef, float* dgamma, float* dbeta, void* dy,
                      void* dz_out, float* dbias, int64_t M, int C, float* scratch, void* stream);

int ecgmm_conv_bwd_data_bnred(int dtype, const ecgmm_conv_desc* c, const void* dy, const void* w_dgrad,
                              const void* addend, void* dx, const void* bn_y, const void* bn_mask, const float* bn_coef,
                              float* rows, int* nrows, void* stream);
int ecgmm_conv_bwd_data_bnred_rows(int dtype, const ecgmm_conv_desc* c);
int ecgmm_conv_bwd_data_with_downsample(int dtype, const ecgmm_conv_desc* c, const void* dy, const void* w_dgrad,
                                        const void* dy_down, const void* w_down_dgrad, void* dx, void* tmp,
                                        void* stream);
int ecgmm_bn_bwd_from_rows(int dtype, const void* dout, const void* maskref, const void* y, const float* coef,
                           const float* gamma, float* dgamma, float* dbeta, void* dy, const float* rows, int nrows,
                           int64_t M, int C, void* scratch, void* stream);

int ecgmm_bn_fuse_min_pixels(int64_t m);
int ecgmm_bn_fold(int on);
int ecgmm_bn_fold_slice(int on);
int ecgmm_bn_act_from_rows_bits(int dtype, const void* y, const float* partial, int rows, double count, const float* gamma,
                                const float* beta, float* running_mean, float* running_var, int64_t* num_batches_tracked,
                                float momentum, float eps, float* coef_out, const void* res, const float* rcoef,
                                const float* gate, int rows_per_sample, int relu, void* out, uint8_t* relu_bits, int64_t M,
                                int C, void* stream);
int ecgmm_bn_bwd_bits(int dtype, const void* dout, const uint8_t* mask_bits, const float* gate, const float* addc,
                      int rows_per_sample, const void* y, const float* coef, const float* gamma, float* dgamma,
                      float* dbeta, void* dy, void* dz_out, float* dbias, int64_t M, int C, void* scratch, void* stream);
int ecgmm_bn_bwd_dual(int dtype, const void* dout, const void* maskref, const uint8_t* mask_bits, const float* gate,
                      const float* addc, const void* y_a, const float* coef_a, const float* gamma_a, float* dgamma_a,
                      float* dbeta_a, void* dy_a, const void* y_b, const float* coef_b, const float* gamma_b,
                      float* dgamma_b, float* dbeta_b, void* dy_b, void* dz, float* dbias, int64_t M, int C, void* scratch_a,
                      void* scratch_b, void* stream);
int ecgmm_bn_dual(int on);
int ecgmm_stem_recompute(int on);

int ecgmm_bnrelu_maxpool(int dtype, const void* y, const float* coef, void* out, uint8_t* idx, int N, int H, int W,
                         int C, void* stream);
int ecgmm_maxpool_relu_bwd(int dtype, const void* dp, const void* pooled, const uint8_t* idx, void* dz, int N, int H,
                           int W, int C, void* stream);
int ecgmm_pool_bn_bwd(int dtype, const void* dp, const void* pooled, const uint8_t* idx, const void* y, const float* coef,
                      const float* gamma, float* dgamma, float* dbeta, void* dy, float* dbias, int N, int H, int W, int C,
                      void* scratch, void* stream);
int ecgmm_avgpool(int dtype, const void* x, float* out, int N, int R, int C, const float* coef, void* stream);
int ecgmm_bcast_rows(int dtype, const float* v, void* out, int N, int R, int C, float scale, void* stream);
int ecgmm_se_gate_grad(int dtype, const void* dout, const void* maskref, const void* y, const float* coef, float* dg,
                       int N, int R, int C, void* stream);
int ecgmm_se_gate_bn(int dtype, const void* dout, const void* maskref, const void* y, const float* coef, void* dz, float* dg,
                     float* a1, float* a2, float* a3, int N, int R, int C, void* stream);
int ecgmm_se_mlp_fwd(const float* m, const float* w1, const float* b1, const float* w2, const float* b2, float* h, float* g,
                     int N, int C, int CR, void* stream);
int ecgmm_se_mlp_bwd(const float* dg, const float* g, const float* h, const float* m, const float* w1, const float* w2,
                     float* ds, float* dh, float* dm, float* dw1, float* db1, float* dw2, float* db2, int N, int C, int CR,
                     float scale, void* stream);

int ecgmm_linear_fwd(const float* x, const float* w, const float* bias, float* y, int B, int In, int Out, int act,
                     void* stream);
size_t ecgmm_linear_bwd_scratch(int B, int In, int Out);
int ecgmm_linear_bwd(const float* dz, const float* x, const float* w, float* dx, float* dw, float* db, int B, int In,
                     int Out, void* scratch, size_t scratch_bytes, void* stream);
int ecgmm_act_bwd(const float* dy, const float* y, float* dz, int64_t n, int act, void* stream);

int ecgmm_layernorm_fwd(const float* const* seg, const int* dims, int nseg, const float* fusion_w, const float* gamma,
                        const float* beta, float* out, float* stat, float* soft_w, int B, float eps, void* stream);
size_t ecgmm_layernorm_bwd_scratch(int B, int D);
int ecgmm_layernorm_bwd(const float* const* seg, const int* dims, int nseg, const float* fusion_w, const float* gamma,
                        const float* stat, const float* dout, float* const* dseg, int dseg_accumulate, float* dgamma,
                        float* dbeta, float* dfusion_w, int B, void* scratch, void* stream);

int ecgmm_varloss_fwd(const float* f0, const float* f1, const float* f2, int B, int D0, int D1, int D2, float* loss,
                      float* scratch, void* stream);
int ecgmm_varloss_bwd(const float* f, int B, int D, const float* gout, const float* scratch, int which, float* df,
                      int accumulate, void* stream);

int ecgmm_ce_fwd(const float* logits, const int64_t* labels, int B, int C, int focal, float alpha, float gamma,
                 float* loss, float* dcoef, void* stream);
int ecgmm_ce_bwd(const float* logits, const int64_t* labels, int B, int C, const float* dcoef, const float* gout,
                 float* dlogits, void* stream);
int ecgmm_ce_plus_fwd(const float* logits, const int64_t* labels, int B, int C, const float* extra, float extra_w,
                      float* loss, float* dcoef, void* stream);
int ecgmm_ce_plus_bwd(const float* logits, const int64_t* labels, int B, int C, const float* dcoef, const float* gout,
                      float* dlogits, float* dextra, float extra_w, void* stream);

int ecgmm_dropout_fwd(const float* x, float* y, uint8_t* mask, int64_t n, float p, uint64_t seed, uint64_t offset,
                      void* stream);
int ecgmm_dropout_bwd(const float* dy, const uint8_t* mask, float* dx, int64_t n, float p, void* stream);

// ... 211 lines not shown
```

Before: 40470 samples/s.

## Fold ReLU mask into conv input-gradient stores in ResNet18 backward

Adds a masked-store variant of the dgrad kernels (halo stream, halo ping-pong, stride-2 igemm) and of the avgpool broadcast. Each of these zeroes output gradients using the saved ReLU bit mask as it stores them. The ResNet18 backward plan then feeds the already-masked gradient straight into the BN backward. This skips the separate mask application and the dz write/read in the BN backward for the non-fused blocks. In exchange the kernels do extra bit-mask loads in the epilogue, and there are more template instantiations and dispatch conditions that must agree.

After: 40820 samples/s (median of 6 runs). No clear change (+0.9%).

```diff
diff --git a/ecg-multimodal-model_amd/csrc/api.hip b/ecg-multimodal-model_amd/csrc/api.hip
--- a/ecg-multimodal-model_amd/csrc/api.hip
+++ b/ecg-multimodal-model_amd/csrc/api.hip
@@ -248,6 +248,29 @@
   ECG_TRY(ecg_conv_igemm(dtype, 1, gd, dy_down, w_down_dgrad, tmp, nullptr, nullptr, nullptr, 0, S_(stream)));
   return ecg_conv_igemm(dtype, 1, g, dy, w_dgrad, dx, nullptr, tmp, nullptr, 0, S_(stream));
 }
+int ecgmm_conv_bwd_data_masked(int dtype, const ecgmm_conv_desc* c, const void* dy, const void* w_dgrad, const void* addend,
+                               const void* dy_down, const void* w_down_dgrad, void* dx, const uint8_t* mask_bits,
+                               int* mask_done, void* stream) {
+  if (!c || !dy || !w_dgrad || !dx || !mask_bits || !mask_done) ECG_FAIL(ECGMM_ERR_SHAPE, "conv_bwd_data_masked: null operand");
+  if ((dy_down != nullptr) != (w_down_dgrad != nullptr) || (dy_down && addend))
+    ECG_FAIL(ECGMM_ERR_SHAPE, "conv_bwd_data_masked: the downsample operands come as a pair and without an addend");
+  ConvEpi e = {};
+  e.src2 = dy_down; e.wpk2 = w_down_dgrad; e.mask_bits = mask_bits;
+  *mask_done = 0;
+  ECG_TRY(ecg_conv_igemm(dtype, 1, geom_of(c), dy, w_dgrad, dx, nullptr, addend, nullptr, 0, S_(stream), &e));
+  if (dy_down && !e.src2_done) ECG_FAIL(ECGMM_ERR_SHAPE, "conv_bwd_data_masked: this geometry does not take the folded downsample tap");
+  *mask_done = e.mask_done;
+  return 0;
+}
+int ecgmm_bcast_rows_masked(int dtype, const float* v, void* out, int N, int R, int C, float scale, const uint8_t* mask_bits,
+                            int* mask_done, void* stream) {
+  if (!mask_bits || !mask_done) ECG_FAIL(ECGMM_ERR_SHAPE, "bcast_rows_masked: null operand");
+  return ecg_bcast_rows(dtype, v, out, N, R, C, scale, S_(stream), mask_bits, mask_done);
+}
+int ecgmm_masked_dgrad(int level) {
+  sw::MASKED_DGRAD = level < 0 ? 0 : level > 2 ? 2 : level;
+  return 0;
+}
 int ecgmm_bn_bwd_from_rows(int dtype, const void* dout, const void* maskref, const void* y, const float* coef,
                            const float* gamma, float* dgamma, float* dbeta, void* dy, const float* rows, int nrows,
                            int64_t M, int C, void* scratch, void* stream) {
diff --git a/ecg-multimodal-model_amd/csrc/common.h b/ecg-multimodal-model_amd/csrc/common.h
--- a/ecg-multimodal-model_amd/csrc/common.h
+++ b/ecg-multimodal-model_amd/csrc/common.h
@@ -76,6 +76,15 @@
   for (int i = 0; i < 4; ++i) v[i] = (unsigned)f2bf(f[2 * i]) | ((unsigned)f2bf(f[2 * i + 1]) << 16);
   return v;
 }
+__device__ __forceinline__ u32x4 relu_bits_select(const u32x4& v, unsigned bits) {
+  u32x4 o;
+#pragma unroll
+  for (int i = 0; i < 4; ++i) {
+    const unsigned lo = (unsigned)__builtin_amdgcn_sbfe((int)bits, 2 * i, 1), hi = (unsigned)__builtin_amdgcn_sbfe((int)bits, 2 * i + 1, 1);
+    o[i] = v[i] & ((lo & 0xFFFFu) | (hi & 0xFFFF0000u));
+  }
+  return o;
+}
 
 __device__ __forceinline__ float wave_sum(float v) {
 #pragma unroll
diff --git a/ecg-multimodal-model_amd/csrc/conv_halo.hip b/ecg-multimodal-model_amd/csrc/conv_halo.hip
--- a/ecg-multimodal-model_amd/csrc/conv_halo.hip
+++ b/ecg-multimodal-model_amd/csrc/conv_halo.hip
@@ -28,6 +28,7 @@
   const void* red_mask;
   const float* red_coef;
   float* red_rows;
+  const unsigned char* mask_bits;
   int wg_rows;
   int M, H, W, Cs, Cd, ph, pw, act;
   int ncs;
@@ -84,9 +85,10 @@
   static constexpr int CPW = BN / WCN;
 };
 
-template <int BN, int RS, int MODE, bool NCS1 = false, int NW = 8, bool PP = false, bool ST = false, bool AD = false>
+template <int BN, int RS, int MODE, bool NCS1 = false, int NW = 8, bool PP = false, bool ST = false, bool AD = false, bool MK = false>
 __global__ __launch_bounds__(NW * 64, NW == 8 ? 2 : 2) void conv_halo_kernel(HaloParams p) {
   using C = HaloCfg<BN, NW>;
+  static_assert(!MK || (MODE == 2 && ((ST && AD) || (PP && BN == 128))), "masked stores: the two input-gradient forms the ResNet18 plan dispatches");
   static_assert(!ST || (BN == 64 && RS == 9 && NCS1 && NW == 8 && !PP && MODE != 1), "stream form: 64 -> 64 channel 3x3 tiles, no fused reduction");
   static_assert(!AD || (ST && MODE == 2), "AD = the stream form of the input gradient with a residual addend");
   static_assert(!PP || (NW == 8 && !NCS1), "ping-pong: 8-wave workgroups");
@@ -289,7 +291,8 @@
     const size_t e = (size_t)(m0 + wp * 64 + lane) * p.Cd + n0 + wc * C::CPW;
 #pragma unroll
     for (int k = 0; k < 3; ++k) {
-      const bf16_t* g = pf_base[k] ? pf_base[k] + e : (const bf16_t*)p.wpk;
+      const void* g = pf_base[k] ? (const void*)(pf_base[k] + e) : p.wpk;
+      if (MK && k == 1) g = p.mask_bits + (e >> 3);
       __builtin_amdgcn_global_load_lds((const __attribute__((address_space(1))) void*)g,
                                        (__attribute__((address_space(3))) void*)(smem + C::TRASH), 4, 0, 0);
     }
@@ -468,8 +471,8 @@
       for (int b = 0; b < TP; ++b) baddr[b][t2] = (avalid[b][t2] & mk[b]) | (zz & ~mk[b]);
     };
     constexpr auto st_ = [](int t) { t = (t + RS) % RS; return AD ? (t >= 4 && t <= 7 ? 1 : 0) : (t >= 1 && t <= 4 ? 1 : 0); };
-    constexpr auto ld_ = [](int t) { t = (t + RS) % RS; return AD && t >= 1 && t <= 4 ? 1 : 0; };
-    constexpr auto pf_ = [](int t) { t = (t + RS) % RS; return AD && t == 5 ? 1 : 0; };
+    constexpr auto ld_ = [](int t) { t = (t + RS) % RS; return AD && t >= 1 && t <= 4 ? (MK ? 2 : 1) : 0; };
+    constexpr auto pf_ = [](int t) { t = (t + RS) % RS; return AD && t == 5 ? (MK ? 2 : 1) : 0; };
     constexpr auto ex_ = [=](int t) { return st_(t) + ld_(t) + pf_(t); };
     constexpr auto hl_ = [](int t) { t = (t + RS) % RS; return t < C::NPW_MAX ? 1 : 0; };
     static_assert(C::NPW_MAX <= RS - 1 && HPS == 1, "one halo piece per step, none in the tile's last step");
@@ -478,13 +481,20 @@
     f32x4 accp[TC][TP];
     static_assert(TC == 2, "one channel-tile pair per wave");
     u32x4 adv[3];
+    unsigned mkv[MK ? 3 : 1];
     auto load_addend = [&](int b, int m0_) {
-      adv[b % 3] = *reinterpret_cast<const u32x4*>(addend + (size_t)(m0_ + wp * 64 + b * 16 + fr) * p.Cd + cw + cl);
+      const size_t e = (size_t)(m0_ + wp * 64 + b * 16 + fr) * p.Cd + cw + cl;
+      adv[b % 3] = *reinterpret_cast<const u32x4*>(addend + e);
+      if constexpr (MK) mkv[b % 3] = p.mask_bits[e >> 3];
     };
     auto prefetch_addend = [&](int m0_) {
 #if defined(__HIP_DEVICE_COMPILE__)
-      __builtin_amdgcn_global_load_lds((const __attribute__((address_space(1))) void*)(addend + (size_t)(m0_ + wp * 64 + lane) * p.Cd + cw),
+      const size_t e = (size_t)(m0_ + wp * 64 + lane) * p.Cd + cw;
+      __builtin_amdgcn_global_load_lds((const __attribute__((address_space(1))) void*)(addend + e),
                                        (__attribute__((address_space(3))) void*)(smem + C::TRASH), 4, 0, 0);
+      if constexpr (MK)
+        __builtin_amdgcn_global_load_lds((const __attribute__((address_space(1))) void*)(p.mask_bits + (e >> 3)),
+                                         (__attribute__((address_space(3))) void*)(smem + C::TRASH), 4, 0, 0);
 #endif
     };
     auto epi_unit = [&](int b, int m0_) {
@@ -525,7 +535,9 @@
       __builtin_amdgcn_global_load_lds((const __attribute__((address_space(1))) void*)p.wpk,
                                        (__attribute__((address_space(3))) void*)(smem + C::TRASH), 4, 0, 0);
 #else
-      *reinterpret_cast<u32x4*>(dst + (size_t)(m0_ + wp * 64 + b * 16 + fr) * p.Cd + cw + cl) = (u32x4){lo[0], hi[0], lo[1], hi[1]};
+      u32x4 o = (u32x4){lo[0], hi[0], lo[1], hi[1]};
+      if constexpr (MK) o = relu_bits_select(o, mkv[b % 3]);
+      *reinterpret_cast<u32x4*>(dst + (size_t)(m0_ + wp * 64 + b * 16 + fr) * p.Cd + cw + cl) = o;
 #endif
 #endif
     };
@@ -736,6 +748,7 @@
       };
       uint2 adv[2][TC][2];
       u32x4 yq[2][TA][2], mq[2][TA][2], oq[2][TA][2];
+      unsigned mkq[MK ? 2 : 1][MK ? TA : 1][2];
       auto loads = [&](auto h_tag) {
         constexpr int h = decltype(h_tag)::value;
 #pragma unroll
@@ -744,6 +757,10 @@
           if (addend) {
 #pragma unroll
             for (int a = 0; a < TC; ++a) adv[h][a][bb] = *reinterpret_cast<const uint2*>(addend + prow[b] + a * 16 + fq * 4);
+          }
+          if constexpr (MK) {
+#pragma unroll
+            for (int ap = 0; ap < TA; ++ap) mkq[h][ap][bb] = p.mask_bits[(prow[b] + ap * 32 + cl) >> 3];
           }
           if (MODE == 1 && red) {
 #pragma unroll
@@ -828,6 +845,7 @@
                   q2[ap][u * 4 + j] += g[u][j] * (yv[u][j] - c_mu[u][j]);
                 }
             }
+            if constexpr (MK) o = relu_bits_select(o, mkq[h][ap][bb]);
             oq[h][ap][bb] = o;
           }
         }
@@ -849,7 +867,7 @@
       };
       using H0 = std::integral_constant<int, 0>;
       using H1 = std::integral_constant<int, 1>;
-      if (addend == nullptr && !red) {
+      if (addend == nullptr && !red && !MK) {
         if (more) tile_fills(m0, !NCS1);
         __builtin_amdgcn_sched_barrier(0);
         compute(H0{});
@@ -1028,14 +1046,14 @@
   return Gk < 1 ? 1 : Gk;
 }
 
-template <int BN, int RS, int MODE, bool NCS1 = false, int NW = 8, bool PP = false, bool ST = false, bool AD = false>
+template <int BN, int RS, int MODE, bool NCS1 = false, int NW = 8, bool PP = false, bool ST = false, bool AD = false, bool MK = false>
 int launch_halo(const HaloParams& p, int* rows_out, hipStream_t stream) {
   using C = HaloCfg<BN, NW>;
   static bool attr_set[16] = {false};
   int dev = 0;
   (void)hipGetDevice(&dev);
   if (dev >= 0 && dev < 16 && !attr_set[dev]) {
-    if (hipFuncSetAttribute((const void*)conv_halo_kernel<BN, RS, MODE, NCS1, NW, PP, ST, AD>, hipFuncAttributeMaxDynamicSharedMemorySize,
+    if (hipFuncSetAttribute((const void*)conv_halo_kernel<BN, RS, MODE, NCS1, NW, PP, ST, AD, MK>, hipFuncAttributeMaxDynamicSharedMemorySize,
                             C::LDS) != hipSuccess)
       ECG_FAIL(ECGMM_ERR_LAUNCH, "conv_halo: cannot reserve %d bytes of LDS", C::LDS);
     attr_set[dev] = true;
@@ -1045,7 +1063,7 @@
   q.ntn = p.Cd / BN;
   const int Gk = halo_gk(q.ntn, q.ntm, NW == 4 ? 2 : 1);
   *rows_out = Gk;
-  hipLaunchKernelGGL((conv_halo_kernel<BN, RS, MODE, NCS1, NW, PP, ST, AD>), dim3(Gk * q.ntn), dim3(NW * 64), C::LDS, stream, q);
+  hipLaunchKernelGGL((conv_halo_kernel<BN, RS, MODE, NCS1, NW, PP, ST, AD, MK>), dim3(Gk * q.ntn), dim3(NW * 64), C::LDS, stream, q);
   ECG_CHECK_LAUNCH("conv_halo_kernel");
   return 0;
 }
@@ -1080,6 +1098,12 @@
 
 static bool halo_w4(const ConvGeom& g, int Cs, int Cd) {
   return sw::HALO_W4.get() && g.R == 3 && Cs == 64 && Cd == 64;
+}
+bool ecg_conv_halo_masks(const ConvGeom& g, bool addend) {
+  const int Cs = g.Cout, Cd = g.Cin;
+  if (g.R != 3 || halo_w4(g, Cs, Cd)) return false;
+  if (Cd > 64) return sw::HALO_PP.get() != 0;
+  return Cs == 64 && sw::HALO_NCS1.get() && sw::HALO_STREAM.get() && addend;
 }
 int ecg_conv_halo_rows(int mode, const ConvGeom& g) {
   const int Cd = mode == 0 ? g.Cout : g.Cin;
@@ -1113,6 +1137,9 @@
   int wg = 0;
   const bool wide = p.Cd > 64;
   int rc;
+  const bool want_mask = epi && epi->mask_bits && mode != 0 && !p.red_y && !bias && act != 1 &&
+                         ((uintptr_t)epi->mask_bits & 3) == 0 && ecg_conv_halo_masks(g, addend != nullptr);
+  if (epi) epi->mask_done = 0;
   if (halo_w4(g, p.Cs, p.Cd) && !p.red_y) {
     if (mode == 0) rc = launch_halo<64, 9, 0, false, 4>(p, &wg, stream);
     else rc = launch_halo<64, 9, 2, false, 4>(p, &wg, stream);
@@ -1120,6 +1147,11 @@
     const bool st = sw::HALO_STREAM.get() != 0;
     if (mode == 0 && st && (!p.stats || p.wg_rows) && !p.addend && !p.bias && p.act != 1) rc = launch_halo<64, 9, 0, true, 8, false, true>(p, &wg, stream);
     else if (mode != 0 && st && !p.red_y && !p.addend && !p.bias && p.act != 1) rc = launch_halo<64, 9, 2, true, 8, false, true>(p, &wg, stream);
+    else if (mode != 0 && st && want_mask && p.addend) {
+      p.mask_bits = epi->mask_bits;
+      epi->mask_done = 1;
+      rc = launch_halo<64, 9, 2, true, 8, false, true, true, true>(p, &wg, stream);
+    }
     else if (mode != 0 && st && !p.red_y && p.addend && !p.bias && p.act != 1) rc = launch_halo<64, 9, 2, true, 8, false, true, true>(p, &wg, stream);
     else if (mode == 0) rc = launch_halo<64, 9, 0, true>(p, &wg, stream);
     else if (p.red_y) rc = launch_halo<64, 9, 1, true>(p, &wg, stream);
@@ -1127,6 +1159,11 @@
   } else if (wide && g.R == 3 && sw::HALO_PP.get()) {
     if (mode == 0) rc = launch_halo<128, 9, 0, false, 8, true>(p, &wg, stream);
     else if (p.red_y) rc = launch_halo<128, 9, 1, false, 8, true>(p, &wg, stream);
+    else if (want_mask) {
+      p.mask_bits = epi->mask_bits;
+      epi->mask_done = 1;
+      rc = launch_halo<128, 9, 2, false, 8, true, false, false, true>(p, &wg, stream);
+    }
     else rc = launch_halo<128, 9, 2, false, 8, true>(p, &wg, stream);
   } else if (g.R == 3) {
     if (mode == 0) rc = wide ? launch_halo<128, 9, 0>(p, &wg, stream) : launch_halo<64, 9, 0>(p, &wg, stream);
diff --git a/ecg-multimodal-model_amd/csrc/conv_igemm.hip b/ecg-multimodal-model_amd/csrc/conv_igemm.hip
--- a/ecg-multimodal-model_amd/csrc/conv_igemm.hip
+++ b/ecg-multimodal-model_amd/csrc/conv_igemm.hip
@@ -36,6 +36,7 @@
   int act;
   const void* src2;
   const void* wpk2;
+  const unsigned char* mask_bits;
   unsigned mul_hw[4], sh_hw[4], mul_w[4], sh_w[4];
 };
 
@@ -53,8 +54,9 @@
 constexpr int ROWB = 128;
 constexpr int NTHREADS = 256;
 
-template <typename T, int BN, int MODE, int ST>
+template <typename T, int BN, int MODE, int ST, bool MK = false>
 __global__ __launch_bounds__(NTHREADS) void igemm_kernel(IgemmParams p) {
+  static_assert(!MK || (MODE == 1 && ST == 2 && sizeof(T) == 2), "masked stores: the bf16 parity-class kernel");
   constexpr int VEC = Elem<T>::VEC;
   constexpr int KBE = ROWB / (int)sizeof(T);
   constexpr int TP = 4;
@@ -202,6 +204,18 @@
     for (int b = 0; b < TP; ++b) acc[a][b] = (f32x4){0.f, 0.f, 0.f, 0.f};
 
   const int fr = lane & 15, fq = lane >> 4;
+  unsigned mb[MK ? TC / 2 : 1][MK ? TP : 1];
+  if constexpr (MK) {
+#pragma unroll
+    for (int b = 0; b < TP; ++b) {
+      const int pc = m0 + wp * 64 + b * 16 + fr;
+      const int n = div_hw(pc), rem = pc - n * HWd;
+      const int h2 = div_w(rem), w2 = rem - h2 * Wc;
+      const size_t e = (size_t)((n * p.Hd + h2 * 2 + ph) * p.Wd + w2 * 2 + pw) * p.Cd + n0 + wc * (BN / 2);
+#pragma unroll
+      for (int a = 0; a < TC; a += 2) mb[a / 2][b] = p.mask_bits[(e + ((fq & 1) ? (a + 1) * 16 + (fq - 1) * 4 : a * 16 + fq * 4)) >> 3];
+    }
+  }
   auto compute = [&](int stage) {
     const unsigned char* sW = smem + stage * STAGE_BYTES;
     const unsigned char* sX = sW + BN * ROWB;
@@ -332,7 +346,9 @@
           auto lo = __builtin_amdgcn_permlane16_swap(x0, x1, false, false);
           auto hi = __builtin_amdgcn_permlane16_swap(y0, y1, false, false);
           const int ch = (fq & 1) ? (a + 1) * 16 + (fq - 1) * 4 : a * 16 + fq * 4;
-          *reinterpret_cast<u32x4*>(dst + prow[b] + ch) = (u32x4){lo[0], hi[0], lo[1], hi[1]};
+          u32x4 o = (u32x4){lo[0], hi[0], lo[1], hi[1]};
+          if constexpr (MK) o = relu_bits_select(o, mb[a / 2][b]);
+          *reinterpret_cast<u32x4*>(dst + prow[b] + ch) = o;
         }
 #ifdef ECG_STAMP
       unsigned long long tf1;
@@ -505,7 +521,7 @@
 }
 #endif
 
-template <typename T, int BN, int MODE, int ST>
+template <typename T, int BN, int MODE, int ST, bool MK = false>
 int launch_one(const IgemmParams& p, hipStream_t stream) {
   dim3 grid(ceil_div(p.M, BM), ceil_div(p.Cd, BN));
   if (MODE == 1 && ST == 2) {
@@ -515,11 +531,11 @@
   size_t lds = 2 * (size_t)(BN + BM) * ROWB;
   static bool attr_set = false;
   if (!attr_set) {
-    (void)hipFuncSetAttribute((const void*)igemm_kernel<T, BN, MODE, ST>, hipFuncAttributeMaxDynamicSharedMemorySize,
+    (void)hipFuncSetAttribute((const void*)igemm_kernel<T, BN, MODE, ST, MK>, hipFuncAttributeMaxDynamicSharedMemorySize,
                         (int)lds);
     attr_set = true;
   }
-  hipLaunchKernelGGL((igemm_kernel<T, BN, MODE, ST>), grid, dim3(NTHREADS), lds, stream, p);
+  hipLaunchKernelGGL((igemm_kernel<T, BN, MODE, ST, MK>), grid, dim3(NTHREADS), lds, stream, p);
   ECG_CHECK_LAUNCH("igemm_kernel");
   return 0;
 }
@@ -529,6 +545,9 @@
   const bool wide = p.Cd > 64;
   if (mode == 0) return wide ? launch_one<T, 128, 0, 1>(p, stream) : launch_one<T, 64, 0, 1>(p, stream);
   if (p.stride == 1) return wide ? launch_one<T, 128, 1, 1>(p, stream) : launch_one<T, 64, 1, 1>(p, stream);
+  if constexpr (sizeof(T) == 2) {
+    if (p.stride == 2 && p.mask_bits) return wide ? launch_one<T, 128, 1, 2, true>(p, stream) : launch_one<T, 64, 1, 2, true>(p, stream);
+  }
   if (p.stride == 2) return wide ? launch_one<T, 128, 1, 2>(p, stream) : launch_one<T, 64, 1, 2>(p, stream);
   ECG_FAIL(ECGMM_ERR_SHAPE, "conv dgrad: stride %d unsupported (1 or 2)", p.stride);
 }
@@ -539,6 +558,19 @@
 
 static inline double conv_flops(const ConvGeom& g) {
   return 2.0 * (double)g.N * g.OH * g.OW * g.Cout * g.R * g.S * g.Cin;
+}
+
+bool ecg_conv_dgrad_masks(int dtype, const ConvGeom& g, bool addend) {
+  if (dtype != ECGMM_BF16) return false;
+  if (ecg_conv_halo_ok(dtype, 1, g)) return ecg_conv_halo_masks(g, addend);
+  if (g.stride != 2) return false;
+  const int Cd = g.Cin, bn = Cd > 64 ? 128 : 64;
+  if (Cd % 32 != 0 || Cd % bn != 0) return false;
+  for (int c = 0; c < 4; ++c) {
+    const long mc = (long)g.N * ((g.H - (c >> 1) + 1) >> 1) * ((g.W - (c & 1) + 1) >> 1);
+    if (mc <= 0 || mc % BM != 0) return false;
+  }
+  return true;
 }
 
 int ecg_conv_igemm(int dtype, int mode, const ConvGeom& g, const void* src, const void* wpk, void* dst,
@@ -589,8 +621,14 @@
     p.src2 = epi->src2; p.wpk2 = epi->wpk2;
     epi->src2_done = 1;
   }
+  if (epi) epi->mask_done = 0;
+  const bool halo = ecg_conv_halo_ok(dtype, mode, g);
+  if (epi && epi->mask_bits && !halo && mode == 1 && !stats && !bias && act != 1 && ecg_conv_dgrad_masks(dtype, g, addend != nullptr)) {
+    p.mask_bits = epi->mask_bits;
+    epi->mask_done = 1;
+  }
   int rc;
-  if (ecg_conv_halo_ok(dtype, mode, g)) {
+  if (halo) {
     rc = ecg_conv_halo(mode, g, src, wpk, dst, bias, addend, stats, act, epi, stream);
   } else {
     if (epi) {
diff --git a/ecg-multimodal-model_amd/csrc/elementwise.hip b/ecg-multimodal-model_amd/csrc/elementwise.hip
--- a/ecg-multimodal-model_amd/csrc/elementwise.hip
+++ b/ecg-multimodal-model_amd/csrc/elementwise.hip
@@ -605,13 +605,13 @@
         const unsigned bits = p.mask_bits[r * (p.C / VEC) + c0 / VEC];
 #pragma unroll
         for (int j = 0; j < VEC; ++j) d[j] = (bits >> j) & 1u ? d[j] : 0.f;
-      } else {
+      } else if (mref) {
         float m[VEC];
         unpack16<T>(ld16s(mref + r * p.C + c0), m);
 #pragma unroll
         for (int j = 0; j < VEC; ++j) d[j] = m[j] > 0.f ? d[j] : 0.f;
       }
-      st16((T*)p.dz + r * p.C + c0, pack16<T>(d));
+      if (p.dz) st16((T*)p.dz + r * p.C + c0, pack16<T>(d));
 #pragma unroll
       for (int j = 0; j < VEC; ++j) {
         const float xa = (va[j] - mean[0][j]) * inv[0][j];
@@ -1281,7 +1281,8 @@
 
 template <typename T>
 __global__ __launch_bounds__(1024) void bcast_rows_vec_kernel(const float* __restrict__ v, T* __restrict__ out, long M,
-                                                              RowDiv rdiv, int C, float scale) {
+                                                              RowDiv rdiv, int C, float scale,
+                                                              const unsigned char* __restrict__ bits) {
   constexpr int VEC = Elem<T>::VEC;
   const int cpr = C / VEC, rpi = 1024 / cpr;
   const int c0 = (threadIdx.x % cpr) * VEC, r0 = threadIdx.x / cpr;
@@ -1290,6 +1291,11 @@
     float f[VEC];
 #pragma unroll
     for (int j = 0; j < VEC; ++j) f[j] = src[j] * scale;
+    if (VEC == 8 && bits) {
+      const unsigned m = bits[r * cpr + c0 / VEC];
+#pragma unroll
+      for (int j = 0; j < VEC; ++j) f[j] = (m >> j) & 1u ? f[j] : 0.f;
+    }
     st16(out + r * C + c0, pack16<T>(f));
   }
 }
@@ -1620,10 +1626,11 @@
                     hipStream_t stream) {
   if (!chunk_ok(C, dtype)) ECG_FAIL(ECGMM_ERR_SHAPE, "bn_bwd_dual: C=%d unsupported", C);
   if (gate || addc || dbias) ECG_FAIL(ECGMM_ERR_SHAPE, "bn_bwd_dual: gate / addc / dbias are not supported");
+  const bool premasked = !maskref && !mask_bits && !dz;
   if (dtype != ECGMM_BF16) mask_bits = nullptr;
-  if (!dout || !y_a || !y_b || !coef_a || !coef_b || !dy_a || !dy_b || !dz || !scratch_a || !scratch_b || M < 1)
+  if (!dout || !y_a || !y_b || !coef_a || !coef_b || !dy_a || !dy_b || (!dz && !premasked) || !scratch_a || !scratch_b || M < 1)
     ECG_FAIL(ECGMM_ERR_SHAPE, "bn_bwd_dual: null operand");
-  if ((!mask_bits && !maskref) || maskref == y_a || maskref == y_b)
+  if (!premasked && ((!mask_bits && !maskref) || maskref == y_a || maskref == y_b))
     ECG_FAIL(ECGMM_ERR_SHAPE, "bn_bwd_dual: needs the ReLU mask as bits (bf16) or as a tensor of its own");
   const int grid = bn_bwd_rows(dtype, M, C);
   const float* const gamma[2] = {gamma_a, gamma_b};
@@ -1655,7 +1662,7 @@
     p.bcoef[b] = bcoef[b];
   }
   if (fold) agrid = bn_fold_grid(dtype, M, C, bn_fold_slices(C), BWD_THREADS, 8);
-  p.dout = dz; p.maskref = nullptr; p.mask_bits = nullptr; p.dz = nullptr;
+  p.dout = premasked ? dout : dz; p.maskref = nullptr; p.mask_bits = nullptr; p.dz = nullptr;
   p.dy[0] = dy_a; p.dy[1] = dy_b;
   DISPATCH_T(dtype, (bn_bwd_dual_launch<bf16_t, true>(p, agrid, stream)), (bn_bwd_dual_launch<float, true>(p, agrid, stream)),
              "bn_bwd_dual");
@@ -1824,16 +1831,20 @@
   return 0;
 }
 
-int ecg_bcast_rows(int dtype, const float* v, void* out, int N, int R, int C, float scale, hipStream_t stream) {
+int ecg_bcast_rows(int dtype, const float* v, void* out, int N, int R, int C, float scale, hipStream_t stream,
+                   const unsigned char* mask_bits, int* mask_done) {
   long total = (long)N * R * C;
+  if (mask_done) *mask_done = 0;
   const int vecw = dtype == ECGMM_BF16 ? 8 : 4;
   if (C % vecw == 0 && C / vecw <= 1024 && 1024 % (C / vecw) == 0 && ((uintptr_t)out & 15) == 0) {
     const long M = (long)N * R;
     int g = ew_grid(M, (1024 / (C / vecw)) * 4);
     if (g > 256) g = 256;
+    const unsigned char* bits = dtype == ECGMM_BF16 ? mask_bits : nullptr;
+    if (bits && mask_done) *mask_done = 1;
     DISPATCH_T(dtype,
-               hipLaunchKernelGGL(bcast_rows_vec_kernel<bf16_t>, dim3(g), dim3(1024), 0, stream, v, (bf16_t*)out, M, make_row_div(R), C, scale),
-               hipLaunchKernelGGL(bcast_rows_vec_kernel<float>, dim3(g), dim3(1024), 0, stream, v, (float*)out, M, make_row_div(R), C, scale),
+               hipLaunchKernelGGL(bcast_rows_vec_kernel<bf16_t>, dim3(g), dim3(1024), 0, stream, v, (bf16_t*)out, M, make_row_div(R), C, scale, bits),
+               hipLaunchKernelGGL(bcast_rows_vec_kernel<float>, dim3(g), dim3(1024), 0, stream, v, (float*)out, M, make_row_div(R), C, scale, bits),
                "bcast_rows");
     ECG_CHECK_LAUNCH("bcast_rows_vec");
     return 0;
diff --git a/ecg-multimodal-model_amd/csrc/ops.h b/ecg-multimodal-model_amd/csrc/ops.h
--- a/ecg-multimodal-model_amd/csrc/ops.h
+++ b/ecg-multimodal-model_amd/csrc/ops.h
@@ -13,6 +13,8 @@
   int wg_rows;
   const void* src2;
   const void* wpk2;
+  const unsigned char* mask_bits;
+  int mask_done;
   int src2_done;
   int stats_rows;
   int red_done;
@@ -21,8 +23,10 @@
 int ecg_conv_igemm(int dtype, int mode, const ConvGeom& g, const void* src, const void* wpk, void* dst,
                    const float* bias, const void* addend, float* stats, int act, hipStream_t stream,
                    ConvEpi* epi = nullptr);
+bool ecg_conv_dgrad_masks(int dtype, const ConvGeom& g, bool addend);
 bool ecg_conv_halo_ok(int dtype, int mode, const ConvGeom& g);
 int ecg_conv_halo_rows(int mode, const ConvGeom& g);
+bool ecg_conv_halo_masks(const ConvGeom& g, bool addend);
 int ecg_conv_halo(int mode, const ConvGeom& g, const void* src, const void* wpk, void* dst, const float* bias,
                   const void* addend, float* stats, int act, ConvEpi* epi, hipStream_t stream);
 size_t ecg_conv_wgrad_workspace(int dtype, const ConvGeom& g);
@@ -115,7 +119,8 @@
                     int H, int W, int C, float* scratch, hipStream_t stream);
 bool ecg_stem_fuse_on();
 int ecg_avgpool(int dtype, const void* x, float* out, int N, int R, int C, const float* coef, hipStream_t stream);
-int ecg_bcast_rows(int dtype, const float* v, void* out, int N, int R, int C, float scale, hipStream_t stream);
+int ecg_bcast_rows(int dtype, const float* v, void* out, int N, int R, int C, float scale, hipStream_t stream,
+                   const unsigned char* mask_bits = nullptr, int* mask_done = nullptr);
 int ecg_se_gate_grad(int dtype, const void* dout, const void* maskref, const void* y, const float* coef, float* dg,
                      int N, int R, int C, hipStream_t stream);
 constexpr int ECG_PACK_MAX = 24;
diff --git a/ecg-multimodal-model_amd/csrc/plan_resnet18.hip b/ecg-multimodal-model_amd/csrc/plan_resnet18.hip
--- a/ecg-multimodal-model_amd/csrc/plan_resnet18.hip
+++ b/ecg-multimodal-model_amd/csrc/plan_resnet18.hip
@@ -313,6 +313,16 @@
   struct NarrowOff { ~NarrowOff() { ecg_conv_wgrad_narrow(false); } } narrow_off;
   hipStream_t ws = side ? g_side.s : s;
 
+  auto fuse_at = [&](int j) { return (long)N * r.blk[j].hout * r.blk[j].wout >= sw::BN_FUSE_MIN_M.get(); };
+  auto masked = [&](int i) -> bool {
+    const int level = sw::MASKED_DGRAD;
+    const long Mi = (long)N * r.blk[i].hout * r.blk[i].wout;
+    if (!train || !relu_bits_on() || dt != ECGMM_BF16 || level <= 0 || !sw::BN_FUSE.get() || fuse_at(i)) return false;
+    if (level < 2 && Mi < sw::MASKED_DGRAD_MIN_M) return false;
+    if (i == 7) return true;
+    return !fuse_at(i + 1) && ecg_conv_dgrad_masks(dt, r.blk[i + 1].conv1_geom(N), !r.blk[i + 1].down);
+  };
+
   if (stage_begin == 0) ecg_tl_mark(200, s);
   for (int st = stage_begin; st < stage_end; ++st) {
     if (st > 0) ecg_tl_mark(200 + st, s);
@@ -322,7 +332,10 @@
       const Blk18& last = r.blk[7];
       ECG_TRY(fc_bwd(r, w, q, dfeat, params, grads, s));
       const int R = last.hout * last.wout;
-      ECG_TRY(ecg_bcast_rows(dt, q.dpooled, q.X[0], N, R, 512, 1.f / (float)R, s));
+      int mdone = 0;
+      const bool mk7 = masked(7);
+      ECG_TRY(ecg_bcast_rows(dt, q.dpooled, q.X[0], N, R, 512, 1.f / (float)R, s, mk7 ? w.b[7].bits : nullptr, &mdone));
+      if (mk7 && !mdone) ECG_FAIL(ECGMM_ERR_LAUNCH, "resnet18 bwd: the avgpool backward did not store the masked gradient");
     } else if (st <= 8) {
       const int i = 8 - st;
       const Blk18& k = r.blk[i];
@@ -348,12 +361,17 @@
       const void* dzp = q.dz;
       const bool dual = k.down && train && !fused2 && ecg_bn_dual_on() &&
                         ecg_bn_bwd_scratch(dt, M, k.cout) <= RED_ROWS_FLOATS * sizeof(float);
+      const bool in_masked = masked(i);
+      if (in_masked) dzp = dcur;
       if (dual) {
         main_wait(s, g_side.done2[2][pp]);
-        ECG_TRY(ecg_bn_bwd_dual(dt, dcur, b.out, relu_bits_on() ? b.bits : nullptr, nullptr, nullptr, b.y2, b.coef2,
-                                P(params, k.p_bn2), G(grads, k.p_bn2), G(grads, k.p_bn2 + 1), dyb, b.yd, b.coefd,
-                                P(params, k.p_dbn), G(grads, k.p_dbn), G(grads, k.p_dbn + 1), dydb, q.dz, nullptr, M, k.cout,
-                                q.bn_scratch, q.red2, s));
+        ECG_TRY(ecg_bn_bwd_dual(dt, dcur, in_masked ? nullptr : b.out, !in_masked && relu_bits_on() ? b.bits : nullptr, nullptr,
+                                nullptr, b.y2, b.coef2, P(params, k.p_bn2), G(grads, k.p_bn2), G(grads, k.p_bn2 + 1), dyb, b.yd,
+                                b.coefd, P(params, k.p_dbn), G(grads, k.p_dbn), G(grads, k.p_dbn + 1), dydb,
+                                in_masked ? nullptr : q.dz, nullptr, M, k.cout, q.bn_scratch, q.red2, s));
+      } else if (in_masked) {
+        ECG_TRY(bn_bwd_mode(r.bn, dcur, nullptr, nullptr, nullptr, 1, b.y2, b.coef2, P(params, k.p_bn2), G(grads, k.p_bn2),
+                            G(grads, k.p_bn2 + 1), dyb, nullptr, nullptr, M, k.cout, q.bn_scratch, s));
       } else if (fused2) {
         dzp = dcur;
         ECG_TRY(ecg_bn_bwd_tail(dt, dcur, nullptr, b.y2, b.coef2, P(params, k.p_bn2), G(grads, k.p_bn2),
@@ -384,6 +402,8 @@
         ECG_TRY(ecg_conv_wgrad(dt, g1, in, dy1b, G(grads, k.p_conv1), 0, q.wg_ws, q.wg_bytes, ws));
         if (side) g_side.done2[1][pp] = side_mark();
       }
+      const unsigned char* out_bits = i > 0 && masked(i - 1) ? w.b[i - 1].bits : nullptr;
+      int out_done = 0;
       if (k.down) {
         ConvGeom gd = k.down_geom(N);
         if (!dual) {
@@ -398,22 +418,27 @@
         }
         ConvEpi ed = {};
         ed.src2 = dydb; ed.wpk2 = b.wdd;
+        ed.mask_bits = out_bits;
         if (!sw::DOWN_FOLD.get()) ed.src2 = nullptr;
         if (ed.src2) {
           ECG_TRY(ecg_conv_igemm(dt, 1, g1, dy1b, b.w1d, din, nullptr, nullptr, nullptr, 0, s, &ed));
         }
         if (!ed.src2_done) {
           ECG_TRY(ecg_conv_igemm(dt, 1, gd, dydb, b.wdd, q.dtmp, nullptr, nullptr, nullptr, 0, s));
-          ECG_TRY(ecg_conv_igemm(dt, 1, g1, dy1b, b.w1d, din, nullptr, q.dtmp, nullptr, 0, s));
+          ECG_TRY(ecg_conv_igemm(dt, 1, g1, dy1b, b.w1d, din, nullptr, q.dtmp, nullptr, 0, s, &ed));
         }
+        out_done = ed.mask_done;
       } else {
         ConvEpi eb = {};
         if (fuse_here && i > 0 && ecg_conv_halo_ok(dt, 1, g1)) {
           const BlockWs& pb = w.b[i - 1];
           eb.wg_rows = 1; eb.red_y = pb.y2; eb.red_mask = pb.out; eb.red_coef = pb.coef2; eb.red_rows = q.red2;
         }
+        eb.mask_bits = out_bits;
         ECG_TRY(ecg_conv_igemm(dt, 1, g1, dy1b, b.w1d, din, nullptr, dzp, nullptr, 0, s, &eb));
-      }
+        out_done = eb.mask_done;
+      }
+      if (out_bits && !out_done) ECG_FAIL(ECGMM_ERR_LAUNCH, "resnet18 bwd: block %d's conv1 input gradient did not store the masked gradient", i);
     } else if (st == 9) {
       const void* dp0 = q.X[8 & 1];
       if (stem_recompute(dt)) {
diff --git a/ecg-multimodal-model_amd/csrc/switches.h b/ecg-multimodal-model_amd/csrc/switches.h
--- a/ecg-multimodal-model_amd/csrc/switches.h
+++ b/ecg-multimodal-model_amd/csrc/switches.h
@@ -65,6 +65,9 @@
 inline Switch HEAD_FUSED     {"ECGMM_HEAD_FUSED",      Switch::ON,    1,     0, 0,     false, "fusion head on the row kernels of head_fused.hip (0: ~45 per-op launches)"};
 inline Switch DENSE16        {"ECGMM_DENSE16",         Switch::ON,    1,     0, 0,     false, "batch-sized Linear layers on dense16_kernel (0: the implicit-GEMM route)"};
 
+inline int MASKED_DGRAD = 1;
+constexpr long MASKED_DGRAD_MIN_M = 64;
+
 inline Switch* const ALL[] = {
     &CONV_HALO,  &HALO_CUS,      &HALO_W4,       &HALO_STAGGER, &HALO_STREAM,   &HALO_PP,   &HALO_NCS1,  &WGRAD_RING,      &WGRAD_PP,
     &WGRAD_GROUPS, &WGRAD_WGS,   &BN_FOLD,       &BN_FOLD_SLICE, &BN_FUSE,      &BN_FUSE_MIN_M, &RELU_BITS, &STEM_FUSE,    &STEM_RECOMPUTE,
diff --git a/ecg-multimodal-model_amd/hip/lib.py b/ecg-multimodal-model_amd/hip/lib.py
--- a/ecg-multimodal-model_amd/hip/lib.py
+++ b/ecg-multimodal-model_amd/hip/lib.py
@@ -145,6 +145,9 @@
     "ecgmm_pool_bn_bwd": (i32, [i32, vp, vp, vp, vp, vp, vp, vp, vp, vp, vp, i32, i32, i32, i32, vp, vp]),
     "ecgmm_avgpool": (i32, [i32, vp, vp, i32, i32, i32, vp, vp]),
     "ecgmm_bcast_rows": (i32, [i32, vp, vp, i32, i32, i32, f32, vp]),
+    "ecgmm_bcast_rows_masked": (i32, [i32, vp, vp, i32, i32, i32, f32, vp, P(i32), vp]),
+    "ecgmm_conv_bwd_data_masked": (i32, [i32, P(ConvDesc), vp, vp, vp, vp, vp, vp, vp, P(i32), vp]),
+    "ecgmm_masked_dgrad": (i32, [i32]),
     "ecgmm_se_gate_grad": (i32, [i32, vp, vp, vp, vp, vp, i32, i32, i32, vp]),
     "ecgmm_se_gate_bn": (i32, [i32, vp, vp, vp, vp, vp, vp, vp, vp, vp, i32, i32, i32, vp]),
     "ecgmm_se_mlp_fwd": (i32, [vp, vp, vp, vp, vp, vp, vp, i32, i32, i32, vp]),
@@ -310,7 +313,8 @@
                  "ecgmm_crnn_front_infer_workspace", "ecgmm_crnn_front_infer",
                  "ecgmm_linear_res_ln", "ecgmm_ffn_res_ln", "ecgmm_transformer_infer_prepared_bytes",
                  "ecgmm_transformer_infer_prepare", "ecgmm_transformer_infer_workspace", "ecgmm_transformer_infer",
-                 "ecgmm_tabnet_infer_prepared_bytes", "ecgmm_tabnet_infer_prepare", "ecgmm_tabnet_infer")
+                 "ecgmm_tabnet_infer_prepared_bytes", "ecgmm_tabnet_infer_prepare", "ecgmm_tabnet_infer",
+                 "ecgmm_conv_bwd_data_masked", "ecgmm_bcast_rows_masked", "ecgmm_masked_dgrad")
 
 _lib = None
 
diff --git a/include/ecgmm.h b/include/ecgmm.h
--- a/include/ecgmm.h
+++ b/include/ecgmm.h
@@ -222,6 +222,12 @@
                       float* dgamma_b, float* dbeta_b, void* dy_b, void* dz, float* dbias, int64_t M, int C, void* scratch_a,
                       void* scratch_b, void* stream);
 int ecgmm_bn_dual(int on);
+int ecgmm_conv_bwd_data_masked(int dtype, const ecgmm_conv_desc* c, const void* dy, const void* w_dgrad, const void* addend,
+                               const void* dy_down, const void* w_down_dgrad, void* dx, const uint8_t* mask_bits,
+                               int* mask_done, void* stream);
+int ecgmm_bcast_rows_masked(int dtype, const float* v, void* out, int N, int R, int C, float scale, const uint8_t* mask_bits,
+                            int* mask_done, void* stream);
+int ecgmm_masked_dgrad(int level);
 int ecgmm_stem_recompute(int on);
 
 int ecgmm_bnrelu_maxpool(int dtype, const void* y, const float* coef, void* out, uint8_t* idx, int N, int H, int W,
```
